# lamm-mit/MoleculeDiffusionTransformer

Measured on AMD Instinct MI355X. Metric: molecules/sec @64 diffusion steps (QM9 max_len=64), higher is better.
Workload: dtype f32 storage/accumulate; GEMM products as split-bf16 (bf16x3) MFMA; 1 GPU; QMDiffusion inverse sample(): channels=64 pred_dim=16 max_len=64 cond_len=12, batch=1024/GPU, 64 timesteps (126 U-Net evals), cond_scale=1.0, fp32; global_batch=1024, parallelism=batch-shard x1

## Files before the change

### include/mdt_hip.h

```cpp
#ifndef MDT_HIP_H
#define MDT_HIP_H

#include <stdint.h>

#ifdef __cplusplus
extern "C" {
#endif

#define MDT_ABI_VERSION 5

int mdt_abi_version(void);
const char *mdt_last_error(void);
int mdt_set_tuning(const char *key, int32_t value);
int32_t mdt_pair_capacity(void);
int32_t mdt_tf256_block_core(int32_t T, int32_t Tk, int32_t cross);
int mdt_test_occupy(int32_t n_workgroups, int32_t lds_bytes, uint64_t ticks, void *stream);


enum mdt_space {
  MDT_SP_NONE = 0,
  MDT_SP_WEIGHT = 1,
  MDT_SP_ACT = 2,
  MDT_SP_SHR = 3,
  MDT_SP_EXT0 = 4
// ... 65 lines not shown
                MDT_N_CA = 6      };
enum mdt_gn_f { MDT_NF_EPS = 0, MDT_NF_SCALE2 = 1 };

enum mdt_rconv_i { MDT_R_T = 0, MDT_R_C = 1, MDT_R_LDA = 2, MDT_R_LDC = 3, MDT_R_LDR = 4, MDT_R_TAPS = 5,
                   MDT_R_GSIZE = 6 , MDT_R_SILU = 7,
                   MDT_R_FILM_LD = 8 ,
                   MDT_R_LDA2 = 9 ,
                   MDT_R_WF32 = 10 ,
                   MDT_R_KSRC = 11 ,
                   MDT_R_HALF_OUT = 12 ,
                   MDT_R_NB = 13  };
enum mdt_rconv_f { MDT_RF_EPS = 0, MDT_RF_IN_SCALE = 1 ,
                   MDT_RF_IN_SCALE2 = 2  };
enum mdt_resblock_i { MDT_K_T = 0, MDT_K_CIN = 1, MDT_K_COUT = 2, MDT_K_FILM_LD = 3,
                      MDT_K_WF32 = 4 ,
                      MDT_K_CIN_REAL = 5, MDT_K_COUT_REAL = 6 ,
                      MDT_K_PATCH_IN = 7, MDT_K_PATCH_OUT = 8  };
enum mdt_resblock_f { MDT_KF_EPS = 0 };

enum mdt_attn_i {
  MDT_A_T = 0, MDT_A_TK = 1, MDT_A_HEADS = 2, MDT_A_LDQ = 3, MDT_A_LDKV = 4, MDT_A_LDO = 5,
  MDT_A_KV_BSTRIDE = 6,
  MDT_A_OUT16 = 7,
  MDT_A_QCOL = 8,
  MDT_A_KCOL = 9,
  MDT_A_SPLIT = 10,
  MDT_A_IN16 = 11
};
enum mdt_attn_f { MDT_AF_SCALE = 0 };

enum mdt_concat_i { MDT_C_ROWS = 0, MDT_C_CA = 1, MDT_C_CB = 2 };
enum mdt_concat_f { MDT_CF_SCALE_B = 0 };

enum mdt_patch_i { MDT_P_ROWS_IN = 0, MDT_P_C_IN = 1, MDT_P_LD_IN = 2, MDT_P_LD_OUT = 3, MDT_P_PATCH = 4,
                   MDT_P_INVERSE = 5 };

enum mdt_time_i { MDT_T_HALF = 0, MDT_T_LD = 1 };

enum mdt_tblock_mode { MDT_TB_SELF = 0, MDT_TB_CROSS = 1, MDT_TB_FF = 2 };
enum mdt_tblock_i {
  MDT_B_MODE = 0, MDT_B_C = 1,
  MDT_B_T = 2,
  MDT_B_NCHUNK = 3,
  MDT_B_NBIAS = 4, MDT_B_TK = 5, MDT_B_KV_BSTRIDE = 6, MDT_B_LDKV = 7, MDT_B_HEADS = 8,
  MDT_B_KV2 = 11,
  MDT_B_POST = 10,
  MDT_B_VARIANT = 9,
  MDT_B_WF32 = 12
};
enum mdt_tblock_f { MDT_BF_EPS = 0, MDT_BF_SCALE = 1 };

enum mdt_tf128_i {
  MDT_F_C = 0,
  MDT_F_T = 1,
  MDT_F_NT = 2,
  MDT_F_NVEC = 3,
  MDT_F_TK = 4, MDT_F_KV_BSTRIDE = 5, MDT_F_LDKV = 6, MDT_F_HEADS = 7,
  MDT_F_HAS_IN = 8,
  MDT_F_NBLOCKS = 9 , MDT_F_NFF = 10 ,
  MDT_F_NPOST = 11,
  MDT_F_KV2 = 12,
  MDT_F_CROSS = 13,
  MDT_F_KV_LSTRIDE = 14,
  MDT_F_RES_KIND = 15,
  MDT_F_N_RES = 16,
  MDT_F_RES_PAIR1 = 17,
  MDT_F_RES_PAIR2 = 18,
  MDT_F_NFILM = 19,
  MDT_F_NSPLIT = 20,
  MDT_F_PAIR_STRIDE = 21,
  MDT_F_WF32 = 22
};
enum mdt_tf128_f { MDT_FF_EPS_LN = 0, MDT_FF_SCALE = 1, MDT_FF_EPS_GN = 2, MDT_FF_EPS_RES = 3, MDT_FF_SKIP_SCALE = 4 };

typedef struct mdt_op {
  int32_t kind;
  int32_t film_bstride;
  mdt_ref a;
  mdt_ref a2;
  mdt_ref w;
  mdt_ref bias;
  mdt_ref out;
  mdt_ref res;
  mdt_ref p0, p1, p2, p3;
  int32_t i[24];
  float f[8];
} mdt_op;

typedef struct mdt_bindings {
  const float *weights;
  float *act;
  float *shr;
  float *ext[MDT_N_EXT];
} mdt_bindings;

typedef struct mdt_program mdt_program;

mdt_program *mdt_program_create(const mdt_op *ops, int32_t n_ops);
void mdt_program_destroy(mdt_program *p);
int32_t mdt_program_num_ops(const mdt_program *p);
int mdt_program_run(const mdt_program *p, const mdt_bindings *b, int32_t B, int32_t n_shared_rows,
                    int32_t first, int32_t count, void *stream);

int mdt_cond_embed(const float *seq, const float *fc1_w, const float *fc1_b, const float *inv_freq,
                   float *out, int32_t B, int32_t n, int32_t D1, int32_t D2, void *stream);
int mdt_cond_embed_add(const float *seq, const float *fc1_w, const float *fc1_b, const float *inv_freq,
                       float *out, int32_t B, int32_t n, int32_t D1, int32_t D2, void *stream);

int mdt_precond_in(const float *x, float *xin, float c_in, int32_t B, int32_t C, int32_t L, int32_t Cp,
                   void *stream);
int mdt_precond_out(const float *x, const float *pred, float *D, float c_skip, float c_out, int32_t B,
                    int32_t C, int32_t L, int32_t Cp, const float *dyn_scale, void *stream);
int mdt_dyn_scale(const float *x, const float *pred, float *scale, float c_skip, float c_out, float q, int32_t B,
                  int32_t C, int32_t L, int32_t Cp, void *stream);
int mdt_noise_in_rows(const float *x0, const float *noise, const float *sigma, const float *c_in, float *x_noisy, float *xin,
                      uint64_t seed, uint32_t step, int64_t sample0, int32_t B, int32_t C, int32_t L, int32_t Cp, void *stream);
int mdt_precond_in_rows(const float *x, float *xin, const float *c_in, int32_t B, int32_t C, int32_t L, int32_t Cp, void *stream);
int mdt_precond_out_rows(const float *x, const float *pred, float *D, const float *c_skip, const float *c_out, int32_t B,
                         int32_t C, int32_t L, int32_t Cp, const float *dyn_scale, void *stream);
int mdt_dyn_scale_rows(const float *x, const float *pred, float *scale, const float *c_skip, const float *c_out, float q,
                       int32_t B, int32_t C, int32_t L, int32_t Cp, void *stream);
int mdt_loss_rows(const float *x0, const float *x_noisy, const float *pred, const float *c_skip, const float *c_out,
                  const float *weight, const float *dyn_scale, float *loss, int32_t B, int32_t C, int32_t L, int32_t Cp,
                  void *stream);
int mdt_cfg_mix(const float *cond, const float *uncond, float *out, float scale, int64_t n, void *stream);
int mdt_cfg_mix_rows(const float *cond, const float *uncond, float *out, const float *scale, int32_t B, int64_t row_elems,
                     void *stream);
int mdt_adpm2_mid(const float *x, const float *pred, float *x_mid, float *xin_mid, float c_skip,
                  float c_out, float sigma, float dt_mid, float c_in_mid, int32_t B, int32_t C, int32_t L,
                  int32_t Cp, const float *dyn_scale, void *stream);
int mdt_adpm2_next(float *x, const float *x_mid, const float *pred, const float *noise, float *xin_next,
                   float c_skip, float c_out, float sigma_mid, float dt_down, float sigma_up,
                   float c_in_next, uint64_t seed, uint32_t step, int64_t sample0, int32_t B, int32_t C,
                   int32_t L, int32_t Cp, int32_t *tokens, const float *dyn_scale, void *stream);
int mdt_adpm2_euler(const float *x_base, const float *x_from, const float *denoised, const float *noise,
                    float *out, float sigma, float dt, float sigma_up, int32_t noise_mode, uint64_t seed,
                    uint32_t step, int64_t sample0, int32_t B, int32_t C, int32_t L, void *stream);
int mdt_aeuler_next(float *x, const float *pred, const float *noise, float *xin_next, float c_skip, float c_out,
                    float sigma, float dt, float sigma_up, float c_in_next, uint64_t seed, uint32_t step,
                    int64_t sample0, int32_t B, int32_t C, int32_t L, int32_t Cp, int32_t *tokens,
                    const float *dyn_scale, void *stream);
int mdt_karras_hat(const float *x, const float *noise, float *x_hat, float *xin, float noise_scale, float s_noise,
                   float c_in_hat, uint64_t seed, uint32_t step, int64_t sample0, int32_t B, int32_t C, int32_t L,
                   int32_t Cp, void *stream);
int mdt_karras_mid(const float *x_hat, const float *pred, float *d, float *x_next, float *xin_next, float c_skip,
                   float c_out, float sigma_hat, float dt, float c_in_next, int32_t B, int32_t C, int32_t L,
                   int32_t Cp, int32_t *tokens, const float *dyn_scale, void *stream);
int mdt_karras_next(const float *x_hat, const float *x_next, const float *d, const float *pred, float *x,
                    float c_skip, float c_out, float sigma_next, float half, int32_t B, int32_t C, int32_t L,
                    int32_t Cp, int32_t *tokens, const float *dyn_scale, void *stream);
int mdt_init_noise(float *x, const float *noise, float sigma0, uint64_t seed, uint32_t step,
                   int64_t sample0, int32_t B, int32_t C, int32_t L, void *stream);
int mdt_copy_f32(float *dst, const float *src, int64_t n, void *stream);
int mdt_clamp(float *x, float lo, float hi, int64_t n, void *stream);
int mdt_inpaint_merge(float *x, const float *src, const uint8_t *mask, const float *noise, float sigma,
                      uint64_t seed, uint32_t step, int64_t sample0, int32_t B, int32_t C, int32_t L,
                      void *stream);
int mdt_add_noise(float *x, const float *noise, float s, uint64_t seed, uint32_t step, int64_t sample0,
                  int32_t B, int32_t C, int32_t L, void *stream);
int mdt_inpaint_enter(float *x, float *xin, const float *src, const int32_t *draft, const uint8_t *keep,
                      int32_t keep_per_token, const float *n_src, const float *n_re, float sigma, float renoise,
                      float c_in, uint64_t seed, uint32_t step_src, uint32_t step_re, int64_t sample0, int32_t B,
                      int32_t C, int32_t L, int32_t Cp, void *stream);
int mdt_inpaint_finish(float *x, const float *src, const int32_t *draft, const uint8_t *keep, int32_t keep_per_token,
                       int32_t *tokens, int32_t B, int32_t C, int32_t L, void *stream);
int mdt_refine_enter(float *x, float *xin, const int32_t *start, int32_t step_i, const float *src, const int32_t *draft,
                     const float *noise, float sigma, float c_in, uint64_t seed, uint32_t step, int64_t sample0, int32_t B,
                     int32_t C, int32_t L, int32_t Cp, void *stream);
int mdt_refine_keep_enter(float *x, float *xin, const int32_t *start, int32_t step_i, const float *src, const int32_t *draft,
                          const uint8_t *keep, int32_t keep_per_token, const float *n_entry, const float *n_src, float sigma,
                          float c_in, uint64_t seed, uint32_t step_entry, uint32_t step_src, int64_t sample0, int32_t B,
                          int32_t C, int32_t L, int32_t Cp, void *stream);
int mdt_argmax_tokens(const float *x, int32_t *tokens, int32_t B, int32_t C, int32_t L, void *stream);

int mdt_tokens_compact(const int32_t *tokens, int32_t B, int32_t L, float *fwd_in, int32_t Lf, double x_norm, int32_t *packed,
                       int32_t *length, uint64_t *key, void *stream);
int mdt_screen_score(const float *props, int64_t row_stride, const float *target, const float *weights, int32_t N, int32_t G,
                     int32_t n, float *score, void *stream);
enum mdt_screen_status {
  MDT_SCREEN_EMPTY = 1,
  MDT_SCREEN_NONFINITE = 2,
  MDT_SCREEN_DUPLICATE = 4,
  MDT_SCREEN_KNOWN = 8,
  MDT_SCREEN_CLOSE = 16,
  MDT_SCREEN_MALFORMED = 32,
  MDT_SCREEN_OVERVALENT = 64,
  MDT_SCREEN_SUBSTRUCTURE = 128
};
int mdt_screen_select(const float *score, const uint64_t *key, const int32_t *packed, const int32_t *length, int32_t L, int32_t N,
                      int32_t G, const uint64_t *known_key, const int32_t *known_packed, const int32_t *known_len, int32_t M,
                      int32_t K, uint8_t *status, int32_t *index, int32_t *count, void *stream);
int mdt_screen_select_reject(const float *score, const uint64_t *key, const int32_t *packed, const int32_t *length, int32_t L,
                             int32_t N, int32_t G, const uint64_t *known_key, const int32_t *known_packed, const int32_t *known_len,
                             int32_t M, int32_t K, const uint8_t *reject, uint8_t *status, int32_t *index, int32_t *count,
                             void *stream);

int mdt_edit_distance_rows(const int32_t *a_packed, const int32_t *a_len, const int32_t *b_packed, const int32_t *b_len, int32_t L,
                           int32_t R, int32_t *dist, void *stream);
#define MDT_EDIT_KNOWN_CHUNK 512
int mdt_edit_nearest(const int32_t *packed, const int32_t *length, int32_t L, int32_t R, const int32_t *known_packed,
                     const int32_t *known_len, int32_t M, uint64_t *best, int32_t *dist, int32_t *index, void *stream);
int mdt_screen_select_diverse(const float *score, const uint64_t *key, const int32_t *packed, const int32_t *length, int32_t L,
                              int32_t N, int32_t G, const uint64_t *known_key, const int32_t *known_packed, const int32_t *known_len,
                              int32_t M, int32_t K, const int32_t *known_dist, int32_t min_novelty, int32_t min_distance,
                              uint8_t *status, int32_t *index, int32_t *count, void *stream);
int mdt_screen_select_diverse_reject(const float *score, const uint64_t *key, const int32_t *packed, const int32_t *length,
                                     int32_t L, int32_t N, int32_t G, const uint64_t *known_key, const int32_t *known_packed,
                                     const int32_t *known_len, int32_t M, int32_t K, const int32_t *known_dist, int32_t min_novelty,
                                     int32_t min_distance, const uint8_t *reject, uint8_t *status, int32_t *index, int32_t *count,
                                     void *stream);

int mdt_smiles_check(const int32_t *packed, const int32_t *length, int32_t L, int32_t R, const uint8_t *classes,
                     const uint8_t *max_valence, const uint32_t *elements, uint8_t *status, int32_t *position, void *stream);

int mdt_mol_graph(const int32_t *packed, const int32_t *length, int32_t L, int32_t R, const uint8_t *classes,
                  const uint8_t *max_valence, const uint32_t *elements, int32_t *natoms, uint32_t *atoms, int32_t *nbonds,
                  uint32_t *bonds, uint8_t *status, int32_t *position, void *stream);
int mdt_mol_key(const int32_t *natoms, const uint32_t *atoms, const int32_t *nbonds, const uint32_t *bonds, int32_t L, int32_t R,
                uint64_t *key, void *stream);
int mdt_key_flags(const uint64_t *key, int32_t N, int32_t G, const uint64_t *known_key, int32_t M, uint8_t *flags, void *stream);

#define MDT_FP_BITS 1024
#define MDT_FP_SIM_DEN 65536
int mdt_mol_fp(const int32_t *natoms, const uint32_t *atoms, const int32_t *nbonds, const uint32_t *bonds, int32_t L, int32_t R,
               int32_t radius, uint64_t *fp, int32_t *count, void *stream);
int mdt_fp_tanimoto_rows(const uint64_t *a_fp, const uint64_t *b_fp, int32_t R, int32_t *inter, int32_t *uni, void *stream);
#define MDT_FP_KNOWN_CHUNK 512
int mdt_fp_nearest(const uint64_t *fp, int32_t R, const uint64_t *known_fp, int32_t M, uint64_t *best, int32_t *inter, int32_t *uni,
                   int32_t *index, void *stream);
int mdt_screen_select_similar(const float *score, const uint64_t *key, const int32_t *packed, const int32_t *length, int32_t L,
                              int32_t N, int32_t G, const uint64_t *known_key, const int32_t *known_packed, const int32_t *known_len,
                              int32_t M, int32_t K, const int32_t *known_dist, int32_t min_novelty, int32_t min_distance,
                              const uint8_t *reject, const uint64_t *fp, const int32_t *fp_count, int32_t sim_num, uint8_t *status,
                              int32_t *index, int32_t *count, void *stream);

#define MDT_SUB_MAX_PATTERNS 32
#define MDT_SUB_MAX_WIDTH 32
#define MDT_SUB_MAX_STEPS 4096
int mdt_sub_match(const int32_t *natoms, const uint32_t *atoms, const int32_t *nbonds, const uint32_t *bonds, int32_t L, int32_t R,
                  const int32_t *p_natoms, const uint32_t *p_atoms, const int32_t *p_nbonds, const uint32_t *p_bonds,
                  int32_t LP, int32_t P, uint32_t need, uint32_t ban,
                  uint32_t *match, uint32_t *undecided, uint8_t *flags, void *stream);

#define MDT_MOLH_MAX_STEPS 4096
#define MDT_MOLH_FORMULA 13
enum mdt_molh_verdict { MDT_MOLH_OK = 0, MDT_MOLH_AROMATIC_OVERVALENT = 1, MDT_MOLH_NO_KEKULE = 2, MDT_MOLH_UNDECIDED = 3 };
int mdt_mol_hydrogens(const int32_t *natoms, const uint32_t *atoms, const int32_t *nbonds, const uint32_t *bonds, int32_t L, int32_t R,
                      int32_t max_steps, uint8_t *hydrogens, uint8_t *partner, uint8_t *verdict, int32_t *atom, int32_t *formula,
                      void *stream);

#define MDT_MOLR_DESC 16
enum mdt_molr_slot {
  MDT_MOLR_HEAVY_ATOMS = 0, MDT_MOLR_HETERO_ATOMS = 1, MDT_MOLR_DONORS = 2, MDT_MOLR_ACCEPTORS = 3, MDT_MOLR_ROTATABLE_BONDS = 4,
  MDT_MOLR_RINGS = 5, MDT_MOLR_RING_ATOMS = 6, MDT_MOLR_RING_BONDS = 7, MDT_MOLR_SMALLEST_RING = 8, MDT_MOLR_LARGEST_RING = 9,
  MDT_MOLR_AROMATIC_ATOMS = 10, MDT_MOLR_AROMATIC_OUTSIDE_RING = 11, MDT_MOLR_SP3_CARBONS = 12, MDT_MOLR_CARBONS = 13,
  MDT_MOLR_COMPONENTS = 14, MDT_MOLR_WEIGHT = 15
};
int mdt_mol_rings(const int32_t *natoms, const uint32_t *atoms, const int32_t *nbonds, const uint32_t *bonds, const uint8_t *hydrogens,
                  int32_t L, int32_t R, const int32_t *lo, const int32_t *hi, uint8_t *bond_ring, uint8_t *atom_ring, int32_t *desc,
                  uint8_t *flags, void *stream);

enum mdt_moln_flag { MDT_MOLN_NORMALIZED = 1, MDT_MOLN_AROMATIC = 2, MDT_MOLN_CHANGED = 4 };
int mdt_mol_normalize(const int32_t *natoms, const uint32_t *atoms, const int32_t *nbonds, const uint32_t *bonds,
                      const uint8_t *hydrogens, const uint8_t *partner, const uint8_t *verdict, const uint8_t *bond_ring, int32_t L,
                      int32_t R, uint32_t *out_atoms, uint32_t *out_bonds, uint8_t *flags, void *stream);

typedef struct mdt_timer mdt_timer;
mdt_timer *mdt_timer_create(int32_t max_intervals);
void mdt_timer_destroy(mdt_timer *t);
int mdt_timer_start(mdt_timer *t, void *stream);
int mdt_timer_stop(mdt_timer *t, void *stream);
int32_t mdt_timer_collect(mdt_timer *t, float *ms, int32_t cap);

#ifdef __cplusplus
}
#endif
#endif
```

### moleculediffusiontransformer_amd/build.py

```python
from __future__ import annotations

import hashlib
import os
import shutil
import subprocess
from concurrent.futures import ThreadPoolExecutor

CSRC = os.path.join(os.path.dirname(os.path.abspath(__file__)), "csrc")
INCLUDE = os.path.join(os.path.dirname(os.path.dirname(os.path.abspath(__file__))), "include")
_TAG = os.environ.get("MDT_LIB_TAG", "")
LIB = os.path.join(CSRC, f"libmdt_hip{'_' + _TAG if _TAG else ''}.so")
STAMP = os.path.join(CSRC, f".build_stamp{'_' + _TAG if _TAG else ''}")

SOURCES = [
    ("k_gemm.hip", []),
    ("k_gemm_bf16x3.hip", []),
    ("k_gemm_b16.hip", []),
    ("k_gemm_as.hip", []),
    ("k_tblock_lw.hip", ["-mllvm", "-amdgpu-mfma-vgpr-form=1"]),
    ("k_tblock32.hip", ["-mllvm", "-amdgpu-mfma-vgpr-form=1"]),
    ("k_tf128.hip", ["-mllvm", "-amdgpu-mfma-vgpr-form=1"]),
    ("k_tf128_f32.hip", ["-mllvm", "-amdgpu-mfma-vgpr-form=1"]),
    ("k_tf256.hip", ["-mllvm", "-amdgpu-mfma-vgpr-form=1"]),
    ("k_tf256_f32.hip", ["-mllvm", "-amdgpu-mfma-vgpr-form=1"]),
    ("k_rconv.hip", ["-mllvm", "-amdgpu-mfma-vgpr-form=1"]),
    ("k_rconv_f32.hip", ["-mllvm", "-amdgpu-mfma-vgpr-form=1"]),
    ("k_proj.hip", ["-mllvm", "-amdgpu-mfma-vgpr-form=1"]),
    ("k_res256.hip", ["-mllvm", "-amdgpu-mfma-vgpr-form=1"]),
    ("k_resblock.hip", ["-mllvm", "-amdgpu-mfma-vgpr-form=1"]),
    ("k_norm.hip", []),
    ("k_attn.hip", []),
    ("k_elem.hip", ["-ffp-contract=off"]),
    ("k_screen.hip", ["-ffp-contract=off"]),
    ("k_edit.hip", []),
    ("k_smiles.hip", []),
    ("k_molgraph.hip", []),
    ("k_molfp.hip", []),
    ("k_molsub.hip", []),
    ("k_molh.hip", []),
    ("k_molring.hip", []),
    ("k_molnorm.hip", []),
    ("mdt_api.cpp", ["-x", "hip"]),
]
COMMON = ["-O3", "-std=c++17", "-fPIC", "--offload-arch=gfx950", "-fno-gpu-rdc", "-Wall", "-Wno-unused-function"]


def _hipcc() -> str:
    for cand in (shutil.which("hipcc"), "/opt/rocm/bin/hipcc"):
        if cand and os.path.exists(cand):
            return cand
    raise RuntimeError("hipcc not found: libmdt_hip.so cannot be built")


def _digest() -> str:
    h = hashlib.sha256()
    paths = [os.path.join(CSRC, n) for n in sorted(os.listdir(CSRC))] + [os.path.join(INCLUDE, "mdt_hip.h")]
    for p in paths:
        if p.endswith((".hip", ".cpp", ".h")):
            h.update(os.path.basename(p).encode())
            with open(p, "rb") as f:
                h.update(f.read())
    h.update(repr((SOURCES, COMMON, os.environ.get('MDT_BUILD_DEFS', ''))).encode())
    return h.hexdigest()


def library_path() -> str:
    return LIB


def is_fresh() -> bool:
    if not (os.path.exists(LIB) and os.path.exists(STAMP)):
        return False
    with open(STAMP) as f:
        return f.read().strip() == _digest()


def build_library(force: bool = False, verbose: bool = False) -> str:
    if not force and is_fresh():
        return LIB
    import fcntl
    with open(os.path.join(CSRC, ".build_lock"), "w") as lock:
        fcntl.flock(lock, fcntl.LOCK_EX)
        try:
            if not force and is_fresh():
                return LIB
            return _build_locked(verbose)
        finally:
            fcntl.flock(lock, fcntl.LOCK_UN)


def _build_locked(verbose: bool) -> str:
    hipcc = _hipcc()

    def compile_one(item):
        src, extra = item
        obj = os.path.join(CSRC, os.path.splitext(src)[0] + (f".{_TAG}.o" if _TAG else ".o"))
        defs = os.environ.get("MDT_BUILD_DEFS", "").split()
        cmd = [hipcc, *COMMON, *extra, *defs, "-I", INCLUDE, "-c", os.path.join(CSRC, src), "-o", obj]
        r = subprocess.run(cmd, capture_output=True, text=True)
        if r.returncode != 0:
            raise RuntimeError(f"hipcc failed on {src}:\n{r.stdout}\n{r.stderr}")
        if verbose and r.stderr.strip():
            print(r.stderr)
        return obj

    with ThreadPoolExecutor(max_workers=min(5, os.cpu_count() or 1)) as ex:
        objs = list(ex.map(compile_one, SOURCES))
    cmd = [hipcc, "-shared", "-fPIC", "--offload-arch=gfx950", "-o", LIB, *objs]
    r = subprocess.run(cmd, capture_output=True, text=True)
    if r.returncode != 0:
        raise RuntimeError(f"link failed:\n{r.stdout}\n{r.stderr}")
    with open(STAMP, "w") as f:
        f.write(_digest())
    return LIB


if __name__ == "__main__":
    import sys
    print(build_library(force="--force" in sys.argv, verbose=True))
```

### moleculediffusiontransformer_amd/compiler.py

```python
from __future__ import annotations

import os
from dataclasses import dataclass, field
from typing import Dict, List, Optional, Tuple

import torch

from . import runtime as rt
from .netspec import UNetConfig

EXT_XIN, EXT_CTX, EXT_OUT = 0, 1, 2
EXT_XFLAGS, EXT_XBUF = 3, 4
EXT_FILM = 5


def pad16(c: int) -> int:
    return (c + 15) // 16 * 16


@dataclass
class Ten:
    space: int
    off: int
    rows: int
    ld: int
    c: int = 0
    b16: bool = False

    def ref(self) -> rt.MdtRef:
        return rt.MdtRef(self.space, 0, self.off)


def _ref(space: int = 0, off: int = 0) -> rt.MdtRef:
    return rt.MdtRef(space, 0, off)


class _Arena:

    def __init__(self):
        self.free: List[Tuple[int, int]] = []
        self.top = 0

    def alloc(self, n: int) -> int:
        n = (n + 63) // 64 * 64
        for i, (o, s) in enumerate(self.free):
            if s >= n:
                if s == n:
                    self.free.pop(i)
                else:
                    self.free[i] = (o + n, s - n)
                return o
        o = self.top
        self.top += n
        return o

    def release(self, off: int, n: int) -> None:
        n = (n + 63) // 64 * 64
        self.free.append((off, n))
        self.free.sort()
        merged: List[Tuple[int, int]] = []
        for o, s in self.free:
            if merged and merged[-1][0] + merged[-1][1] == o:
                merged[-1] = (merged[-1][0], merged[-1][1] + s)
            else:
                merged.append((o, s))
        self.free = merged


class _Weights:
    def __init__(self):
        self.chunks: List[torch.Tensor] = []
        self.n = 0
        self.index: Dict[str, int] = {}
        self.starts: Dict[int, torch.Tensor] = {}

    def read(self, off: int, n: int) -> torch.Tensor:
        t = self.starts[off]
        assert t.numel() >= n, (off, n, t.numel())
        return t[:n].clone()

    def add(self, name: str, t: torch.Tensor) -> int:
        t = t.detach().to(torch.float32).contiguous().reshape(-1).cpu()
        off = self.n
        pad = (-t.numel()) % 64
        self.chunks.append(t)
        self.starts[off] = t
        if pad:
            self.chunks.append(torch.zeros(pad))
        self.n += t.numel() + pad
        self.index[name] = off
        return off

    def pack(self) -> torch.Tensor:
        return torch.cat(self.chunks) if self.chunks else torch.zeros(0)


@dataclass
class CompiledUNet:
    cfg: UNetConfig
    length: int
    cond_len: int
    in_pad: int
    weights: torch.Tensor
    programs: Dict[str, List[rt.MdtOp]]
    act_floats: int
    shr_floats: int
    max_time_rows: int
    shr: Dict[str, int]
    ss_total: int
    n_cross: int
    flops_per_sample_eval: int
    flops_ctx_per_sample: int
    gemm_mode: str = "bf16x3"
    weight_index: Dict[str, int] = field(default_factory=dict)
    dual_multiple: int = 1
    tf256: bool = False
    xchg_tokens: int = 0
    rows: bool = False
    act_named: Dict[str, int] = field(default_factory=dict)


class UNetCompiler:
    def __init__(self, cfg: UNetConfig, length: int, cond_len: int, sd: Dict[str, torch.Tensor],
                 max_time_rows: int = 1024, gemm_mode: str = "bf16x3", fuse_blocks: bool = True, tf256: bool = False):
        self.fuse_blocks = fuse_blocks
        self.use_rconv = os.environ.get("MDT_RCONV", "1") == "1"
        self.use_resblock = os.environ.get("MDT_RESBLOCK", "1") == "1"
        self.t1_fold = os.environ.get("MDT_T1_FOLD", "1") == "1"
        self.ctx_split = os.environ.get("MDT_CTX_SPLIT", "1") == "1"
        self.fold_out = os.environ.get("MDT_FOLD_OUT", "1") == "1"
        self.rconv_two = os.environ.get("MDT_RCONV2", "k1") == "1"
        self.rconv_two_k1 = os.environ.get("MDT_RCONV2", "k1") in ("1", "k1")
        self.res128 = os.environ.get("MDT_RES128", "1") == "1"
        self.res256_mode = os.environ.get("MDT_RES256", "auto")
        self.patch_conv = os.environ.get("MDT_PATCH_CONV", "1") != "0"
        self.fold_patch = os.environ.get("MDT_FOLD_PATCH", "1") != "0"
        self.use_proj = os.environ.get("MDT_PROJ", "1") != "0"
        self.b16 = os.environ.get("MDT_B16", "1") == "1"
        self.res16 = os.environ.get("MDT_RES16", "1") == "1"
        self.lnfold = os.environ.get("MDT_LNFOLD", "1") == "1"
        self.cat_fold = os.environ.get("MDT_CAT_FOLD", "1") == "1"
        self.qkv_merge = os.environ.get("MDT_QKV_MERGE", "1") == "1"
        self.fold_ctx = os.environ.get("MDT_FOLD_CTX", "1") == "1"
        self.has_chat = False
        self.tf128 = os.environ.get("MDT_TF128", "1") == "1"
        self.tf256 = bool(tf256)
        self.tf256_pair = os.environ.get("MDT_TF256_PAIR", "1") == "1"
        self.pair_stride = int(os.environ.get("MDT_PAIR_STRIDE", "8"))
        self.xchg_tokens = 0
        if gemm_mode not in ("f32", "bf16x3", "bf16"):
            raise ValueError("gemm_mode must be 'f32' (exact fp32 MFMA), 'bf16x3' (split-bf16 MFMA, fp32-class) or 'bf16' "
                             "(plain bf16 products, reduced precision: layer-by-layer GEMMs only)")
        self.gemm_mode = gemm_mode
        self.wf32 = gemm_mode == "f32" and os.environ.get("MDT_F32_FUSED", "1") == "1"
        self.ring_mode = gemm_mode == "bf16x3" or self.wf32
        self.rows = False
        self._packed: Dict = {}
        self._zeros_off, self._zeros_len = 0, 0
        if cfg.channels % 16:
            raise ValueError("channels must be a multiple of 16")
        if length % (cfg.patch_size * _prod(cfg.factors)):
            raise ValueError("max_length must be divisible by patch_size * prod(factors)")
        if cfg.head_features != 64:
            raise ValueError("attention kernel is specialised for head_features == 64")
        if cfg.ctx_features % 16:
            raise ValueError("context features must be a multiple of 16")
        self.cfg, self.L, self.n_ctx, self.sd = cfg, length, cond_len, sd
        self.W = _Weights()
        self.arena = _Arena()
        self._ones_off: Dict[int, int] = {}
        self.ops: List[rt.MdtOp] = []
        self.flops = 0
        self.max_time_rows = max_time_rows
        self.kv_slots: List[int] = []
        self.kv_fixed: List[int] = []
        self.cross_layers: List[str] = []
        self.ss_offsets: Dict[str, int] = {}
        self.ss_total = 0
        self.shr_top = 0
        self.shr: Dict[str, int] = {}

    def use_rows(self) -> "UNetCompiler":
        if self.gemm_mode == "bf16":
            raise ValueError("the per-row evaluation (batched=True, eval_loss) is built and pinned for gemm_mode 'bf16x3' and 'f32'; "
                             "in the plain-bf16 mode the FiLM rows also enter MDT_OP_PREP16, which reads one shared row")
        self.rows = True
        self.res128, self.res256_mode = False, "0"
        return self

    def _shr_alloc(self, name: str, n: int) -> int:
        off = self.shr_top
        self.shr_top += (n + 63) // 64 * 64
        self.shr[name] = off
        return off

    def _new(self, rows: int, ld: int, c: int = 0) -> Ten:
        return Ten(rt.SP_ACT, self.arena.alloc(rows * ld), rows, ld, c or ld)

    def _new16(self, rows: int, n: int) -> Ten:
        return Ten(rt.SP_ACT, self.arena.alloc(rows * n // 2), rows, n, n, True)

    def _free(self, t: Ten) -> None:
        if t.space == rt.SP_ACT:
            self.arena.release(t.off, t.rows * t.ld // (2 if t.b16 else 1))

    def b16_ok(self, cin: int) -> bool:
        return self.gemm_mode == "bf16" and self.b16 and cin % 64 == 0

    def _ones(self, n: int) -> int:
        if n not in self._ones_off:
            self._ones_off[n] = self.W.add(f"ones{n}", torch.ones(n))
        return self._ones_off[n]

    def _zeros(self, n: int) -> int:
        if n > self._zeros_len:
            self._zeros_off = self.W.add(f"zeros{n}", torch.zeros(n))
            self._zeros_len = n
        return self._zeros_off

    def _vec(self, key: str, pad_to: int) -> int:
        v = self.sd[key]
        out = torch.zeros(pad_to)
        out[: v.numel()] = v
        return self.W.add(key, out)

    def _lin_w(self, key: str, n_pad: Optional[int] = None, k_pad: Optional[int] = None):
        w = self.sd[key]
        n, k = w.shape
        out = torch.zeros(n_pad or pad16(n), k_pad or pad16(k))
        out[:n, :k] = w
        return (key, out)

    def _conv_w(self, key: str, cin_pad: int, n_pad: int):
        w = self.sd[key]
        co, ci, k = w.shape
        out = torch.zeros(n_pad, k, cin_pad)
        out[:co, :, :ci] = w.permute(0, 2, 1)
        return (key, out.reshape(n_pad, k * cin_pad))

    def _pack_w(self, wt, cin: int):
        name, w = wt
        split = self.gemm_mode == "bf16x3" and cin % 32 == 0
        plain = self.gemm_mode == "bf16" and cin % 32 == 0
        key = (name, split, plain)
        if key not in self._packed:
            if plain:
                hi = w.to(torch.bfloat16)
                self._packed[key] = (self.W.add(name + "/bf16", hi.contiguous().view(-1).view(torch.float32)), None, 1)
            elif split:
                hi = w.to(torch.bfloat16)
                lo = (w - hi.float()).to(torch.bfloat16)
                self._packed[key] = (self.W.add(name + "/bf16_hi", hi.contiguous().view(-1).view(torch.float32)),
                                     self.W.add(name + "/bf16_lo", lo.contiguous().view(-1).view(torch.float32)))
            else:
                self._packed[key] = (self.W.add(name, w), None)
        return self._packed[key]

    def _emit(self, op: rt.MdtOp) -> None:
        self.ops.append(op)

    def gemm(self, a: Ten, wt, n: int, out: Ten, *, cin: int, bias_off: Optional[int] = None,
             taps: int = 1, t_stride: int = 1, t_dj: int = 0, t_off: int = 0, r_out: Optional[int] = None,
             o_stride: int = 1, o_off: int = 0, res: Optional[Ten] = None, pro: int = rt.PRO_NONE,
             gain: Optional[int] = None, nbias: Optional[int] = None, stats: Optional[Ten] = None,
             film: Optional[rt.MdtRef] = None, groups: int = 0, gsize: int = 0, pro_silu: int = 0,
             act: int = 0, eps: float = 0.0, m_mode: int = 0, a_col: int = 0, o_col: int = 0,
             count_flops: bool = True, phases: int = 0, copy16: Optional[Ten] = None) -> None:
        r_out_ = a.rows if r_out is None else r_out
        a16 = None
        regular = (self.b16_ok(cin) and t_stride == 1 and phases <= 1 and o_stride == 1 and o_off == 0 and r_out_ == a.rows
                   and out.rows == r_out_ and m_mode == 0)
        assert not (a.b16 or out.b16) or (regular and (not a.b16 or (pro in (rt.PRO_NONE, rt.PRO_LAYERNORM) and a_col == 0))), "bf16 operand"
        lnf = None
        if (self.lnfold and regular and a.b16 and pro == rt.PRO_LAYERNORM and taps == 1 and t_off == 0 and out.b16 and res is None
                and copy16 is None and n % 8 == 0 and o_col % 8 == 0 and out.ld % 8 == 0):
            key = (wt[0], "lnfold", gain, nbias, bias_off)
            if key not in self._packed:
                w = wt[1].double()
                gv, bv = self.W.read(gain, cin).double(), self.W.read(nbias, cin).double()
                b0 = self.W.read(bias_off, n).double() if bias_off is not None else torch.zeros(n, dtype=torch.float64)
                w2 = (w * gv.unsqueeze(0)).float()
                csum = w2.to(torch.bfloat16).double().sum(dim=1).float()
                self._packed[key] = ((wt[0] + "/lnfold", w2), self.W.add(wt[0] + "/lnfold.bias", (b0 + w @ bv).float()),
                                     self.W.add(wt[0] + "/lnfold.csum", csum))
            wt, bias_off, csum_off = self._packed[key]
            lnf = csum_off
            pro, gain, nbias = rt.PRO_NONE, None, None
        if regular and (not a.b16 or pro == rt.PRO_LAYERNORM):
            a16 = self._new16(a.rows, cin)
            pre = rt.MdtOp()
            pre.kind = rt.OP_PREP16
            pre.a, pre.out = a.ref(), a16.ref()
            if gain is not None:
                pre.p0 = _ref(rt.SP_WEIGHT, gain)
            if nbias is not None:
                pre.p1 = _ref(rt.SP_WEIGHT, nbias)
            if stats is not None:
                pre.p2 = stats.ref()
# ... 1322 lines not shown
            blocks = [dp + f"blocks.{j}." for j in range(nb)]
            res_ok = nb > 0 and all(self.res128_ok(bp, co, x.rows, g, False) for bp in blocks)
            together = res_ok and self.tf128_ok(co, x.rows, nat, nat > 0, 1, nb)
            alone = res_ok and not together and self.tf128_ok(co, x.rows, 0, False, 1, nb)
            if together or alone:
                n_out = nb + (1 if nat > 0 else 0)
                base = self.arena.alloc(n_out * x.rows * co)
                outs = [Ten(rt.SP_ACT, base + k * x.rows * co, x.rows, co, co) for k in range(n_out)]
                if together:
                    self.transformer_fused128(x, dp + "transformer.", co, nat, nat > 0, free_input=not x_is_skip,
                                              res=(1, blocks, g, outs[:nb], 1.0), y=outs[-1])
                else:
                    self.transformer_fused128(x, "", co, 0, False, free_input=not x_is_skip,
                                              res=(1, blocks, g, outs[:nb], 1.0), y=outs[nb - 1])
                    if nat > 0:
                        yy = self.transformer(outs[nb - 1], dp + "transformer.", co, nat, True, free_input=False, y_out=outs[nb])
                        if yy is not outs[nb]:
                            self._free(outs[nb])
                            outs[nb] = yy
                skips += outs
                x = outs[-1]
            elif nb > 0 and x.ld == co and all(self.res256_ok(bp, co, x.rows, g, False) for bp in blocks):
                n_out = nb + (1 if nat > 0 else 0)
                base = self.arena.alloc(n_out * x.rows * co)
                outs = [Ten(rt.SP_ACT, base + k * x.rows * co, x.rows, co, co) for k in range(n_out)]
                self.resnet_chain256(x, blocks, 1, outs[:nb], 1.0, outs[nb - 1], free_input=not x_is_skip)
                if nat > 0:
                    yy = self.transformer(outs[nb - 1], dp + "transformer.", co, nat, True, free_input=False, y_out=outs[nb])
                    if yy is not outs[nb]:
                        self._free(outs[nb])
                        outs[nb] = yy
                skips += outs
                x = outs[-1]
            else:
                for bp in blocks:
                    x = self.resnet(x, bp, co, co, g, free_input=not x_is_skip)
                    skips.append(x)
                    x_is_skip = True
                if nat > 0:
                    x = self.transformer(x, dp + "transformer.", co, nat, True, free_input=False)
                    skips.append(x)
            skips_list.append(skips)
        cb = cfg.level_channels(cfg.num_layers)
        keep = x in skips_list[-1]
        x = self.resnet(x, "bottleneck.pre_block.", cb, cb, g, free_input=not keep)
        if cfg.attentions[-1] > 0:
            x = self.transformer(x, "bottleneck.transformer.", cb, cfg.attentions[-1], True)
        x = self.resnet(x, "bottleneck.post_block.", cb, cb, g)
        for u, i in enumerate(reversed(range(cfg.num_layers))):
            up = f"upsamples.{u}."
            ci, co, f = cfg.level_channels(i + 1), cfg.level_channels(i), cfg.factors[i]
            skips = skips_list.pop()
            n_res = cfg.num_blocks[i] + (1 if cfg.attentions[i] else 0)
            blocks = [up + f"blocks.{j}." for j in range(n_res)]
            tfs = []
            if cfg.pre_transformer > 0:
                tfs.append((up + "pre_transformer_block.", cfg.pre_transformer, False))
            if cfg.attentions[i] > 0:
                tfs.append((up + "transformer.", cfg.attentions[i], True))
            cons = skips[len(skips) - n_res:][::-1] if 0 < n_res <= len(skips) else []
            nxt = tfs[0] if tfs else ("", 0, False)
            res_ok = (bool(cons) and x.ld == ci and all(self.res128_ok(bp, ci, x.rows, g, True) for bp in blocks)
                      and all(sk.space == rt.SP_ACT and sk.rows == x.rows and sk.ld == ci
                              and sk.off == cons[0].off - k * x.rows * ci for k, sk in enumerate(cons)))
            together = res_ok and nxt[1] > 0 and self.tf128_ok(ci, x.rows, nxt[1], nxt[2], 2, n_res)
            fused = together or (res_ok and self.tf128_ok(ci, x.rows, 0, False, 2, n_res))
            if fused:
                del skips[len(skips) - n_res:]
                if together:
                    x = self.transformer_fused128(x, nxt[0], ci, nxt[1], nxt[2], True, res=(2, blocks, g, cons, 2 ** -0.5))
                    tfs = tfs[1:]
                else:
                    x = self.transformer_fused128(x, "", ci, 0, False, True, res=(2, blocks, g, cons, 2 ** -0.5))
                for sk in cons:
                    self._free(sk)
            elif (bool(cons) and x.ld == ci and all(self.res256_ok(bp, ci, x.rows, g, True) for bp in blocks)
                  and all(sk.space == rt.SP_ACT and sk.rows == x.rows and sk.ld == ci
                          and sk.off == cons[0].off - k * x.rows * ci for k, sk in enumerate(cons))):
                del skips[len(skips) - n_res:]
                x = self.resnet_chain256(x, blocks, 2, cons, 2 ** -0.5, self._new(x.rows, ci), True)
                for sk in cons:
                    self._free(sk)
            else:
                for bp in blocks:
                    sk = skips.pop()
                    x = self.resnet_cat(x, sk, 2 ** -0.5, bp, ci, g)
            for sk in skips:
                self._free(sk)
            for tp, tl, tc in tfs:
                x = self.transformer(x, tp, ci, tl, tc)
            if f % 2:
                raise ValueError("odd upsample factors are not supported")
            wt = self.sd[up + "upsample.weight"]
            bias = self._vec(up + "upsample.bias", co)
            y = self._new(x.rows * f, co)
            last = u == cfg.num_layers - 1
            res = skips_list[0][0] if last else None
            if self.up_patch_ok(x, ci, co, f, res):
                self.up_patch(x, up, ci, co, f, y, res)
            else:
                wall = torch.cat([torch.stack((wt[:, :, ph], wt[:, :, ph + f]), dim=0).permute(2, 0, 1).reshape(co, 2 * ci)
                                  for ph in range(f)])
                self.gemm(x, (f"{up}upsample.weight/phases", wall), co, y, cin=ci, bias_off=bias, taps=2, t_stride=1,
                          t_dj=-1, t_off=0, r_out=x.rows, o_stride=f, o_off=0, res=res, phases=f)
            self._free(x)
            x = y
        self._free(skips_list.pop()[0])
        fold_in = (ps > 1 and self.fold_patch and x.ld % ps == 0
                   and self.resblock_ok(x.rows * ps, c0 // ps, cin, 1, "to_out.block.") and x.ld // ps == pad16(c0 // ps))
        if fold_in:
            x = Ten(x.space, x.off, x.rows * ps, x.ld // ps, x.ld // ps)
        elif ps > 1:
            y = self.patch(x, ps, inverse=True)
            self._free(x)
            x = y
        out = Ten(rt.SP_EXT0 + EXT_OUT, 0, L, self.in_pad, cin)
        y = self.resnet(x, "to_out.block.", c0 // ps, cin, 1)
        if fold_in:
            assert self.ops[-1].kind == rt.OP_RESBLOCK
            self.ops[-1].i[rt.K_PATCH_IN] = ps
        last_op = self.ops[-1]
        assert last_op.kind in (rt.OP_GEMM, rt.OP_RESBLOCK)
        last_op.out = out.ref()
        self._free(y)

    def build(self) -> CompiledUNet:
        cfg = self.cfg
        mid2 = 2 * cfg.mid_features
        self.build_eval()
        eval_ops = self.ops
        flops_eval = self.flops
        n_cross = len(self.cross_layers)
        kv_base = self.arena.top
        self.kv_slots = [kv_base + i * self.n_ctx * mid2 for i in range(n_cross)]
        act_floats = kv_base + n_cross * self.n_ctx * mid2
        chat_slot = act_floats
        if self.has_chat:
            act_floats += (self.n_ctx * cfg.ctx_features + 63) // 64 * 64

        rows = 0 if self.rows else self.max_time_rows
        mapf = cfg.mapping_features
        ldt = pad16(cfg.channels + 1)
        cn = self._shr_alloc("c_noise", rows)
        temb = self._shr_alloc("time_embed", rows * ldt)
        m1 = self._shr_alloc("map1", rows * mapf)
        m2 = self._shr_alloc("map2", rows * mapf)
        m3 = self._shr_alloc("map3", rows * mapf)
        ss_all = self._shr_alloc("ss_all", rows * self.ss_total)
        ss_cur = self._shr_alloc("ss_cur", self.ss_total)
        kvf = self._shr_alloc("kv_fixed", n_cross * self.n_ctx * mid2)
        self.kv_fixed = [kvf + i * self.n_ctx * mid2 for i in range(n_cross)]
        chat_fixed = self._shr_alloc("chat_fixed", self.n_ctx * cfg.ctx_features)

        def resolve(ops, fixed: bool):
            out = []
            for op in ops:
                o = rt.MdtOp()
                C_memmove(o, op)
                if op.kind in (rt.OP_GEMM, rt.OP_GN_ACT, rt.OP_RCONV, rt.OP_RESBLOCK, rt.OP_PREP16, rt.OP_TF128, rt.OP_RES256) and isinstance(getattr(op, "_film", None), tuple):
                    if self.rows:
                        if not (op.kind in (rt.OP_GN_ACT, rt.OP_RCONV, rt.OP_RESBLOCK)
                                or (op.kind == rt.OP_GEMM and op.i[rt.G_PRO] == rt.PRO_GROUPNORM and op.i[rt.G_WFMT] == 0
                                    and op.i[rt.G_M_MODE] == 0)):
                            raise NotImplementedError(f"per-row evaluation: the FiLM rows reach op kind {op.kind} "
                                                      f"({rt.OP_NAMES.get(op.kind)}), which reads one shared row: this U-Net shape is "
                                                      "outside the per-row envelope")
                        o.p3 = _ref(rt.SP_EXT0 + EXT_FILM, op._film[1])
                        o.film_bstride = self.ss_total
                    else:
                        o.p3 = _ref(rt.SP_SHR, ss_cur + op._film[1])
                if op.kind == rt.OP_ATTN_CTX:
                    if fixed:
                        o.a2 = _ref(rt.SP_SHR, chat_fixed)
                        o.i[rt.A_KV_BSTRIDE] = 0
                    else:
                        o.a2 = _ref(rt.SP_ACT, chat_slot)
                elif op.kind in (rt.OP_ATTN, rt.OP_TBLOCK, rt.OP_TF128, rt.OP_TF256) and isinstance(getattr(op, "_kv", None), tuple):
                    idx = op._kv[1]
                    slot = {rt.OP_ATTN: rt.A_KV_BSTRIDE, rt.OP_TBLOCK: rt.B_KV_BSTRIDE, rt.OP_TF128: rt.F_KV_BSTRIDE,
                            rt.OP_TF256: rt.F_KV_BSTRIDE}[op.kind]
                    if fixed:
                        o.a2 = _ref(rt.SP_SHR, self.kv_fixed[idx])
                        o.i[slot] = 0
                    else:
                        o.a2 = _ref(rt.SP_ACT, self.kv_slots[idx])
                out.append(o)
            return out

        if self.rows:
            programs = {"eval_rows": resolve(eval_ops, False), "eval_rows_fixed": resolve(eval_ops, True)}
        else:
            programs = {"eval": resolve(eval_ops, False), "eval_fixed": resolve(eval_ops, True)}
        cross = [op for op in eval_ops if isinstance(getattr(op, "_kv", None), tuple)]
        ring = all(op.kind in (rt.OP_TF128, rt.OP_TF256) or
                   (op.kind == rt.OP_TBLOCK and (op.i[rt.B_VARIANT] >= 2 or (op.i[rt.B_VARIANT] == 0 and op.i[rt.B_C] == 128
                                                                         and (16 // op.i[rt.B_T]) * op.i[rt.B_TK] <= 16)))
                   for op in cross)
        dual_multiple = 1
        if cross and ring and not self.rows and os.environ.get("MDT_CFG_DUAL", "1") == "1":
            dual_multiple = max(64 // op.i[rt.F_T] if op.kind == rt.OP_TF128 else 32 // op.i[rt.F_T] if op.kind == rt.OP_TF256
                                else (32 if op.i[rt.B_VARIANT] >= 2 else 64) // op.i[rt.B_T] for op in cross)
            dual = resolve(eval_ops, False)
            for o, op in zip(dual, eval_ops):
                if isinstance(getattr(op, "_kv", None), tuple):
                    o.p1 = _ref(rt.SP_SHR, self.kv_fixed[op._kv[1]])
                    o.i[rt.F_KV2 if op.kind in (rt.OP_TF128, rt.OP_TF256) else rt.B_KV2] = 1
            programs["eval_dual"] = dual

        self.ops, self.flops = [], 0
        act_named: Dict[str, int] = {}
        tm = 0 if self.rows else 1
        if self.rows:
            def act_alloc(name: str, n: int) -> int:
                nonlocal act_floats
                off = act_named[name] = act_floats
                act_floats += (n + 63) // 64 * 64
                return off
            sp = rt.SP_ACT
            cn, temb = act_alloc("c_noise", 1), act_alloc("time_embed", ldt)
            m1, m2, m3 = act_alloc("map1", mapf), act_alloc("map2", mapf), act_alloc("map3", mapf)
        else:
            sp = rt.SP_SHR
        t_cn = Ten(sp, cn, 1, 1)
        t_emb = Ten(sp, temb, 1, ldt)
        op = rt.MdtOp()
        op.kind = rt.OP_TIME_EMBED
        op.a, op.w, op.out = t_cn.ref(), _ref(rt.SP_WEIGHT, self.W.add("to_time.0.0.weights", self.sd["to_time.0.0.weights"])), t_emb.ref()
        op.i[rt.T_HALF], op.i[rt.T_LD] = cfg.channels // 2, ldt
        self._emit(op)
        t1, t2, t3 = Ten(sp, m1, 1, mapf), Ten(sp, m2, 1, mapf), Ten(sp, m3, 1, mapf)
        self.gemm(t_emb, self._lin_w("to_time.0.1.weight", mapf, ldt), mapf, t1, cin=ldt,
                  bias_off=self._vec("to_time.0.1.bias", mapf), act=1, m_mode=tm)
        self.gemm(t1, self._lin_w("to_mapping.0.weight"), mapf, t2, cin=mapf,
                  bias_off=self._vec("to_mapping.0.bias", mapf), act=1, m_mode=tm)
        self.gemm(t2, self._lin_w("to_mapping.2.weight"), mapf, t3, cin=mapf,
                  bias_off=self._vec("to_mapping.2.bias", mapf), act=1, m_mode=tm)
        w_all = torch.zeros(self.ss_total, mapf)
        b_all = torch.zeros(self.ss_total)
        for p, off in self.ss_offsets.items():
            w = self.sd[p + "to_scale_shift.to_scale_shift.1.weight"]
            b = self.sd[p + "to_scale_shift.to_scale_shift.1.bias"]
            c = w.shape[0] // 2
            cp = pad16(c)
            w_all[off: off + c] = w[:c]
            w_all[off + cp: off + cp + c] = w[c:]
            b_all[off: off + c] = b[:c]
            b_all[off + cp: off + cp + c] = b[c:]
        t_ss = Ten(rt.SP_EXT0 + EXT_FILM, 0, 1, self.ss_total) if self.rows else Ten(rt.SP_SHR, ss_all, 1, self.ss_total)
        self.gemm(t3, ("scale_shift_all.weight", w_all), self.ss_total, t_ss, cin=mapf,
                  bias_off=self.W.add("scale_shift_all.bias", b_all), pro=rt.PRO_SILU, m_mode=tm)
        programs["time_rows" if self.rows else "time"] = self.ops

        self.ops, self.flops = [], 0
        ctx = Ten(rt.SP_EXT0 + EXT_CTX, 0, self.n_ctx, cfg.ctx_features)
        fixed = Ten(rt.SP_WEIGHT, self.W.add("fixed_embedding.embedding.weight",
                                             self.sd["fixed_embedding.embedding.weight"][: self.n_ctx]),
                    self.n_ctx, cfg.ctx_features)
        ctx_ops, fixed_ops = [], []
        for idx, p in enumerate(self.cross_layers):
            w = self._lin_w(p + "to_kv.weight")
            gain = self._vec(p + "norm_context.weight", cfg.ctx_features)
            nb = self._vec(p + "norm_context.bias", cfg.ctx_features)
            self.ops = ctx_ops
            self.gemm(ctx, w, mid2, Ten(rt.SP_ACT, self.kv_slots[idx], self.n_ctx, mid2), cin=cfg.ctx_features,
                      pro=rt.PRO_LAYERNORM, gain=gain, nbias=nb, eps=1e-5)
            self.ops = fixed_ops
            self.gemm(fixed, w, mid2, Ten(rt.SP_SHR, self.kv_fixed[idx], self.n_ctx, mid2), cin=cfg.ctx_features,
                      pro=rt.PRO_LAYERNORM, gain=gain, nbias=nb, eps=1e-5, m_mode=2, count_flops=False)
        if self.has_chat:
            F_ = cfg.ctx_features
            eye = ("ctx_identity", torch.eye(F_))
            ones, zeros = self.W.add("ctx_ones", torch.ones(F_)), self._zeros(F_)
            self.ops = ctx_ops
            self.gemm(ctx, eye, F_, Ten(rt.SP_ACT, chat_slot, self.n_ctx, F_), cin=F_, pro=rt.PRO_LAYERNORM, gain=ones,
                      nbias=zeros, eps=1e-5)
            self.ops = fixed_ops
            self.gemm(fixed, eye, F_, Ten(rt.SP_SHR, chat_fixed, self.n_ctx, F_), cin=F_, pro=rt.PRO_LAYERNORM, gain=ones,
                      nbias=zeros, eps=1e-5, m_mode=2, count_flops=False)
        programs["ctx"], programs["ctx_fixed"] = ctx_ops, fixed_ops
        flops_ctx = self.flops

        return CompiledUNet(cfg=cfg, length=self.L, cond_len=self.n_ctx, in_pad=self.in_pad, weights=self.W.pack(),
                            programs=programs, act_floats=act_floats, shr_floats=self.shr_top,
                            max_time_rows=rows, shr=dict(self.shr), ss_total=self.ss_total, n_cross=n_cross,
                            flops_per_sample_eval=flops_eval, flops_ctx_per_sample=flops_ctx, gemm_mode=self.gemm_mode,
                            weight_index=dict(self.W.index), dual_multiple=dual_multiple, tf256=self.tf256,
                            xchg_tokens=self.xchg_tokens, rows=self.rows, act_named=act_named)


def C_memmove(dst: rt.MdtOp, src: rt.MdtOp) -> None:
    import ctypes
    ctypes.memmove(ctypes.byref(dst), ctypes.byref(src), ctypes.sizeof(rt.MdtOp))


def _prod(xs) -> int:
    r = 1
    for x in xs:
        r *= x
    return r


def compile_unet(cfg: UNetConfig, length: int, cond_len: int, sd: Dict[str, torch.Tensor],
                 max_time_rows: int = 1024, gemm_mode: str = "bf16x3", fuse_blocks: bool = True,
                 tf256: bool = False, rows: bool = False) -> CompiledUNet:
    comp = UNetCompiler(cfg, length, cond_len, sd, max_time_rows, gemm_mode, fuse_blocks, tf256)
    return (comp.use_rows() if rows else comp).build()
```

### moleculediffusiontransformer_amd/csrc/k_tf128.hip

```cpp
#include <cstdlib>
#include <type_traits>

#include "mdt_kernels.h"
#include "mdt_device.h"

#ifndef MDT_TF_F32
#define MDT_TF_F32 0
#endif

#ifndef MDT_KV_CPOL
#define MDT_KV_CPOL 2
#endif

namespace mdt {

namespace {

enum { K_T = 0, K_N = 1, K_O = 2 };

constexpr int C = 128;
constexpr int SLOT = 256 * C;
constexpr int NS = 4;
constexpr int IPT = C / 16;
constexpr int NST = C / 32;
constexpr int NCT = C / 16;
constexpr int NU = 8;

typedef short s16x4 __attribute__((ext_vector_type(4)));
__device__ __forceinline__ f32x4 mfma_k16(const bf16x4& a, const bf16x4& b, const f32x4& c) {
  return __builtin_amdgcn_mfma_f32_16x16x16bf16_1k(__builtin_bit_cast(s16x4, a), __builtin_bit_cast(s16x4, b), c, 0, 0, 0);
}
__device__ __forceinline__ f32x4 scores_split(const f32x4* kf, const f32x4* qf) {
  f32x4 s = {0.f, 0.f, 0.f, 0.f};
#pragma unroll
  for (int sp = 0; sp < 2; ++sp) {
    float kv[8], qv[8];
#pragma unroll
    for (int e = 0; e < 8; ++e) {
      kv[e] = kf[2 * sp + (e >> 2)][e & 3];
      qv[e] = qf[2 * sp + (e >> 2)][e & 3];
    }
    bf16x8 kh, kl, qh, ql;
    split8<false>(kv, kh, kl);
    split8<false>(qv, qh, ql);
    s = MDT_MFMA_BF16(kl, qh, s, 0, 0, 0);
    s = MDT_MFMA_BF16(kh, ql, s, 0, 0, 0);
    s = MDT_MFMA_BF16(kh, qh, s, 0, 0, 0);
  }
  return s;
}
__device__ __forceinline__ void split_v(const f32x4* vT, bf16x4* vh, bf16x4* vl) {
#pragma unroll
  for (int dt = 0; dt < 4; ++dt) {
    const float v[4] = {vT[dt][0], vT[dt][1], vT[dt][2], vT[dt][3]};
    split4(v, vh[dt], vl[dt]);
  }
}
__device__ __forceinline__ void pv_split(const bf16x4* vh, const bf16x4* vl, const float p[4], f32x4* oT) {
  bf16x4 ph, pl;
  split4(p, ph, pl);
  const f32x4 zero = {0.f, 0.f, 0.f, 0.f};
#pragma unroll
  for (int dt = 0; dt < 4; ++dt) oT[dt] = mfma_k16(vl[dt], ph, zero);
#pragma unroll
  for (int dt = 0; dt < 4; ++dt) oT[dt] = mfma_k16(vh[dt], pl, oT[dt]);
#pragma unroll
  for (int dt = 0; dt < 4; ++dt) oT[dt] = mfma_k16(vh[dt], ph, oT[dt]);
}

}

template <int NPW, int RES, bool F32>
__global__ __launch_bounds__(512) void k_tf128(TFArgs a) {
  extern __shared__ __attribute__((aligned(1024))) unsigned char smem[];

  const int tid = threadIdx.x, lane = tid & 63;
  const int wave = __builtin_amdgcn_readfirstlane(tid >> 6);
  const int NT = a.NT;
  const unsigned char* wsrc = reinterpret_cast<const unsigned char*>(a.w);

  if (wave >= 4) {
    const int iw = wave - 4;
    __builtin_amdgcn_s_setprio(MDT_LOADER_PRIO);
    const cu32p tiles = (cu32p)a.tiles;
    const int lpP = lane >> 5;
    const int xP = (lane & 15) ^ lpP;
    const int baseP = ((lane >> 4) & 1) * (128 * C) + lpP * (2 * C);
    const int xO = (lane & 7) ^ (lane >> 4);
    const int baseO = (lane >> 3) * 128;
    unsigned voffP[IPT], voffO[IPT];
#pragma unroll
    for (int q = 0; q < IPT; ++q) {
      const int inst = iw + 4 * q;
      const int U = 2 * inst;
      voffP[q] = F32 ? (unsigned)(inst * 1024 + lane * 16) : (unsigned)(U * (2 * C) + ((xP ^ (U & 15)) << 4) + baseP);
      voffO[q] = F32 ? (unsigned)(inst * 1024 + lane * 16)
                     : (unsigned)(((inst * 8) / C) * (128 * C) + ((inst * 8) % C) * 128 + ((xO ^ (4 * (inst & 1))) << 4) + baseO);
    }
    const int sample0 = blockIdx.x * (64 / a.T);
    const bool second = a.kv2 && sample0 >= a.nsamples / 2;
    unsigned voffKV[4];
    if constexpr (NPW > 0) {
      const int kv_rows = (64 / a.T) * a.Tk;
      const int bstr = second ? 0 : a.kv_bstride;
#pragma unroll
      for (int q = 0; q < NPW; ++q) {
        const int R = 4 * (iw + 4 * q) + (lane >> 4);
        const int Rc = min(R, kv_rows - 1);
        const int sm = min(Rc / a.Tk, a.nsamples - 1 - sample0), key = Rc % a.Tk;
        voffKV[q] = (unsigned)(((sm * bstr + key) * a.ldkv + 4 * ((lane & 15) ^ (R & 15))) * 4);
      }
    }
    const int rowb = blockIdx.x * 64;
    auto pieces_of = [&](unsigned d) -> int { return (NPW > 0 && (d & 2u)) ? NPW : IPT; };
    auto issue_tile = [&](int tau, unsigned d) {
      unsigned char* slot = smem + MDT_SLOT_IDX(tau) * SLOT + iw * 1024;
      const unsigned kind = d & 3u, aux = d >> 2;
      if (NPW > 0 && kind >= 2u) {
        if constexpr (NPW > 0) {
          const int layer = (int)(aux >> 4), head = (int)(aux & 15u);
          const float* lb = second ? a.kv2 + (int64_t)layer * a.kv2_lstride
                                   : a.kv + (int64_t)layer * a.kv_lstride + (int64_t)sample0 * a.kv_bstride * a.ldkv;
          const unsigned char* base = reinterpret_cast<const unsigned char*>(lb + 64 * head + (kind == 3u ? 64 * a.nheads : 0));
#pragma unroll
          for (int q = 0; q < NPW; ++q)
            __builtin_amdgcn_global_load_lds(base + voffKV[q], (__attribute__((address_space(3))) void*)(slot + q * 4096), 16, 0, MDT_KV_CPOL);
        }
      } else if (RES == 2 && kind == 0u && (aux >> 20)) {
        if constexpr (RES == 2) {
          const unsigned char* base = reinterpret_cast<const unsigned char*>(
              a.skip + (int64_t)(aux & 0xffu) * a.skip_stride + (int64_t)blockIdx.x * 64 * C);
#pragma unroll
          for (int q = 0; q < IPT; ++q) {
            const int R = 2 * (iw + 4 * q) + (lane >> 5), pch = lane & 31;
            const int c = (pch & 16) | ((pch & 15) ^ (R & 15));
            const unsigned off = (unsigned)((min(rowb + R, a.M - 1) - rowb) * (C * 4) + c * 16);
            __builtin_amdgcn_global_load_lds(base + off, (__attribute__((address_space(3))) void*)(slot + q * 4096), 16, 0, 0);
          }
        }
      } else {
        const unsigned char* tile = wsrc + (int64_t)aux * SLOT;
        const bool ptile = kind == 0u;
#pragma unroll
        for (int q = 0; q < IPT; ++q) {
          const unsigned off = ptile ? voffP[q] : voffO[q];
          __builtin_amdgcn_global_load_lds(tile + off, (__attribute__((address_space(3))) void*)(slot + q * 4096), 16, 0, 0);
        }
      }
    };
    auto wait_vm = [&](int allow) {
      switch (allow) {
        case 0: asm volatile("s_waitcnt vmcnt(0)" ::: "memory"); break;
        case 1: asm volatile("s_waitcnt vmcnt(1)" ::: "memory"); break;
        case 2: asm volatile("s_waitcnt vmcnt(2)" ::: "memory"); break;
        case 3: asm volatile("s_waitcnt vmcnt(3)" ::: "memory"); break;
        case 4: asm volatile("s_waitcnt vmcnt(4)" ::: "memory"); break;
        case 5: asm volatile("s_waitcnt vmcnt(5)" ::: "memory"); break;
        case 6: asm volatile("s_waitcnt vmcnt(6)" ::: "memory"); break;
        case 7: asm volatile("s_waitcnt vmcnt(7)" ::: "memory"); break;
        default: asm volatile("s_waitcnt vmcnt(8)" ::: "memory"); break;
      }
    };
    const unsigned d0 = tiles[0], d1 = NT > 1 ? tiles[1] : 0u;
    __builtin_amdgcn_s_barrier();
    for (int q = iw; q * 256 < a.nvec; q += 4)
      __builtin_amdgcn_global_load_lds(reinterpret_cast<const unsigned char*>(a.vec) + q * 1024 + lane * 16,
                                       (__attribute__((address_space(3))) void*)(smem + NS * SLOT + q * 1024), 16, 0, 0);
    if constexpr (RES > 0) {
      for (int q = iw; q * 256 < a.nfilm; q += 4)
        __builtin_amdgcn_global_load_lds(reinterpret_cast<const unsigned char*>(a.film) + q * 1024 + lane * 16,
                                         (__attribute__((address_space(3))) void*)(smem + NS * SLOT + a.nvec * 4 + q * 1024), 16, 0, 0);
    }
    issue_tile(0, d0);
    if (NT > 1) issue_tile(1, d1);
    unsigned dn = d1;
    for (int k = 0; k < NT; ++k) {
      const unsigned d2 = k + 2 < NT ? tiles[k + 2] : 0u;
      if (k + 1 < NT && pieces_of(dn) == IPT) asm volatile("s_waitcnt vmcnt(8)" ::: "memory");
      else if (NPW > 0 && k + 1 < NT) asm volatile("s_waitcnt vmcnt(%0)" ::"n"(NPW > 0 ? NPW : 1) : "memory");
      else wait_vm(k + 1 < NT ? pieces_of(dn) : 0);
      __builtin_amdgcn_s_barrier();
      if (k + 2 < NT) issue_tile(k + 2, d2);
      dn = d2;
    }
    prefetch_next_weights(a.pf_ptr, a.pf_lines, iw * 64 + lane);
    return;
  }

  const int i = lane & 15, g = lane >> 4;
  const int row0 = blockIdx.x * 64 + wave * 16;
  const int m = row0 + i;
  const bool mvalid = m < a.M;
  const int mc = mvalid ? m : a.M - 1;
  float* vec_s = reinterpret_cast<float*>(smem + NS * SLOT);

  f32x4 accT[NCT];
  {
    const float* xp = a.x + (int64_t)mc * C + 4 * g;
    float4 xr[NCT];
#pragma unroll
    for (int ct = 0; ct < NCT; ++ct) xr[ct] = *reinterpret_cast<const float4*>(xp + 16 * ct);
    __builtin_amdgcn_sched_barrier(0);
    __builtin_amdgcn_s_barrier();
    __builtin_amdgcn_sched_barrier(0);
#pragma unroll
    for (int ct = 0; ct < NCT; ++ct) accT[ct] = f32x4{xr[ct].x, xr[ct].y, xr[ct].z, xr[ct].w};
  }

  int aP[NST], aO[2];
#pragma unroll
  for (int st = 0; st < NST; ++st) {
    const int lc = 4 * st + g;
    aP[st] = F32 ? lane * 16 : i * (4 * C) + ((lc & ~15) | ((lc & 15) ^ i)) * 16;
  }
#pragma unroll
  for (int sp = 0; sp < 2; ++sp) aO[sp] = F32 ? lane * 16 : i * 128 + ((4 * sp + g) ^ ((i >> 1) & 7)) * 16;

  bf16x8 fh[3][2], fl[3][2];
  auto frag_read = [&](auto kind, unsigned base, auto uc, int set, auto jc) __attribute__((always_inline)) {
    constexpr int KIND = decltype(kind)::value, u = decltype(uc)::value, j = decltype(jc)::value;
    constexpr int q = j >> 1, lo = j & 1;
    constexpr int off = F32 ? ((KIND == K_O) ? ((2 * (u % (NCT / 2)) + q) * 4096 + (u / (NCT / 2)) * 2048 + lo * 1024)
                                             : ((2 * (u & 1) + q) * 8192 + (u >> 1) * 2048 + lo * 1024))
                            : ((KIND == K_O) ? ((2 * (u % (NCT / 2)) + q) * 16 * 128 + lo * (C * 128))
                                             : ((2 * (u & 1) + q) * 16 * 4 * C + lo * (2 * C)));
#ifdef MDT_ABL_LDSBC
    lds_read16_off<off>(lo ? fl[set][q] : fh[set][q], base & 0x18000u);
#else
    lds_read16_off<off>(lo ? fl[set][q] : fh[set][q], base);
#endif
  };
  using J0 = std::integral_constant<int, 0>;
  using J1 = std::integral_constant<int, 1>;
  using J2 = std::integral_constant<int, 2>;
  using J3 = std::integral_constant<int, 3>;
  auto prefetch2 = [&](auto kind, const unsigned char* slot, int off) __attribute__((always_inline)) {
    constexpr int KIND = decltype(kind)::value;
    const unsigned base = lds_addr(slot) + (KIND == K_O ? aO[0] : aP[0]);
    frag_read(kind, base, J0{}, off % 3, J0{}); frag_read(kind, base, J0{}, off % 3, J1{});
    frag_read(kind, base, J0{}, off % 3, J2{}); frag_read(kind, base, J0{}, off % 3, J3{});
    frag_read(kind, base, J1{}, (off + 1) % 3, J0{}); frag_read(kind, base, J1{}, (off + 1) % 3, J1{});
    frag_read(kind, base, J1{}, (off + 1) % 3, J2{}); frag_read(kind, base, J1{}, (off + 1) % 3, J3{});
  };

  int tau = 0;
  auto slot_of = [&](int t) -> const unsigned char* { return smem + MDT_SLOT_IDX(t) * SLOT; };

  auto phase = [&](auto kind, auto offc, auto nkind, bool has_next, f32x4* acc, const bf16x8* bh, const bf16x8* bl) __attribute__((always_inline)) {
    constexpr int KIND = decltype(kind)::value, OFF = decltype(offc)::value, NK = decltype(nkind)::value;
    const unsigned lc = lds_addr(slot_of(tau)), ln = lds_addr(slot_of(tau + 1));
    unsigned bc[4];
#pragma unroll
    for (int k = 0; k < 4; ++k) bc[k] = lc + (KIND == K_O ? aO[k & 1] : aP[k]);
    const unsigned bn = ln + (NK == K_O ? aO[0] : aP[0]);
    auto unit = [&](auto uc) __attribute__((always_inline)) {
      constexpr int u = decltype(uc)::value;
      if (u == NU - 2 && has_next) {
        __builtin_amdgcn_sched_barrier(0);
        __builtin_amdgcn_s_barrier();
        __builtin_amdgcn_sched_barrier(0);
      }
      constexpr int s0 = (OFF + u) % 3, s2 = (OFF + u + 2) % 3;
      constexpr bool in_phase = u + 2 < NU;
      const bool pre = in_phase || has_next;
      const bool later = (u + 1 < NU) || has_next;
      if (later) lgkm_wait<4>(); else lgkm_wait<0>();
      constexpr int ia = (KIND == K_O) ? 2 * (u % (NCT / 2)) : 2 * (u & 1);
      constexpr int ib = (KIND == K_O) ? u / (NCT / 2) : (u >> 1);
      auto rd = [&](auto jc) __attribute__((always_inline)) {
        if (!pre) return;
        __builtin_amdgcn_sched_barrier(0);
        if constexpr (in_phase) {
          constexpr int u2 = u + 2;
          frag_read(kind, bc[KIND == K_O ? u2 / (NCT / 2) : (u2 >> 1)], std::integral_constant<int, u2>{}, s2, jc);
        } else {
          frag_read(nkind, bn, std::integral_constant<int, u + 2 - NU>{}, s2, jc);
        }
        __builtin_amdgcn_sched_barrier(0);
      };
      auto mm = [&](const bf16x8& w, const bf16x8& x, int q) __attribute__((always_inline)) {
        if constexpr (KIND == K_N) acc[ia + q] = MDT_MFMA_BF16(x, w, acc[ia + q], 0, 0, 0);
        else acc[ia + q] = MDT_MFMA_BF16(w, x, acc[ia + q], 0, 0, 0);
      };
      if constexpr (F32) {
        auto mm4 = [&](const bf16x8& w0, const bf16x8& w1, const bf16x8& x, auto r0c) __attribute__((always_inline)) {
          constexpr int r0 = decltype(r0c)::value;
          const f32x4 a0 = __builtin_bit_cast(f32x4, w0), a1 = __builtin_bit_cast(f32x4, w1), xb = __builtin_bit_cast(f32x4, x);
#pragma unroll
          for (int r = r0; r < r0 + 2; ++r) {
            if constexpr (KIND == K_N) {
              acc[ia] = MDT_MFMA_F32(xb[r], a0[r], acc[ia], 0, 0, 0);
              acc[ia + 1] = MDT_MFMA_F32(xb[r], a1[r], acc[ia + 1], 0, 0, 0);
            } else {
              acc[ia] = MDT_MFMA_F32(a0[r], xb[r], acc[ia], 0, 0, 0);
              acc[ia + 1] = MDT_MFMA_F32(a1[r], xb[r], acc[ia + 1], 0, 0, 0);
            }
          }
        };
        mm4(fh[s0][0], fh[s0][1], bh[ib], J0{}); rd(J0{});
        mm4(fh[s0][0], fh[s0][1], bh[ib], J2{}); rd(J1{});
        mm4(fl[s0][0], fl[s0][1], bl[ib], J0{}); rd(J2{});
        mm4(fl[s0][0], fl[s0][1], bl[ib], J2{}); rd(J3{});
      } else {
        mm(fl[s0][0], bh[ib], 0); rd(J0{});
        mm(fl[s0][1], bh[ib], 1); rd(J1{});
        mm(fh[s0][0], bl[ib], 0); rd(J2{});
        mm(fh[s0][1], bl[ib], 1); rd(J3{});
        mm(fh[s0][0], bh[ib], 0);
        mm(fh[s0][1], bh[ib], 1);
      }
      __builtin_amdgcn_sched_barrier(0);
    };
    unit(std::integral_constant<int, 0>{}); unit(std::integral_constant<int, 1>{});
    unit(std::integral_constant<int, 2>{}); unit(std::integral_constant<int, 3>{});
    unit(std::integral_constant<int, 4>{}); unit(std::integral_constant<int, 5>{});
    unit(std::integral_constant<int, 6>{}); unit(std::integral_constant<int, 7>{});
    ++tau;
  };
  using IC0 = std::integral_constant<int, 0>;
  using IC1 = std::integral_constant<int, 1>;
  using IC2 = std::integral_constant<int, 2>;
  const IC0 kT{};
  const IC1 kN{};
  const IC2 kO{};

  const f32x4 zero4 = f32x4{0.f, 0.f, 0.f, 0.f};
  const float t1 = a.T > 1 ? 1.f : 0.f, t2 = a.T > 2 ? 1.f : 0.f, t4 = a.T > 4 ? 1.f : 0.f, t8 = a.T > 8 ? 1.f : 0.f;
  auto dpp_fma = [](float v, float f, auto ctrl) {
// ... 87 lines not shown
#pragma unroll
        for (int r = 0; r < 4; ++r) {
          const float d = src[ct][r] - mu[ct];
          ss += d * d;
        }
        rs[ct] = ss;
      }
      reduce(rs);
#pragma unroll
      for (int ct = 0; ct < NCT; ++ct) rs[ct] = __builtin_amdgcn_rsqf(rs[ct] * inv_n + a.eps_res);
    };
    auto gn_operands = [&](const f32x4* src, const float (&mu)[NCT], const float (&rs)[NCT], const float* gam, const float* bet,
                           const float* film) __attribute__((always_inline)) {
#pragma unroll
      for (int st = 0; st < NST; ++st) {
        float v[8];
#pragma unroll
        for (int hf = 0; hf < 2; ++hf) {
          const int ct = 2 * st + hf;
          const float4 gv = *reinterpret_cast<const float4*>(gam + 16 * ct + 4 * g);
          const float4 bv = *reinterpret_cast<const float4*>(bet + 16 * ct + 4 * g);
          const float g4[4] = {gv.x, gv.y, gv.z, gv.w}, b4[4] = {bv.x, bv.y, bv.z, bv.w};
          float u[4];
#pragma unroll
          for (int r = 0; r < 4; ++r) {
            const float sc = rs[ct] * g4[r];
            u[r] = src[ct][r] * sc + (b4[r] - sc * mu[ct]);
          }
          if (film) {
            const float4 fv = *reinterpret_cast<const float4*>(film + 16 * ct + 4 * g);
            const float4 hv = *reinterpret_cast<const float4*>(film + C + 16 * ct + 4 * g);
            const float f4[4] = {fv.x, fv.y, fv.z, fv.w}, h4[4] = {hv.x, hv.y, hv.z, hv.w};
#pragma unroll
            for (int r = 0; r < 4; ++r) u[r] = u[r] * f4[r] + (u[r] + h4[r]);
          }
#pragma unroll
          for (int r = 0; r < 4; ++r) v[4 * hf + r] = mvalid ? u[r] * __builtin_amdgcn_rcpf(1.0f + __expf(-u[r])) : 0.f;
        }
        split8<F32>(v, xh[st], xl[st]);
      }
    };
    auto raw_operands = [&](const f32x4* src) __attribute__((always_inline)) {
#pragma unroll
      for (int st = 0; st < NST; ++st) {
        float v[8];
#pragma unroll
        for (int e = 0; e < 8; ++e) v[e] = mvalid ? src[2 * st + (e >> 2)][e & 3] : 0.f;
        split8<F32>(v, xh[st], xl[st]);
      }
    };
    auto set_vec = [&](f32x4* acc, const float* p, bool add) __attribute__((always_inline)) {
#pragma unroll
      for (int ct = 0; ct < NCT; ++ct) {
        const float4 b = *reinterpret_cast<const float4*>(p + 16 * ct + 4 * g);
        const f32x4 bb = f32x4{b.x, b.y, b.z, b.w};
        acc[ct] = add ? acc[ct] + bb : bb;
      }
    };
    auto conv3 = [&](auto o0, f32x4* acc, bool has_next) __attribute__((always_inline)) {
      constexpr int O0 = decltype(o0)::value;
      using A0 = std::integral_constant<int, O0 % 3>;
      using A1 = std::integral_constant<int, (O0 + 2) % 3>;
      using A2 = std::integral_constant<int, (O0 + 1) % 3>;
      bf16x8 sh[NST], sl[NST];
#pragma unroll
      for (int st = 0; st < NST; ++st) { sh[st] = row_shift<true>(xh[st], keep_l); sl[st] = row_shift<true>(xl[st], keep_l); }
      phase(kT, A0{}, kT, true, acc, sh, sl);
      phase(kT, A1{}, kT, true, acc + 4, sh, sl);
      phase(kT, A2{}, kT, true, acc, xh, xl);
      phase(kT, A0{}, kT, true, acc + 4, xh, xl);
#pragma unroll
      for (int st = 0; st < NST; ++st) { sh[st] = row_shift<false>(xh[st], keep_r); sl[st] = row_shift<false>(xl[st], keep_r); }
      phase(kT, A1{}, kT, true, acc, sh, sl);
      phase(kT, A2{}, kT, has_next, acc + 4, sh, sl);
    };
    const bool tf_follows = a.has_in || a.nblocks > 0;
    float mu[NCT], rs[NCT];
    for (int rb = 0; rb < a.n_res; ++rb) {
      const bool more = rb + 1 < a.n_res || tf_follows;
      const float* pv = vec_s + voff;
      f32x4 hT[NCT];
      if constexpr (RES == 1) {
        gn_stats(accT, a.res_pair1 != 0, mu, rs);
        gn_operands(accT, mu, rs, pv, pv + C, nullptr);
        set_vec(hT, pv + 2 * C, false);
        conv3(IC0{}, hT, true);
        gn_stats(hT, a.res_pair2 != 0, mu, rs);
        gn_operands(hT, mu, rs, pv + 3 * C, pv + 4 * C, film_s + rb * 2 * C);
        set_vec(accT, pv + 5 * C, true);
        conv3(IC0{}, accT, more);
        if (mvalid) {
          float* so = a.skip + (int64_t)rb * a.skip_stride + (int64_t)m * C + 4 * g;
#pragma unroll
          for (int ct = 0; ct < NCT; ++ct)
            store_nt(so + 16 * ct, make_float4(accT[ct][0], accT[ct][1], accT[ct][2], accT[ct][3]));
        }
        voff += 6 * C;
      } else {
        auto skip_rows = [&](f32x4* xbT) __attribute__((always_inline)) {
          __builtin_amdgcn_s_barrier();
          const unsigned char* ss_ = slot_of(tau) + (wave * 16 + i) * (C * 4);
#pragma unroll
          for (int ct = 0; ct < NCT; ++ct) {
            const int ch = 4 * ct + g;
            const float4 xr = *reinterpret_cast<const float4*>(ss_ + (((ch & 16) | ((ch & 15) ^ i)) << 4));
            xbT[ct] = f32x4{xr.x, xr.y, xr.z, xr.w} * a.skip_scale;
          }
          asm volatile("s_waitcnt lgkmcnt(0)" ::: "memory");
          ++tau;
          __builtin_amdgcn_s_barrier();
        };
        f32x4 rT[NCT];
        raw_operands(accT);
        set_vec(rT, pv + 5 * C, false);
        phase(kT, IC0{}, kT, true, rT, xh, xl);
        phase(kT, IC2{}, kT, false, rT + 4, xh, xl);
        {
          f32x4 xbT[NCT];
          skip_rows(xbT);
          prefetch2(kT, slot_of(tau), 0);
          raw_operands(xbT);
        }
        phase(kT, IC0{}, kT, true, rT, xh, xl);
        phase(kT, IC2{}, kT, true, rT + 4, xh, xl);
        gn_stats(accT, a.res_pair1 != 0, mu, rs);
        gn_operands(accT, mu, rs, pv, pv + 2 * C, nullptr);
        set_vec(hT, pv + 4 * C, false);
        conv3(IC1{}, hT, false);
        {
          f32x4 xbT[NCT];
          skip_rows(xbT);
          gn_stats(xbT, a.res_pair1 != 0, mu, rs);
          gn_operands(xbT, mu, rs, pv + C, pv + 3 * C, nullptr);
          prefetch2(kT, slot_of(tau), 0);
        }
        conv3(IC0{}, hT, true);
#pragma unroll
        for (int ct = 0; ct < NCT; ++ct) accT[ct] = rT[ct];
        gn_stats(hT, a.res_pair2 != 0, mu, rs);
        gn_operands(hT, mu, rs, pv + 6 * C, pv + 7 * C, film_s + rb * 2 * C);
        set_vec(accT, pv + 8 * C, true);
        conv3(IC0{}, accT, more);
        voff += 9 * C;
      }
    }
  }
  const int samp_q = i / a.T;
  float kmask[4];
#pragma unroll
  for (int r = 0; r < 4; ++r) kmask[r] = ((4 * g + r) / a.T == samp_q) ? 0.f : -INFINITY;
  const float scale2 = a.scale * 1.44269504088896340736f;
  int aK = 0, xK = 0, aV[4] = {0, 0, 0, 0}, xV[4] = {0, 0, 0, 0};
  bool kok[4] = {false, false, false, false};
  if constexpr (NPW > 0) {
    const int nkeys = (16 / a.T) * a.Tk;
    const int Rw = wave * nkeys;
    const int Rk = Rw + min(i, nkeys - 1);
    aK = Rk * 256;
    xK = Rk & 15;
#pragma unroll
    for (int r = 0; r < 4; ++r) {
      const int jj = 4 * g + r;
      const int Rv = Rw + min(jj, nkeys - 1);
      aV[r] = Rv * 256 + (i & 3) * 4;
      xV[r] = Rv & 15;
      kok[r] = jj < nkeys && (jj / a.Tk) == samp_q;
    }
  }
  if (a.has_in) {
    float gm[NCT], gv[NCT];
#pragma unroll
    for (int ct = 0; ct < NCT; ++ct) gm[ct] = (accT[ct][0] + accT[ct][1]) + (accT[ct][2] + accT[ct][3]);
    token_sum(gm);
    const float inv_n = 1.0f / (float)(4 * a.T);
#pragma unroll
    for (int ct = 0; ct < NCT; ++ct) {
      gm[ct] *= inv_n;
      float ss = 0.f;
#pragma unroll
      for (int r = 0; r < 4; ++r) {
        const float d = accT[ct][r] - gm[ct];
        ss += d * d;
      }
      gv[ct] = ss;
    }
    token_sum(gv);
#pragma unroll
    for (int ct = 0; ct < NCT; ++ct) {
      const float rs = __builtin_amdgcn_rsqf(gv[ct] * inv_n + a.eps_gn);
#pragma unroll
      for (int r = 0; r < 4; ++r) accT[ct][r] = (accT[ct][r] - gm[ct]) * rs;
    }
    make_operands(false);
    add_vec(voff, true);
    phase(kT, IC0{}, kT, true, accT, xh, xl);
    phase(kT, IC2{}, kT, false, accT + 4, xh, xl);
    __builtin_amdgcn_s_barrier();
    prefetch2(kT, slot_of(tau), 0);
    voff += C;
  }

  const int nheads = a.nheads, nff = a.nff;
  for (int blk = 0; blk < a.nblocks; ++blk) {
    const bool last_blk = blk + 1 == a.nblocks;
    {
      make_operands(true);
      add_vec(voff + 64 * nheads, false);
      const unsigned bias_l = vec_l + 4u * (unsigned)voff + 16u * (unsigned)g;
      for (int h = 0; h < nheads; ++h) {
        f32x4 oT[4];
        f32x4 qT[4], kTt[4], vT[4];
#pragma unroll
        for (int ft = 0; ft < 4; ++ft) { qT[ft] = zero4; kTt[ft] = zero4; vT[ft] = zero4; }
        phase(kT, IC0{}, kT, true, qT, xh, xl);
        phase(kT, IC2{}, kN, true, kTt, xh, xl);
        phase(kN, IC1{}, kN, false, vT, xh, xl);
        __builtin_amdgcn_s_barrier();
        prefetch2(kO, slot_of(tau), 1);
        {
          f32x4 bq[4];
          lds_read_f4_off<0>(bq[0], bias_l + 256 * h); lds_read_f4_off<64>(bq[1], bias_l + 256 * h);
          lds_read_f4_off<128>(bq[2], bias_l + 256 * h); lds_read_f4_off<192>(bq[3], bias_l + 256 * h);
          lgkm_wait<0>();
#pragma unroll
          for (int ft = 0; ft < 4; ++ft) qT[ft] += bq[ft];
        }
#ifdef MDT_ABL_ATTN
#pragma unroll
        for (int dt = 0; dt < 4; ++dt) oT[dt] = qT[dt] + kTt[dt] + vT[dt];
#else
        f32x4 s0 = zero4, s1 = zero4;
        bf16x4 vh[4], vl[4];
        if constexpr (F32) {
#pragma unroll
          for (int ft = 0; ft < 4; ++ft) {
            s0 = MDT_MFMA_F32(kTt[ft][0], qT[ft][0], s0, 0, 0, 0);
            s1 = MDT_MFMA_F32(kTt[ft][1], qT[ft][1], s1, 0, 0, 0);
            s0 = MDT_MFMA_F32(kTt[ft][2], qT[ft][2], s0, 0, 0, 0);
            s1 = MDT_MFMA_F32(kTt[ft][3], qT[ft][3], s1, 0, 0, 0);
          }
        } else {
          s0 = scores_split(kTt, qT);
          split_v(vT, vh, vl);
        }
        f32x4 st;
        float mx = -INFINITY;
#pragma unroll
        for (int r = 0; r < 4; ++r) {
          const float sv = (F32 ? s0[r] + s1[r] : s0[r]) * scale2 + kmask[r];
          st[r] = sv;
          mx = fmaxf(mx, sv);
        }
        mx = xg16_max(mx);
        mx = xg32_max(mx);
        float sum = 0.f;
#pragma unroll
        for (int r = 0; r < 4; ++r) {
          const float e = __builtin_amdgcn_exp2f(st[r] - mx);
          st[r] = e;
          sum += e;
        }
        sum = xg16_add(sum);
        sum = xg32_add(sum);
        const float inv = __builtin_amdgcn_rcpf(sum);
        if constexpr (F32) {
#pragma unroll
          for (int dt = 0; dt < 4; ++dt) oT[dt] = zero4;
#pragma unroll
          for (int r = 0; r < 4; ++r) {
            const float p = st[r] * inv;
#pragma unroll
            for (int dt = 0; dt < 4; ++dt) oT[dt] = MDT_MFMA_F32(vT[dt][r], p, oT[dt], 0, 0, 0);
          }
        } else {
          const float p[4] = {st[0] * inv, st[1] * inv, st[2] * inv, st[3] * inv};
          pv_split(vh, vl, p, oT);
        }
#endif
        bf16x8 oh[2], ol[2];
#pragma unroll
        for (int sp = 0; sp < 2; ++sp) {
          float v[8];
#pragma unroll
          for (int e = 0; e < 8; ++e) v[e] = oT[2 * sp + (e >> 2)][e & 3];
          split8<F32>(v, oh[sp], ol[sp]);
        }
        phase(kO, IC1{}, kT, true, accT, oh, ol);
      }
      voff += 64 * nheads + C;
    }
    if constexpr (NPW > 0) {
      make_operands(true);
      add_vec(voff + 64 * nheads, false);
      const unsigned bias_l = vec_l + 4u * (unsigned)voff + 16u * (unsigned)g;
      for (int h = 0; h < nheads; ++h) {
        f32x4 oT[4];
        f32x4 qT[4];
#pragma unroll
        for (int ft = 0; ft < 4; ++ft) qT[ft] = zero4;
        phase(kT, IC0{}, kT, false, qT, xh, xl);
        __builtin_amdgcn_s_barrier();
        const unsigned char* sk = slot_of(tau);
        float4 kk[4];
#pragma unroll
        for (int ft = 0; ft < 4; ++ft)
          kk[ft] = *reinterpret_cast<const float4*>(sk + aK + (((4 * ft + g) ^ xK) << 4));
        {
          f32x4 bq[4];
          lds_read_f4_off<0>(bq[0], bias_l + 256 * h); lds_read_f4_off<64>(bq[1], bias_l + 256 * h);
          lds_read_f4_off<128>(bq[2], bias_l + 256 * h); lds_read_f4_off<192>(bq[3], bias_l + 256 * h);
          lgkm_wait<0>();
#pragma unroll
          for (int ft = 0; ft < 4; ++ft) qT[ft] += bq[ft];
        }
        f32x4 s0 = zero4, s1 = zero4;
#ifndef MDT_ABL_ATTNX
        if constexpr (F32) {
#pragma unroll
          for (int ft = 0; ft < 4; ++ft) {
            s0 = MDT_MFMA_F32(kk[ft].x, qT[ft][0], s0, 0, 0, 0);
            s1 = MDT_MFMA_F32(kk[ft].y, qT[ft][1], s1, 0, 0, 0);
            s0 = MDT_MFMA_F32(kk[ft].z, qT[ft][2], s0, 0, 0, 0);
            s1 = MDT_MFMA_F32(kk[ft].w, qT[ft][3], s1, 0, 0, 0);
          }
        } else {
          f32x4 kf[4];
#pragma unroll
          for (int ft = 0; ft < 4; ++ft) kf[ft] = f32x4{kk[ft].x, kk[ft].y, kk[ft].z, kk[ft].w};
          s0 = scores_split(kf, qT);
        }
#endif
        ++tau;
        __builtin_amdgcn_s_barrier();
        const unsigned char* sv = slot_of(tau);
        f32x4 vT[4];
#pragma unroll
        for (int dt = 0; dt < 4; ++dt)
#pragma unroll
          for (int r = 0; r < 4; ++r)
            vT[dt][r] = *reinterpret_cast<const float*>(sv + aV[r] + (((4 * dt + (i >> 2)) ^ xV[r]) << 4));
#ifdef MDT_ABL_ATTNX
#pragma unroll
        for (int dt = 0; dt < 4; ++dt) oT[dt] = qT[dt] + f32x4{kk[dt].x, kk[dt].y, kk[dt].z, kk[dt].w} + vT[dt] + s0 + s1;
#else
        bf16x4 vh[4], vl[4];
        if constexpr (!F32) split_v(vT, vh, vl);
        f32x4 st;
        float mx = -INFINITY;
#pragma unroll
        for (int r = 0; r < 4; ++r) {
          const float sv2 = kok[r] ? (F32 ? s0[r] + s1[r] : s0[r]) * scale2 : -INFINITY;
          st[r] = sv2;
          mx = fmaxf(mx, sv2);
        }
        mx = xg16_max(mx);
        mx = xg32_max(mx);
        float sum = 0.f;
#pragma unroll
        for (int r = 0; r < 4; ++r) {
          const float e = __builtin_amdgcn_exp2f(st[r] - mx);
          st[r] = e;
          sum += e;
        }
        sum = xg16_add(sum);
        sum = xg32_add(sum);
        const float inv = __builtin_amdgcn_rcpf(sum);
        if constexpr (F32) {
#pragma unroll
          for (int dt = 0; dt < 4; ++dt) oT[dt] = zero4;
#pragma unroll
          for (int r = 0; r < 4; ++r) {
            const float p = st[r] * inv;
#pragma unroll
            for (int dt = 0; dt < 4; ++dt) oT[dt] = MDT_MFMA_F32(vT[dt][r], p, oT[dt], 0, 0, 0);
          }
        } else {
          const float p[4] = {st[0] * inv, st[1] * inv, st[2] * inv, st[3] * inv};
          pv_split(vh, vl, p, oT);
        }
#endif
        asm volatile("s_waitcnt lgkmcnt(0)" ::: "memory");
        ++tau;
        __builtin_amdgcn_s_barrier();
        prefetch2(kO, slot_of(tau), 1);
        bf16x8 oh[2], ol[2];
#pragma unroll
        for (int sp = 0; sp < 2; ++sp) {
          float v[8];
#pragma unroll
          for (int e = 0; e < 8; ++e) v[e] = oT[2 * sp + (e >> 2)][e & 3];
          split8<F32>(v, oh[sp], ol[sp]);
        }
        phase(kO, IC1{}, kT, true, accT, oh, ol);
      }
      voff += 64 * nheads + C;
    }
    {
      const int npost = last_blk ? a.npost : 0;
      make_operands(false);
      add_vec(voff + 64 * nff, npost > 0);
      const unsigned bias_l = vec_l + 4u * (unsigned)voff + 16u * (unsigned)g;
      for (int h = 0; h < nff; ++h) {
        const bool more = h + 1 < nff;
        f32x4 oT[4];
#pragma unroll
        for (int ft = 0; ft < 4; ++ft) oT[ft] = zero4;
        phase(kT, IC0{}, kT, false, oT, xh, xl);
        __builtin_amdgcn_s_barrier();
        prefetch2(kO, slot_of(tau), 1);
        {
          f32x4 b1[4];
          lds_read_f4_off<0>(b1[0], bias_l + 256 * h); lds_read_f4_off<64>(b1[1], bias_l + 256 * h);
          lds_read_f4_off<128>(b1[2], bias_l + 256 * h); lds_read_f4_off<192>(b1[3], bias_l + 256 * h);
          lgkm_wait<0>();
#pragma unroll
          for (int ft = 0; ft < 4; ++ft)
#pragma unroll
#ifdef MDT_ABL_GELU
            for (int r = 0; r < 4; ++r) oT[ft][r] = oT[ft][r] + b1[ft][r];
#else
            for (int r = 0; r < 4; ++r) oT[ft][r] = gelu(oT[ft][r] + b1[ft][r]);
#endif
        }
        bf16x8 oh[2], ol[2];
#pragma unroll
        for (int sp = 0; sp < 2; ++sp) {
          float v[8];
#pragma unroll
          for (int e = 0; e < 8; ++e) v[e] = oT[2 * sp + (e >> 2)][e & 3];
          split8<F32>(v, oh[sp], ol[sp]);
        }
        if (npost > 0 && !more) phase(kO, IC1{}, kO, true, accT, oh, ol);
        else phase(kO, IC1{}, kT, more || !last_blk, accT, oh, ol);
      }
      if (npost > 0) {
        phase(kO, IC0{}, kO, true, accT, xh, xl);
        phase(kO, IC2{}, kT, false, accT, xh + 2, xl + 2);
      }
      voff += 64 * nff + C;
    }
  }

  if (mvalid) {
    float* xo = a.out + (int64_t)m * C + 4 * g;
#pragma unroll
    for (int ct = 0; ct < NCT; ++ct)
      store_nt(xo + 16 * ct, make_float4(accT[ct][0], accT[ct][1], accT[ct][2], accT[ct][3]));
  }
}

template <int NPW, int RES, bool F32>
static hipError_t launch_tf(const TFArgs& a, hipStream_t s) {
  const size_t smem = (size_t)NS * SLOT + (size_t)(a.nvec + (RES > 0 ? a.nfilm : 0)) * sizeof(float);
  static DevOnce attr_once;
  if (attr_once.first()) {
    (void)hipFuncSetAttribute(reinterpret_cast<const void*>(&k_tf128<NPW, RES, F32>), hipFuncAttributeMaxDynamicSharedMemorySize,
                              (int)(160 * 1024));
  }
  hipLaunchKernelGGL((k_tf128<NPW, RES, F32>), dim3((unsigned)((a.M + 63) / 64)), dim3(512), smem, s, a);
  return hipGetLastError();
}

template <int RES, bool F32>
static hipError_t launch_tf_res(const TFArgs& a, hipStream_t s, bool cross) {
  if (!cross) return launch_tf<0, RES, F32>(a, s);
  switch (((64 / a.T) * a.Tk + 15) / 16) {
    case 1: return launch_tf<1, RES, F32>(a, s);
    case 2: return launch_tf<2, RES, F32>(a, s);
    case 3: return launch_tf<3, RES, F32>(a, s);
    case 4: return launch_tf<4, RES, F32>(a, s);
    default: return hipErrorInvalidValue;
  }
}

#if MDT_TF_F32
hipError_t launch_tf128_f32(const TFArgs& a, hipStream_t s) {
#else
bool tf128_supported(int T, int Tk, int nvec, bool cross) {
  if (T <= 0 || 16 % T || nvec <= 0 || nvec % 256 || nvec > 8192) return false;
  if (cross && (Tk <= 0 || (16 / T) * Tk > 16)) return false;
  return true;
}

hipError_t launch_tf128(const TFArgs& a, hipStream_t s) {
  if (a.wf32) return launch_tf128_f32(a, s);
#endif
  if (a.M <= 0) return hipSuccess;
  const bool cross = a.kv != nullptr;
  if (!tf128_supported(a.T, a.Tk, a.nvec, cross) || a.nblocks < 0 || a.NT <= 0 || a.nheads <= 0 || a.nff <= 0)
    return hipErrorInvalidValue;
  if (a.npost != 0 && a.npost != 2) return hipErrorInvalidValue;
  if (a.n_res < 0 || a.res_kind < 0 || a.res_kind > 2 || (a.res_kind == 0) != (a.n_res == 0)) return hipErrorInvalidValue;
  if (a.n_res == 0 && a.nblocks == 0) return hipErrorInvalidValue;
  if (a.n_res > 0 && (!a.skip || !a.film || a.nfilm % 256 || a.nfilm < 2 * C * a.n_res || a.nvec + a.nfilm > 8192))
    return hipErrorInvalidValue;
  if (a.nblocks == 0 && a.has_in) return hipErrorInvalidValue;
  constexpr bool kF32 = MDT_TF_F32 != 0;
  switch (a.res_kind) {
    case 0: return launch_tf_res<0, kF32>(a, s, cross);
    case 1: return launch_tf_res<1, kF32>(a, s, cross);
    default: return launch_tf_res<2, kF32>(a, s, cross);
  }
}

}
```

### moleculediffusiontransformer_amd/csrc/mdt_api.cpp

```cpp
#include <hip/hip_runtime.h>

#include <cstdio>
#include <cstdlib>
#include <cstring>
#include <string>
#include <vector>

#include "../../include/mdt_hip.h"
#include "mdt_kernels.h"

namespace {
thread_local std::string g_err;

int fail(const std::string& m) {
  g_err = m;
  return 1;
}

int hip_fail(const char* what, hipError_t e) {
  return fail(std::string(what) + ": " + hipGetErrorString(e));
}
}

__global__ void k_test_occupy(unsigned long long ticks) {
  extern __shared__ unsigned char hog_lds[];
  if (threadIdx.x == 0) hog_lds[0] = 1;
  const unsigned long long t0 = __builtin_amdgcn_s_memrealtime();
  while (__builtin_amdgcn_s_memrealtime() - t0 < ticks) __builtin_amdgcn_s_sleep(64);
}

struct mdt_program {
  std::vector<mdt_op> ops;
};

struct mdt_timer {
  std::vector<hipEvent_t> start, stop;
  int n = 0;
  bool open = false;
};

extern "C" {

static int g_pair_stride = 0;

__attribute__((visibility("hidden"))) void mdt_set_error(const char* msg) { g_err = msg ? msg : ""; }
static bool test_hooks_enabled() {
  const char* e = getenv("MDT_TEST_HOOKS");
  return e && e[0] == '1';
}
int mdt_set_tuning(const char* key, int32_t value) {
  const std::string k = key ? key : "";
  if (k == "pair_stride") { g_pair_stride = value; return 0; }
  if (k == "tile16") { mdt::set_tile16(value); return 0; }
  if (k == "w16") { mdt::set_w16(value); return 0; }
  if (k == "pair_capacity") {
    if (value > 0 && !test_hooks_enabled()) return fail("mdt_set_tuning(pair_capacity): a test hook, needs MDT_TEST_HOOKS=1");
    mdt::g_pair_capacity_override = value > 0 ? value : 0;
    return 0;
  }
  g_err = "mdt_set_tuning: unknown key '" + k + "'";
  return 1;
}
const char* mdt_last_error(void) { return g_err.c_str(); }
int32_t mdt_pair_capacity(void) { return mdt::tf256_pair_capacity(); }
int32_t mdt_tf256_block_core(int32_t T, int32_t Tk, int32_t cross) { return mdt::tf256_block_core(T, Tk, cross != 0) ? 1 : 0; }
int mdt_test_occupy(int32_t n_workgroups, int32_t lds_bytes, uint64_t ticks, void* stream) {
  if (!test_hooks_enabled()) return fail("mdt_test_occupy: a test hook, needs MDT_TEST_HOOKS=1 in the environment");
  if (n_workgroups <= 0 || n_workgroups > 4096 || lds_bytes < 0 || lds_bytes > 160 * 1024) return fail("mdt_test_occupy: bad arguments");
  if (ticks > 300000000ull) return fail("mdt_test_occupy: at most 3 s (3e8 ticks of the 100 MHz counter)");
  (void)hipFuncSetAttribute(reinterpret_cast<const void*>(&k_test_occupy), hipFuncAttributeMaxDynamicSharedMemorySize, 160 * 1024);
  hipLaunchKernelGGL(k_test_occupy, dim3((unsigned)n_workgroups), dim3(64), (size_t)lds_bytes, (hipStream_t)stream, (unsigned long long)ticks);
  const hipError_t e = hipGetLastError();
  return e == hipSuccess ? 0 : hip_fail("mdt_test_occupy", e);
}
#ifdef MDT_TUNING
int mdt_abi_version(void) { return MDT_ABI_VERSION | MDT_ABI_TUNING_BIT; }
#else
int mdt_abi_version(void) { return MDT_ABI_VERSION; }
#endif

static const char* validate(const mdt_op& o, int idx, char* buf, size_t nbuf) {
  auto bad = [&](const char* why) {
    snprintf(buf, nbuf, "op %d (kind %d): %s", idx, o.kind, why);
    return buf;
  };
  auto space_ok = [](const mdt_ref& r) { return r.space >= 0 && r.space < MDT_SP_EXT0 + MDT_N_EXT; };
  for (const mdt_ref* r : {&o.a, &o.a2, &o.w, &o.bias, &o.out, &o.res, &o.p0, &o.p1, &o.p2, &o.p3})
    if (!space_ok(*r) || r->off < 0) return bad("bad operand reference");
  if (o.film_bstride && (o.film_bstride < 0 || o.film_bstride % 4 || !o.p3.space ||
                         !(o.kind == MDT_OP_GN_ACT || o.kind == MDT_OP_RESBLOCK ||
                           (o.kind == MDT_OP_RCONV && !o.a2.space && o.i[MDT_R_GSIZE] > 0 && o.i[MDT_R_KSRC] <= 1 && !o.i[MDT_R_HALF_OUT] && o.i[MDT_R_NB] <= 1) ||
                           (o.kind == MDT_OP_GEMM && o.i[MDT_G_PRO] == MDT_PRO_GROUPNORM && o.i[MDT_G_WFMT] == 0 &&
                                                       o.i[MDT_G_M_MODE] == 0))))
    return bad("film_bstride: a FiLM batch stride (a positive multiple of 4 floats, with p3 bound) is taken by MDT_OP_GN_ACT, "
               "MDT_OP_RESBLOCK, a single-source MDT_OP_RCONV with its GroupNorm prologue and the GroupNorm prologue of an fp32 / split-bf16 "
               "MDT_OP_GEMM over the batch (WFMT 0, M_MODE 0) only");
  switch (o.kind) {
    case MDT_OP_GEMM: {
      const int32_t* i = o.i;
      if (i[MDT_G_CIN] <= 0 || i[MDT_G_CIN] % 16) return bad("cin must be a positive multiple of 16");
      if (i[MDT_G_N] <= 0 || i[MDT_G_TAPS] <= 0 || i[MDT_G_R_OUT] <= 0 || i[MDT_G_R_IN] <= 0) return bad("bad dims");
      if (i[MDT_G_LDA] % 4 || i[MDT_G_A_COL] % 4) return bad("A rows must be 16-byte aligned");
      if (i[MDT_G_LDA] < i[MDT_G_A_COL] + i[MDT_G_CIN]) return bad("lda < a_col + cin");
      if (!o.a.space || !o.w.space || !o.out.space) return bad("missing A / W / out");
      if (i[MDT_G_PRO] < 0 || i[MDT_G_PRO] > 3) return bad("bad prologue");
      if (i[MDT_G_PRO] == MDT_PRO_LAYERNORM) {
        if (i[MDT_G_TAPS] != 1) return bad("LayerNorm prologue needs taps == 1");
        if (i[MDT_G_CIN] > 2048) return bad("LayerNorm prologue supports <= 2048 features");
        if ((i[MDT_G_WFMT] == 16 || i[MDT_G_WFMT] == 17) ? (!o.p0.space != !o.p1.space) : (!o.p0.space || !o.p1.space))
          return bad("LayerNorm prologue needs gain and bias (ring-tile projection: both or neither -- neither = no affine)");
      }
      if (i[MDT_G_PRO] == MDT_PRO_GROUPNORM) {
        if (!o.p0.space || !o.p1.space || !o.p2.space) return bad("GroupNorm prologue needs gain, bias, stats");
        if (i[MDT_G_GROUPS] <= 0 || i[MDT_G_GSIZE] <= 0) return bad("bad groups");
      }
      if (i[MDT_G_M_MODE] < 0 || i[MDT_G_M_MODE] > 2) return bad("bad m_mode");
      if (o.res.space && i[MDT_G_LDR] <= 0) return bad("residual without ldr");
      if (o.a2.space && i[MDT_G_CIN] % 32) return bad("split-bf16 weights need cin % 32 == 0");
      if (i[MDT_G_WFMT] < 0 || (i[MDT_G_WFMT] > 2 && i[MDT_G_WFMT] != 6 && i[MDT_G_WFMT] != 10 && i[MDT_G_WFMT] != 16 && i[MDT_G_WFMT] != 17 &&
                                i[MDT_G_WFMT] != 38 && i[MDT_G_WFMT] != 134))
        return bad("bad weight format");
      if (i[MDT_G_WFMT] == 38 && !o.res.space) return bad("WFMT 38 (bf16 residual stream) needs the residual");
      if (i[MDT_G_WFMT] == 134) {
        if (!o.p0.space || o.res.space || i[MDT_G_TAPS] != 1 || i[MDT_G_T_OFF] || i[MDT_G_N] % 8 || i[MDT_G_LDC] % 8 || i[MDT_G_O_COL] % 8)
          return bad("WFMT 134 (folded LayerNorm): p0 = column sums of W, one tap, no residual, N / ldc / o_col % 8 == 0");
      }
      if (i[MDT_G_WFMT] == 16 || i[MDT_G_WFMT] == 17) {
        if (!mdt::proj_supported(i[MDT_G_CIN], i[MDT_G_N], i[MDT_G_LDA], i[MDT_G_LDC], o.res.space ? i[MDT_G_LDR] : 0) || o.a2.space)
          return bad("ring-tile projection needs cin in {128, 256}, N % 64 == 0, 16-byte aligned rows and no lo plane (the tiles hold both)");
        if (i[MDT_G_PRO] > 1 || i[MDT_G_TAPS] != 1 || i[MDT_G_T_STRIDE] != 1 || i[MDT_G_T_OFF] || i[MDT_G_PHASES] > 1 || i[MDT_G_O_STRIDE] != 1 ||
            i[MDT_G_O_OFF] || i[MDT_G_R_OUT] != i[MDT_G_R_IN] || i[MDT_G_O_ROWS] != i[MDT_G_R_OUT] || i[MDT_G_ACT] || i[MDT_G_O_COL] % 4 ||
            i[MDT_G_A_COL] % 4)
          return bad("ring-tile projection: LayerNorm or no prologue, one tap, no stride / phases / output row mapping / activation, "
                     "A_COL and O_COL multiples of 4 (16-byte row pieces)");
      }
      if (i[MDT_G_WFMT] == 10 && (!o.p0.space || i[MDT_G_O_COL] || i[MDT_G_N] % 2)) return bad("bf16 copy needs its tensor (p0) and whole rows");
      if (i[MDT_G_WFMT] & 2) {
        if (!mdt::gemm_b16_supported(i[MDT_G_CIN], i[MDT_G_TAPS], i[MDT_G_LDA], i[MDT_G_A_COL]) || o.a2.space)
          return bad("bf16 x bf16 GEMM needs cin % 64 == 0 and 16-byte aligned bf16 rows");
        if (i[MDT_G_N] % 4 || i[MDT_G_LDC] % 4 || i[MDT_G_O_COL] % 4 || (o.res.space && i[MDT_G_LDR] % 4))
          return bad("bf16 x bf16 GEMM: N, ldc, o_col and ldr must be multiples of 4 (float4 epilogue)");
        if (i[MDT_G_PRO] || i[MDT_G_T_STRIDE] != 1 || i[MDT_G_PHASES] > 1 || i[MDT_G_O_STRIDE] != 1 || i[MDT_G_O_OFF] ||
            i[MDT_G_R_OUT] != i[MDT_G_R_IN] || i[MDT_G_O_ROWS] != i[MDT_G_R_OUT] || i[MDT_G_M_MODE])
          return bad("bf16 x bf16 GEMM: no prologue / stride / phases / output row mapping (use MDT_OP_PREP16 + WFMT 1 forms)");
      }
      if (i[MDT_G_WFMT] == 1 && (i[MDT_G_CIN] % 32 || o.a2.space)) return bad("bf16 weights need cin % 32 == 0 and no lo plane");
      break;
    }
    case MDT_OP_PREP16: {
      const int32_t* i = o.i;
      if (i[MDT_G_CIN] <= 0 || i[MDT_G_CIN] % 8 || i[MDT_G_R_IN] <= 0) return bad("bad dims");
      if (i[MDT_G_LDA] % 4 || i[MDT_G_A_COL] % 4 || i[MDT_G_LDA] < i[MDT_G_A_COL] + i[MDT_G_CIN]) return bad("bad A rows");
      if (i[MDT_G_PRO] < 0 || i[MDT_G_PRO] > 3) return bad("bad prologue");
      if (i[MDT_G_WFMT] != 0 && (i[MDT_G_WFMT] != 2 || i[MDT_G_PRO] != MDT_PRO_LAYERNORM || i[MDT_G_CIN] > 1024 || i[MDT_G_LDA] % 8 || i[MDT_G_A_COL] % 8))
        return bad("PREP16 with a bf16 input (WFMT 2): LayerNorm of rows of at most 1024 channels, LDA / A_COL multiples of 8 elements");
      if (!o.a.space || !o.out.space) return bad("missing operand");
      if (i[MDT_G_PRO] == MDT_PRO_LAYERNORM && (!o.p0.space || !o.p1.space)) return bad("LayerNorm needs gain and bias");
      if (i[MDT_G_PRO] == MDT_PRO_GROUPNORM &&
          (!o.p0.space || !o.p1.space || !o.p2.space || !o.p3.space || i[MDT_G_GROUPS] <= 0 || i[MDT_G_GSIZE] <= 0))
        return bad("GroupNorm needs gain, bias, stats, FiLM vector and groups");
      break;
    }
// ... 241 lines not shown
          mdt::Gemm16Args h;
          h.A = reinterpret_cast<const unsigned short*>(g.A); h.W = reinterpret_cast<const unsigned short*>(g.W);
          h.bias = g.bias; h.res = g.res; h.out = g.out; h.M = g.M; h.N = g.N; h.cin = g.cin; h.taps = g.taps; h.rows = g.r_in;
          h.lda = g.lda; h.a_col = g.a_col; h.t_dj = g.t_dj; h.t_off = g.t_off; h.ldc = g.ldc; h.ldr = g.ldr; h.o_col = g.o_col;
          h.act = g.act; h.out16 = (i[MDT_G_WFMT] & 4) ? 1 : 0; h.res16 = (i[MDT_G_WFMT] & 32) ? 1 : 0;
          h.copy16 = (i[MDT_G_WFMT] & 8) ? reinterpret_cast<unsigned short*>(ptr(o.p0)) : nullptr;
          h.csum = (i[MDT_G_WFMT] & 128) ? ptr(o.p0) : nullptr;
          h.eps = g.eps;
          e = mdt::launch_gemm_b16(h, stream);
        } else if (!missing) {
          static const bool no_as = mdt_tuning_env("MDT_NO_AS") != nullptr;
          if (i[MDT_G_WFMT] == 1) e = mdt::launch_gemm_bf16(g, stream);
          else if (!g.W_lo) e = mdt::launch_gemm(g, stream);
          else if (!no_as && mdt::gemm_as_eligible(g)) e = mdt::launch_gemm_as(g, stream);
          else e = mdt::launch_gemm_bf16x3(g, stream);
        }
        break;
      }
      case MDT_OP_PREP16: {
        const int32_t* i = o.i;
        mdt::Prep16Args g;
        g.a = ptr(o.a); g.out = reinterpret_cast<unsigned short*>(ptr(o.out)); g.p0 = ptr(o.p0); g.p1 = ptr(o.p1);
        g.p2 = ptr(o.p2); g.p3 = ptr(o.p3); g.rows = i[MDT_G_R_IN]; g.total_rows = B * g.rows; g.lda = i[MDT_G_LDA];
        g.a_col = i[MDT_G_A_COL]; g.cin = i[MDT_G_CIN]; g.pro = i[MDT_G_PRO]; g.groups = i[MDT_G_GROUPS];
        g.gsize = i[MDT_G_GSIZE]; g.pro_silu = i[MDT_G_PRO_SILU]; g.eps = o.f[MDT_GF_EPS]; g.in16 = i[MDT_G_WFMT] == 2 ? 1 : 0;
        if (!missing) e = mdt::launch_prep16(g, stream);
        break;
      }
      case MDT_OP_GN_STATS: {
        mdt::GnStatsArgs g;
        g.x = ptr(o.a); g.stats = ptr(o.out); g.batch = B; g.rows = o.i[MDT_N_ROWS]; g.ld = o.i[MDT_N_LD];
        g.groups = o.i[MDT_N_GROUPS]; g.gsize = o.i[MDT_N_GSIZE]; g.eps = o.f[MDT_NF_EPS];
        if (!missing) e = mdt::launch_gn_stats(g, stream);
        break;
      }
      case MDT_OP_GN_ACT: {
        mdt::GnActArgs a;
        a.x = ptr(o.a); a.y = ptr(o.out); a.gamma = ptr(o.p0); a.beta = ptr(o.p1); a.film = ptr(o.p3); a.film_bs = o.film_bstride;
        a.batch = B; a.rows = o.i[MDT_N_ROWS]; a.ld = o.i[MDT_N_LD]; a.groups = o.i[MDT_N_GROUPS];
        a.gsize = o.i[MDT_N_GSIZE]; a.silu = o.i[MDT_N_SILU]; a.eps = o.f[MDT_NF_EPS]; a.out16 = o.i[MDT_N_OUT16];
        a.x2 = ptr(o.a2); a.ca = o.i[MDT_N_CA]; a.scale2 = o.f[MDT_NF_SCALE2]; a.raw16 = reinterpret_cast<unsigned short*>(ptr(o.p2));
        if (!missing) e = mdt::launch_gn_act(a, stream);
        break;
      }
      case MDT_OP_RCONV: {
        mdt::RConvArgs a;
        a.x = ptr(o.a); a.x2 = ptr(o.a2); a.w = ptr(o.w); a.bias = ptr(o.bias); a.res = ptr(o.res); a.out = ptr(o.out);
        a.gamma = ptr(o.p0); a.beta = ptr(o.p1); a.film = ptr(o.p3); a.film_bs = o.film_bstride; a.dbgbuf = ptr(o.p2);
        a.T = o.i[MDT_R_T]; a.M = B * a.T; a.C = o.i[MDT_R_C]; a.lda = o.i[MDT_R_LDA]; a.ldc = o.i[MDT_R_LDC];
        a.ldr = o.i[MDT_R_LDR]; a.taps = o.i[MDT_R_TAPS]; a.gsize = o.i[MDT_R_GSIZE]; a.silu = o.i[MDT_R_SILU];
        a.film_ld = o.i[MDT_R_FILM_LD]; a.eps = o.f[MDT_RF_EPS]; a.in_scale = o.f[MDT_RF_IN_SCALE];
        a.lda2 = o.i[MDT_R_LDA2]; a.in_scale2 = o.f[MDT_RF_IN_SCALE2];
        a.pf_ptr = pf_ptr; a.pf_lines = pf_lines; a.wf32 = o.i[MDT_R_WF32]; a.ksrc = o.i[MDT_R_KSRC]; a.half_out = o.i[MDT_R_HALF_OUT]; a.nb = o.i[MDT_R_NB];
        if (!missing) e = mdt::launch_rconv(a, stream);
        break;
      }
      case MDT_OP_RESBLOCK: {
        mdt::ResBlockArgs a;
        a.x = ptr(o.a); a.out = ptr(o.out); a.w = ptr(o.w); a.vec = ptr(o.bias); a.film = ptr(o.p3); a.film_bs = o.film_bstride;
        a.B = B; a.T = o.i[MDT_K_T]; a.cin = o.i[MDT_K_CIN]; a.cout = o.i[MDT_K_COUT]; a.film_ld = o.i[MDT_K_FILM_LD];
        a.eps = o.f[MDT_KF_EPS]; a.wf32 = o.i[MDT_K_WF32];
        a.cin_real = o.i[MDT_K_CIN_REAL] > 0 ? o.i[MDT_K_CIN_REAL] : a.cin;
        a.cout_real = o.i[MDT_K_COUT_REAL] > 0 ? o.i[MDT_K_COUT_REAL] : a.cout;
        a.patch_in = o.i[MDT_K_PATCH_IN]; a.patch_out = o.i[MDT_K_PATCH_OUT];
        if (!missing) e = mdt::launch_resblock(a, stream);
        break;
      }
      case MDT_OP_ATTN: {
        mdt::AttnArgs a;
        a.q = ptr(o.a); a.k = ptr(o.a2); a.out = ptr(o.out); a.batch = B; a.T = o.i[MDT_A_T]; a.Tk = o.i[MDT_A_TK];
        a.in16 = o.i[MDT_A_IN16]; a.split_scores = 0;
        if (a.q) a.q = reinterpret_cast<const float*>(reinterpret_cast<const char*>(a.q) + (size_t)o.i[MDT_A_QCOL] * ((a.in16 & 1) ? 2 : 4));
        if (a.k) a.k = reinterpret_cast<const float*>(reinterpret_cast<const char*>(a.k) + (size_t)o.i[MDT_A_KCOL] * ((a.in16 & 2) ? 2 : 4));
        a.heads = o.i[MDT_A_HEADS]; a.ldq = o.i[MDT_A_LDQ]; a.ldkv = o.i[MDT_A_LDKV]; a.ldo = o.i[MDT_A_LDO];
        a.kv_bstride = o.i[MDT_A_KV_BSTRIDE]; a.scale = o.f[MDT_AF_SCALE]; a.out16 = o.i[MDT_A_OUT16];
        if (!missing) e = mdt::launch_attn(a, stream);
        break;
      }
      case MDT_OP_ATTN_CTX: {
        mdt::AttnArgs a;
        a.q = ptr(o.a); a.k = ptr(o.a2); a.out = ptr(o.out); a.batch = B; a.T = o.i[MDT_A_T]; a.Tk = o.i[MDT_A_TK];
        a.heads = o.i[MDT_A_HEADS]; a.ldq = 128; a.ldkv = o.i[MDT_A_LDKV]; a.ldo = 128;
        a.kv_bstride = o.i[MDT_A_KV_BSTRIDE]; a.scale = o.f[MDT_AF_SCALE]; a.out16 = 0; a.split_scores = o.i[MDT_A_SPLIT]; a.in16 = 0;
        if (!missing) e = mdt::launch_attn_ctx(a, stream);
        break;
      }
      case MDT_OP_CONCAT: {
        float *a = ptr(o.a), *b2 = ptr(o.a2), *out = ptr(o.out);
        if (!missing)
          e = mdt::launch_concat(a, b2, out, (int64_t)B * o.i[MDT_C_ROWS], o.i[MDT_C_CA], o.i[MDT_C_CB],
                                 o.f[MDT_CF_SCALE_B], stream);
        break;
      }
      case MDT_OP_PATCH: {
        float *in = ptr(o.a), *out = ptr(o.out);
        if (!missing)
          e = mdt::launch_patch(in, out, B, o.i[MDT_P_ROWS_IN], o.i[MDT_P_C_IN], o.i[MDT_P_LD_IN], o.i[MDT_P_LD_OUT],
                                o.i[MDT_P_PATCH], o.i[MDT_P_INVERSE], stream);
        break;
      }
      case MDT_OP_TBLOCK: {
        mdt::TBlockArgs a;
        a.x = ptr(o.a); a.w = ptr(o.w); a.bias = ptr(o.bias); a.kv = ptr(o.a2); a.dbgbuf = ptr(o.p0);
        a.mode = o.i[MDT_B_MODE]; a.C = o.i[MDT_B_C]; a.T = o.i[MDT_B_T]; a.M = B * a.T;
        a.nchunk = o.i[MDT_B_NCHUNK]; a.nbias = o.i[MDT_B_NBIAS]; a.ldx = a.C; a.Tk = o.i[MDT_B_TK];
        a.kv_bstride = o.i[MDT_B_KV_BSTRIDE]; a.ldkv = o.i[MDT_B_LDKV]; a.nheads = o.i[MDT_B_HEADS]; a.nsamples = B;
        a.eps = o.f[MDT_BF_EPS]; a.scale = o.f[MDT_BF_SCALE];
        a.part = nullptr; a.nsplit = 1; a.xout = nullptr; a.pin = nullptr; a.pout = nullptr;
        a.pf_ptr = pf_ptr; a.pf_lines = pf_lines;
        a.kv2 = o.i[MDT_B_KV2] ? ptr(o.p1) : nullptr;
        if (o.i[MDT_B_KV2]) {
          const int per_wg = (o.i[MDT_B_VARIANT] >= 2 ? 32 : 64) / a.T;
          if (!o.p1.space || B % 2 || (B / 2) % (per_wg > 0 ? per_wg : 1))
            return fail("mdt_program_run: a dual-batch cross block needs the shared K/V rows and B = 2 x (a multiple of the samples per workgroup)");
        }
        a.post = o.i[MDT_B_POST]; a.wf32 = o.i[MDT_B_WF32];
        if (a.post) a.xout = ptr(o.out);
        if (o.i[MDT_B_VARIANT] == 3) { a.part = ptr(o.out); a.nsplit = 2; }
        if (o.i[MDT_B_VARIANT] == 4) {
          a.xout = ptr(o.out); a.pin = ptr(o.res); a.pout = ptr(o.p2);
          a.nsplit = o.p2.space ? 2 : 1;
        }
        if (!missing)
          e = o.i[MDT_B_VARIANT] >= 2 ? mdt::launch_tblock32(a, stream) : mdt::launch_tblock_lw(a, stream);
        break;
      }
      case MDT_OP_TF128:
      case MDT_OP_TF256: {
        const int32_t* i = o.i;
        const bool wide = o.kind == MDT_OP_TF256;
        mdt::TFArgs a;
        a.x = ptr(o.a); a.out = ptr(o.out); a.w = ptr(o.w); a.vec = ptr(o.bias);
        a.tiles = reinterpret_cast<const unsigned*>(ptr(o.p0));
        a.kv = i[MDT_F_CROSS] ? ptr(o.a2) : nullptr;
        a.kv2 = i[MDT_F_KV2] ? ptr(o.p1) : nullptr;
        a.dbgbuf = nullptr;
        a.T = i[MDT_F_T]; a.M = B * a.T; a.NT = i[MDT_F_NT]; a.nvec = i[MDT_F_NVEC]; a.Tk = i[MDT_F_TK];
        a.kv_bstride = i[MDT_F_KV_BSTRIDE]; a.ldkv = i[MDT_F_LDKV]; a.nheads = i[MDT_F_HEADS]; a.nsamples = B;
        a.has_in = i[MDT_F_HAS_IN]; a.nblocks = i[MDT_F_NBLOCKS]; a.nff = i[MDT_F_NFF]; a.npost = i[MDT_F_NPOST];
        a.kv_lstride = (int64_t)i[MDT_F_KV_LSTRIDE] * (o.a2.space == MDT_SP_ACT ? B : 1);
        a.kv2_lstride = (int64_t)i[MDT_F_KV_LSTRIDE] * (o.p1.space == MDT_SP_ACT ? B : 1);
        a.eps_ln = o.f[MDT_FF_EPS_LN]; a.scale = o.f[MDT_FF_SCALE]; a.eps_gn = o.f[MDT_FF_EPS_GN];
        a.res_kind = wide ? 0 : i[MDT_F_RES_KIND]; a.n_res = wide ? 0 : i[MDT_F_N_RES];
        a.res_pair1 = i[MDT_F_RES_PAIR1]; a.res_pair2 = i[MDT_F_RES_PAIR2]; a.nfilm = wide ? 0 : i[MDT_F_NFILM];
        a.film = a.n_res ? ptr(o.p3) : nullptr; a.skip = a.n_res ? ptr(o.res) : nullptr;
        a.skip_stride = (int64_t)B * a.T * i[MDT_F_C] * (a.res_kind == 2 ? -1 : 1);
        a.skip_scale = o.f[MDT_FF_SKIP_SCALE]; a.eps_res = o.f[MDT_FF_EPS_RES];
        a.pf_ptr = pf_ptr; a.pf_lines = pf_lines;
        a.nsplit = wide && i[MDT_F_NSPLIT] == 2 ? 2 : 1;
        a.pair_stride = g_pair_stride > 0 ? g_pair_stride : (i[MDT_F_PAIR_STRIDE] > 0 ? i[MDT_F_PAIR_STRIDE] : 8);
        a.xflags = a.nsplit == 2 ? reinterpret_cast<unsigned*>(const_cast<float*>(ptr(o.p2))) : nullptr;
        a.xbuf = a.nsplit == 2 ? const_cast<float*>(ptr(o.p3)) : nullptr;
        a.wf32 = i[MDT_F_WF32]; a.rb_base = 0;
        if (i[MDT_F_KV2]) {
          const int per_wg = (wide ? 32 : 64) / a.T;
          if (!o.p1.space || B % 2 || (B / 2) % (per_wg > 0 ? per_wg : 1))
            return fail("mdt_program_run: a dual-batch fused transformer needs the shared K/V rows and B = 2 x (a multiple of the samples per workgroup)");
        }
        if (!missing) e = wide ? mdt::launch_tf256(a, stream) : mdt::launch_tf128(a, stream);
        break;
      }
      case MDT_OP_RES256: {
        const int32_t* i = o.i;
        mdt::TFArgs a = {};
        a.x = ptr(o.a); a.out = ptr(o.out); a.w = ptr(o.w); a.vec = ptr(o.bias);
        a.tiles = reinterpret_cast<const unsigned*>(ptr(o.p0));
        a.T = i[MDT_F_T]; a.M = B * a.T; a.NT = i[MDT_F_NT]; a.nvec = i[MDT_F_NVEC]; a.nsamples = B;
        a.nheads = i[MDT_F_HEADS];
        a.npost = i[MDT_F_NPOST];
        a.res_kind = i[MDT_F_RES_KIND]; a.n_res = i[MDT_F_N_RES]; a.nfilm = i[MDT_F_NFILM];
        a.film = ptr(o.p3); a.skip = ptr(o.res);
        a.skip_stride = (int64_t)B * a.T * 256 * (a.res_kind == 2 ? -1 : 1);
        a.skip_scale = o.f[MDT_FF_SKIP_SCALE]; a.eps_res = o.f[MDT_FF_EPS_RES];
        a.pf_ptr = pf_ptr; a.pf_lines = pf_lines;
        a.nsplit = i[MDT_F_NSPLIT] == 2 ? 2 : 1; a.wf32 = i[MDT_F_WF32];
        a.pair_stride = g_pair_stride > 0 ? g_pair_stride : (i[MDT_F_PAIR_STRIDE] > 0 ? i[MDT_F_PAIR_STRIDE] : 8);
        a.xflags = a.nsplit == 2 ? reinterpret_cast<unsigned*>(const_cast<float*>(ptr(o.a2))) : nullptr;
        a.xbuf = a.nsplit == 2 ? const_cast<float*>(ptr(o.p1)) : nullptr;
        a.nff = i[MDT_F_NFF]; a.rb_base = 0;
        a.dbgbuf = ptr(o.p2);
        if (!missing) e = mdt::launch_res256(a, stream);
        break;
      }
      case MDT_OP_TIME_EMBED: {
        float *cn = ptr(o.a), *w = ptr(o.w), *out = ptr(o.out);
        if (!missing) e = mdt::launch_time_embed(cn, w, out, n_shared_rows, o.i[MDT_T_HALF], o.i[MDT_T_LD], stream);
        break;
      }
      default:
        return fail("mdt_program_run: unknown op kind");
    }
    if (missing) {
      char buf[128];
      snprintf(buf, sizeof buf, "mdt_program_run: op %d references an unbound buffer", idx);
      return fail(buf);
    }
    if (e != hipSuccess) {
      char buf[128];
      snprintf(buf, sizeof buf, "mdt_program_run: op %d (kind %d) launch failed", idx, o.kind);
      return hip_fail(buf, e);
    }
  }
  return 0;
}

mdt_timer* mdt_timer_create(int32_t max_intervals) {
  if (max_intervals <= 0) {
    fail("mdt_timer_create: max_intervals must be positive");
    return nullptr;
  }
  mdt_timer* t = new mdt_timer();
  t->start.resize(max_intervals);
  t->stop.resize(max_intervals);
  for (int i = 0; i < max_intervals; ++i) {
    if (hipEventCreate(&t->start[i]) != hipSuccess || hipEventCreate(&t->stop[i]) != hipSuccess) {
      fail("mdt_timer_create: hipEventCreate failed");
      delete t;
      return nullptr;
    }
  }
  return t;
}

void mdt_timer_destroy(mdt_timer* t) {
  if (!t) return;
  for (auto e : t->start) (void)hipEventDestroy(e);
  for (auto e : t->stop) (void)hipEventDestroy(e);
  delete t;
}

int mdt_timer_start(mdt_timer* t, void* stream) {
  if (!t || t->open || t->n >= (int)t->start.size()) return fail("mdt_timer_start: timer full or interval open");
  hipError_t e = hipEventRecord(t->start[t->n], (hipStream_t)stream);
  if (e != hipSuccess) return hip_fail("mdt_timer_start", e);
  t->open = true;
  return 0;
}

int mdt_timer_stop(mdt_timer* t, void* stream) {
  if (!t || !t->open) return fail("mdt_timer_stop: no open interval");
  hipError_t e = hipEventRecord(t->stop[t->n], (hipStream_t)stream);
  if (e != hipSuccess) return hip_fail("mdt_timer_stop", e);
  t->open = false;
  t->n++;
  return 0;
}

int32_t mdt_timer_collect(mdt_timer* t, float* ms, int32_t cap) {
  if (!t || t->open) {
    fail("mdt_timer_collect: interval still open");
    return -1;
  }
  const int n = t->n < cap ? t->n : cap;
  for (int i = 0; i < n; ++i) {
    hipError_t e = hipEventSynchronize(t->stop[i]);
    if (e == hipSuccess) e = hipEventElapsedTime(&ms[i], t->start[i], t->stop[i]);
    if (e != hipSuccess) {
      hip_fail("mdt_timer_collect", e);
      return -1;
    }
  }
  t->n = 0;
  return n;
}

}
```

### moleculediffusiontransformer_amd/csrc/mdt_kernels.h

```cpp
#pragma once
#include <hip/hip_runtime.h>
#include <stdint.h>

#if (defined(MDT_ABL_BAR) || defined(MDT_ABL_VMWAIT) || defined(MDT_ABL_LGKM) || defined(MDT_ABL_LDSBC) || defined(MDT_ABL_GELU) ||     \
     defined(MDT_ABL_ATTN) || defined(MDT_ABL_ATTNX) || defined(MDT_RING_NODRAIN) || defined(MDT_STAGGER) || defined(MDT_XH_D2) ||                               \
     (defined(MDT_XH_ADDR) && MDT_XH_ADDR == 0) || (defined(MDT_XH_MODE) && MDT_XH_MODE != 0)) &&                                       \
    !defined(MDT_TUNING)
#error "MDT_ABL_* / MDT_RING_NODRAIN / MDT_STAGGER / MDT_XH_D2 / MDT_XH_ADDR=0 / MDT_XH_MODE!=0 give wrong results: timing builds only, add -DMDT_TUNING"
#endif
#define MDT_ABI_TUNING_BIT 0x40000000

#include <cstdlib>
static inline const char* mdt_tuning_env(const char* name) {
#ifdef MDT_TUNING
  return getenv(name);
#else
  (void)name;
  return nullptr;
#endif
}

#include <cstdio>
extern "C" __attribute__((visibility("hidden"))) void mdt_set_error(const char* msg);
static inline int mdt_bad(const char* msg) {
  mdt_set_error(msg);
  return 2;
}
static inline int mdt_bad(const char* name, const char* msg) {
  char buf[256];
  snprintf(buf, sizeof buf, "%s%s", name, msg);
  return mdt_bad(buf);
}
static inline int mdt_finish(const char* who) {
  hipError_t e = hipGetLastError();
  if (e == hipSuccess) return 0;
  char buf[256];
  snprintf(buf, sizeof buf, "%s: %s", who, hipGetErrorString(e));
  mdt_set_error(buf);
  return 1;
}

#ifndef MDT_LOADER_PRIO
#define MDT_LOADER_PRIO 3
#endif

namespace mdt {

struct GemmArgs {
  const float* A;
  const float* W;
  const float* W_lo;
  const float* bias;
  float* out;
  const float* res;
  const float* p0;
  const float* p1;
  const float* p2;
  const float* p3;
  int film_bs = 0;
  int M, r_out, r_in, lda, cin, taps, t_stride, t_dj, t_off;
  int N, ldc, o_rows, o_stride, o_off, ldr;
  int pro, groups, gsize, pro_silu, act, a_col, o_col;
  int wfmt;
  int phases;
  float eps;
};
#ifdef __HIPCC__
__device__ __forceinline__ void gemm_select_phase(GemmArgs& g) {
  if (g.phases > 1) {
    const int ph = blockIdx.z, f = g.phases;
    const int shift = ph < f / 2 ? 1 : 0;
    const long wo = (long)ph * g.N * (g.taps * g.cin) / ((g.W_lo || g.wfmt == 1) ? 2 : 1);
    g.W += wo;
    if (g.W_lo) g.W_lo += wo;
    g.t_off = shift;
    g.o_off = f * shift + ph - f / 2;
  }
}
#endif
hipError_t launch_gemm(const GemmArgs& g, hipStream_t s);
hipError_t launch_gemm_bf16x3(const GemmArgs& g, hipStream_t s);
hipError_t launch_gemm_bf16(const GemmArgs& g, hipStream_t s);

struct Gemm16Args {
  const unsigned short* A;
  const unsigned short* W;
  const float* bias;
  const float* res;
  float* out;
  int M, N, cin, taps, rows;
  int lda, a_col;
  int t_dj, t_off, ldc, ldr, o_col, act;
  int out16;
  int res16;
  unsigned short* copy16;
  const float* csum;
  float eps;
};
bool gemm_b16_supported(int cin, int taps, int lda, int a_col);
bool gemm_b16_epilogue_ok(const Gemm16Args& g);
hipError_t launch_gemm_b16(const Gemm16Args& g, hipStream_t s);
void set_tile16(int v);
void set_w16(int v);
struct Prep16Args {
  const float* a;
  unsigned short* out;
  const float* p0; const float* p1; const float* p2; const float* p3;
  int total_rows, rows, lda, a_col, cin, pro, groups, gsize, pro_silu;
  float eps;
  int in16;
};
hipError_t launch_prep16(const Prep16Args& g, hipStream_t s);
bool gemm_as_eligible(const GemmArgs& g);
hipError_t launch_gemm_as(const GemmArgs& g, hipStream_t s);

struct DevOnce {
  unsigned long long mask = 0;
  bool first() {
    int d = 0;
    if (hipGetDevice(&d) != hipSuccess || d < 0 || d >= 64) return true;
    if ((mask >> d) & 1ull) return false;
    mask |= 1ull << d;
    return true;
  }
};

#ifdef __HIPCC__
__device__ __forceinline__ void prefetch_next_weights(const void* p, int lines, int lane256) {
  if (!p) return;
  const int nwg = gridDim.x * gridDim.y, id = blockIdx.x + blockIdx.y * gridDim.x;
  const int nx = (nwg + 7) >> 3, xw = id >> 3;
  const int per = (lines + nx - 1) / nx;
  const int lo = xw * per, hi = lo + per < lines ? lo + per : lines;
  const unsigned char* b = reinterpret_cast<const unsigned char*>(p);
  unsigned acc = 0;
  for (int l = lo + lane256; l < hi; l += 256) acc |= *reinterpret_cast<const volatile unsigned*>(b + (int64_t)l * 128);
  asm volatile("" :: "v"(acc));
}
#endif

struct GnStatsArgs {
  const float* x;
  float* stats;
  int batch, rows, ld, groups, gsize;
  float eps;
};
hipError_t launch_gn_stats(const GnStatsArgs& g, hipStream_t s);

struct GnActArgs {
  const float* x;
  float* y;
  const float* gamma;
  const float* beta;
  const float* film;
  int film_bs = 0;
  int batch, rows, ld, groups, gsize, silu;
  float eps;
  int out16;
  const float* x2;
  int ca;
  float scale2;
  unsigned short* raw16;
};
bool gn_act_eligible(int rows, int ld, int groups, int gsize);
hipError_t launch_gn_act(const GnActArgs& a, hipStream_t s);

struct RConvArgs {
  const float* x;
  const float* x2;
  const float* w;
  const float* bias;
  const float* res;
  float* out;
  const float* gamma;
  const float* beta;
  const float* film;
  int film_bs = 0;
  const float* dbgbuf;
  int M, T, C, lda, lda2, ldc, ldr, taps, gsize, silu, film_ld;
  float eps, in_scale, in_scale2;
  const void* pf_ptr;
  int pf_lines;
  int wf32;
  int ksrc;
  int half_out;
  int nb;
};
struct ProjArgs {
  const float* x;
  const float* w;
  const float* bias;
  const float* res;
  const float* gamma;
  const float* beta;
  float* out;
  int M, N, K, lda, ldc, ldr, ln;
  float eps;
  int nch;
  int wf32;
};
bool proj_supported(int K, int N, int lda, int ldc, int ldr);
hipError_t launch_proj(const ProjArgs& a, hipStream_t s);

bool rconv_supported(int C, int T, int taps, int gsize);
hipError_t launch_rconv(const RConvArgs& a, hipStream_t s);
hipError_t launch_rconv_f32(const RConvArgs& a, hipStream_t s);

struct ResBlockArgs {
  const float* x;
  float* out;
  const float* w;
  const float* vec;
  const float* film;
  int film_bs = 0;
  int B, T, cin, cout, film_ld;
  float eps;
  int wf32;
  int cin_real, cout_real;
  int patch_in, patch_out;
};
bool resblock_supported(int T, int cin, int cout);
hipError_t launch_resblock(const ResBlockArgs& a, hipStream_t s);

struct AttnArgs {
  const float* q;
  const float* k;
  float* out;
  int batch, T, Tk, heads, ldq, ldkv, ldo, kv_bstride;
  float scale;
  int out16;
  int split_scores;
  int in16;
};
hipError_t launch_attn(const AttnArgs& a, hipStream_t s);
hipError_t launch_attn_ctx(const AttnArgs& a, hipStream_t s);

struct TBlockArgs {
  float* x;
  const float* w;
  const float* bias;
  const float* kv;
  const float* kv2;
  const float* dbgbuf;
  float* part;
  int nsplit;
  float* xout;
  const float* pin;
  float* pout;
  int post;
  int wf32;
  int mode, C, M, T, nchunk, nbias, ldx, Tk, kv_bstride, ldkv, nheads, nsamples;
  float eps, scale;
  const void* pf_ptr;
  int pf_lines;
};
bool tblock_lw_supported(const TBlockArgs& a);
hipError_t launch_tblock_lw(const TBlockArgs& a, hipStream_t s);
hipError_t launch_tblock32(const TBlockArgs& a, hipStream_t s);

struct TFArgs {
  const float* x;
  float* out;
  const float* w;
  const float* vec;
  const unsigned* tiles;
  const float* kv;
  const float* kv2;
  const float* dbgbuf;
  int64_t kv_lstride, kv2_lstride;
  int M, T, NT, nvec, Tk, kv_bstride, ldkv, nheads, nsamples;
  int has_in;
  int nblocks;
  int nff;
  int npost;
  float eps_ln, eps_gn, scale;
  int res_kind;
  int n_res, res_pair1, res_pair2;
  int nfilm;
  const float* film;
  float* skip;
  int64_t skip_stride;
  float skip_scale, eps_res;
  const void* pf_ptr;
  int pf_lines;
  int nsplit;
  int pair_stride;
  float* xbuf;
  unsigned* xflags;
  int wf32;
  int rb_base;
};
bool tf128_supported(int T, int Tk, int nvec, bool cross);
hipError_t launch_tf128(const TFArgs& a, hipStream_t s);
hipError_t launch_tf128_f32(const TFArgs& a, hipStream_t s);
bool tf256_supported(int T, int Tk, int nheads, int nff, bool cross);
bool tf256_block_core(int T, int Tk, bool cross);
hipError_t launch_tf256(const TFArgs& a, hipStream_t s);
hipError_t launch_tf256_f32(const TFArgs& a, hipStream_t s);
bool res256_supported(int T, int kind, int n_res, int taps);
hipError_t launch_res256(const TFArgs& a, hipStream_t s);
int tf256_pair_capacity();
extern int g_pair_capacity_override;

hipError_t launch_concat(const float* a, const float* b, float* out, int64_t rows, int ca, int cb, float scale_b,
                         hipStream_t s);
hipError_t launch_patch(const float* in, float* out, int batch, int rows_in, int c_in, int ld_in, int ld_out,
                        int patch, int inverse, hipStream_t s);
hipError_t launch_time_embed(const float* cn, const float* w, float* out, int rows, int half, int ld,
                             hipStream_t s);


#if defined(__HIPCC__)
template <int BM, int BN>
__device__ __forceinline__ void store_tile_coalesced(const float* Cs, const GemmArgs& g, int m0, int n0) {
  constexpr int C4 = BN / 4, LDC = BN + 4, U = 4;
  typedef float f4 __attribute__((ext_vector_type(4)));
  for (int base = threadIdx.x; base < BM * C4; base += 256 * U) {
    float4 v[U], b[U], r[U];
    int64_t oidx[U], ridx[U];
    int ncol[U];
    bool ok[U];
#pragma unroll
    for (int u = 0; u < U; ++u) {
      const int idx = base + 256 * u;
      const int row = idx / C4, c4 = idx - row * C4;
      const int m = m0 + row, n = n0 + c4 * 4;
      ok[u] = idx < BM * C4 && m < g.M && n < g.N;
      const int mm = ok[u] ? m : m0, nn = ok[u] ? n : n0;
      const int bb = mm / g.r_out;
      const int64_t orow = (int64_t)bb * g.o_rows + (int64_t)(mm - bb * g.r_out) * g.o_stride + g.o_off;
      oidx[u] = orow * g.ldc + g.o_col + nn;
      ridx[u] = orow * g.ldr + nn;
      ncol[u] = nn;
      v[u] = ok[u] ? *reinterpret_cast<const float4*>(Cs + row * LDC + c4 * 4) : make_float4(0.f, 0.f, 0.f, 0.f);
    }
    if (g.bias) {
#pragma unroll
      for (int u = 0; u < U; ++u) b[u] = *reinterpret_cast<const float4*>(g.bias + ncol[u]);
    }
    if (g.res) {
#pragma unroll
      for (int u = 0; u < U; ++u) r[u] = *reinterpret_cast<const float4*>(g.res + ridx[u]);
    }
#pragma unroll
    for (int u = 0; u < U; ++u) {
      float4 w = v[u];
      if (g.bias) { w.x += b[u].x; w.y += b[u].y; w.z += b[u].z; w.w += b[u].w; }
      if (g.act == 1) {
        w.x = 0.5f * w.x * (1.0f + erff(w.x * 0.70710678118654752440f));
        w.y = 0.5f * w.y * (1.0f + erff(w.y * 0.70710678118654752440f));
        w.z = 0.5f * w.z * (1.0f + erff(w.z * 0.70710678118654752440f));
        w.w = 0.5f * w.w * (1.0f + erff(w.w * 0.70710678118654752440f));
      }
      if (g.res) { w.x += r[u].x; w.y += r[u].y; w.z += r[u].z; w.w += r[u].w; }
      if (ok[u]) __builtin_nontemporal_store(f4{w.x, w.y, w.z, w.w}, reinterpret_cast<f4*>(g.out + oidx[u]));
    }
  }
}
#endif

}
```

### moleculediffusiontransformer_amd/engine.py

```python
from __future__ import annotations

import ctypes as C
import os
from typing import Dict, Optional

import torch

from . import runtime as rt
from .compiler import EXT_CTX, EXT_FILM, EXT_OUT, EXT_XBUF, EXT_XFLAGS, EXT_XIN, CompiledUNet


def _require_gpu(device: torch.device) -> None:
    if device.type != "cuda" or not torch.cuda.is_available():
        raise RuntimeError(
            "moleculediffusiontransformer_amd runs its sampling path only on an AMD GPU through libmdt_hip.so; "
            f"device '{device}' is not a HIP device (there is no CPU fallback by design)")


class UNetEngine:

    def __init__(self, compiled: CompiledUNet, device, use_graph: Optional[bool] = None):
        device = torch.device(device)
        _require_gpu(device)
        rt.load_library()
        self.c = compiled
        self.device = device
        with torch.cuda.device(device):
            self.weights = compiled.weights.to(device)
            self.shr = torch.zeros(compiled.shr_floats, device=device)
            try:
                self.programs: Dict[str, rt.Program] = {k: rt.Program(v) for k, v in compiled.programs.items()}
            except RuntimeError as e:
                if "mdt_program_create" not in str(e):
                    raise
                raise RuntimeError(
                    f"U-Net configuration outside the envelope of the MI355X kernels (max_length={compiled.length}, "
                    f"channels={compiled.cfg.channels}, patch_size={compiled.cfg.patch_size}): {e}.  Supported: at most 8192 "
                    "tokens per sample on an attention level, head_features 64, channels a multiple of 16 -- see DESIGN.md "
                    "section 8") from e
            tile = compiled.length * (compiled.in_pad + 1) * 4
            if tile > 160 * 1024:
                raise RuntimeError(f"max_length={compiled.length} with {compiled.in_pad} (padded) channels needs a {tile}-byte "
                                   "sampler tile; the preconditioning / update kernels stage one sample in the 160 KiB of LDS of a "
                                   "compute unit (max_length * (pred_dim_padded + 1) * 4 <= 163840) -- see DESIGN.md section 8")
        if use_graph is None:
            use_graph = os.environ.get("MDT_GRAPH", "1") != "0"
        self.use_graph = use_graph
        self.B = 0
        self.act = None
        self.xin = None
        self.pred = None
        self.pred_fixed = None
        self.xflags = self.xbuf = None
        self.film = None
        self._graphs: Dict[str, torch.cuda.CUDAGraph] = {}
        self._time_rows = 0
        self._fixed_ready = False

    def reserve(self, B: int) -> None:
        if B == self.B:
            return
        c = self.c
        self._graphs.clear()
        self.act = self.xin = self.pred = self.pred_fixed = None
        self.act = torch.empty(c.act_floats * B, device=self.device)
        self.xin = torch.zeros(B, c.length, c.in_pad, device=self.device)
        self.pred = torch.zeros(B, c.length, c.in_pad, device=self.device)
        self.pred_fixed = torch.zeros(B, c.length, c.in_pad, device=self.device)
        self.xflags = self.xbuf = None
        self.film = torch.empty(B, c.ss_total, device=self.device) if c.rows else None
        if c.xchg_tokens:
            nrb = (B * c.xchg_tokens + 31) // 32
            self.xflags = torch.zeros(64 + 64 * nrb + (8 * 4096 + 16384 if os.environ.get("MDT_XH_LOG") else 0), dtype=torch.int32,
                                      device=self.device)
            self.xbuf = torch.empty(2 * nrb * 2 * 32 * 256, device=self.device)
        self.B = B

    def _bind(self, xin=None, ctx=None, out=None) -> rt.MdtBindings:
        b = rt.MdtBindings()
        b.weights, b.act, b.shr = rt.ptr(self.weights), rt.ptr(self.act), rt.ptr(self.shr)
        b.ext[EXT_XIN], b.ext[EXT_CTX], b.ext[EXT_OUT] = rt.ptr(xin), rt.ptr(ctx), rt.ptr(out)
        b.ext[EXT_XFLAGS], b.ext[EXT_XBUF] = rt.ptr(getattr(self, "xflags", None)), rt.ptr(getattr(self, "xbuf", None))
        b.ext[EXT_FILM] = rt.ptr(getattr(self, "film", None))
        return b

    sync_handoff_check = True

    def note_handoff(self) -> None:
        if getattr(self, "xflags", None) is None:
            return
        if getattr(self, "_xstat_host", None) is None:
            self._xstat_host = torch.zeros(1, dtype=torch.int32).pin_memory()
            self._xstat_event = torch.cuda.Event()
        if torch.cuda.is_current_stream_capturing():
            self._xstat_captured = True
            return
        self._xstat_host.copy_(self.xflags[:1], non_blocking=True)
        self._xstat_event.record()
        self._xstat_pending = True
        if self.sync_handoff_check:
            self.handoff_check(wait=True)

    def handoff_check(self, wait: bool = False) -> None:
        if not getattr(self, "_xstat_pending", False):
            if getattr(self, "_xstat_captured", False) and wait and getattr(self, "xflags", None) is not None \
                    and not torch.cuda.is_current_stream_capturing():
                self._xstat_host.copy_(self.xflags[:1], non_blocking=True)
                self._xstat_event.record()
                self._xstat_pending = True
            else:
                return
        if wait:
            self._xstat_event.synchronize()
        if not self._xstat_event.query():
            return
        self._xstat_pending = False
        if int(self._xstat_host[0]) != 0:
            if getattr(self, "xflags", None) is not None:
                self.xflags[0] = 0
            when = "this" if wait else "the PREVIOUS"
            if getattr(self, "_xstat_captured", False):
                when = "this call OR of a replay of a graph that captured evaluations of this engine since the last check; every such"
            raise RuntimeError(f"a pair hand-off inside a 256-channel transformer launch timed out (a partner workgroup was not "
                               f"scheduled within 0.3 s): the results of {when} call are invalid.  The pair-split launches need "
                               "their workgroups resident at the same time (compute units taken by another stream or process?); "
                               "set model.kernel_choice = 'wide' or MDT_TF256_PAIR=0 for forms without in-launch hand-offs")

    def handoff_status(self) -> int:
        if getattr(self, "xflags", None) is None:
            return 0
        return int(self.xflags[0].item())

    def prepare_times(self, c_noise: torch.Tensor) -> None:
        n = c_noise.numel()
        if self.c.rows:
            raise RuntimeError("this engine holds the per-row programs (one time value per sample): use prepare_time_rows / eval_rows")
        if n > self.c.max_time_rows:
            raise ValueError(f"{n} U-Net evaluations per call (timesteps = {n // 2 + 1}) exceed the time table of "
                             f"{self.c.max_time_rows} rows this engine was compiled with (at most "
                             f"{self.c.max_time_rows // 2 + 1} timesteps); compile_unet(max_time_rows=...) sets it")
        off = self.c.shr["c_noise"]
        self.shr[off: off + n].copy_(c_noise.to(device=self.device, dtype=torch.float32), non_blocking=True)
        self.programs["time"].run(self._bind(), max(self.B, 1), n)
        self._time_rows = n

    def select_time(self, row: int) -> None:
        assert 0 <= row < self._time_rows
        c = self.c
        src = c.shr["ss_all"] + row * c.ss_total
        dst = c.shr["ss_cur"]
        base = self.shr.data_ptr()
        rt.check(rt.load_library().mdt_copy_f32(base + 4 * dst, base + 4 * src, c.ss_total, rt.current_stream()))

    def prepare_time_rows(self, c_noise_rows: torch.Tensor) -> None:
        if not self.c.rows:
            raise RuntimeError("this engine holds the shared-row programs: compile_unet(rows=True) builds the per-row form")
        if c_noise_rows.numel() != self.B:
            raise ValueError(f"{c_noise_rows.numel()} time values for a reserved batch of {self.B}: the per-row form takes one per sample")
        off = self.c.act_named["c_noise"] * self.B
        self.act[off: off + self.B].copy_(c_noise_rows.to(device=self.device, dtype=torch.float32).flatten(), non_blocking=True)
        self.programs["time_rows"].run(self._bind(), self.B, self.B)

    def prepare_context(self, embedding: torch.Tensor) -> None:
        B = embedding.shape[0]
        self.reserve(B)
        emb = embedding.to(device=self.device, dtype=torch.float32).contiguous()
        assert emb.shape[1] == self.c.cond_len and emb.shape[2] == self.c.cfg.ctx_features, emb.shape
        self.programs["ctx"].run(self._bind(ctx=emb), B)

    def prepare_fixed(self) -> None:
        if not self._fixed_ready:
            self.programs["ctx_fixed"].run(self._bind(), max(self.B, 1))
            self._fixed_ready = True

    @property
    def has_dual(self) -> bool:
        return "eval_dual" in self.programs

    def eval(self, fixed: bool = False, dual: bool = False) -> torch.Tensor:
        name = "eval_dual" if dual else ("eval_fixed" if fixed else "eval")
        out = self.pred_fixed if fixed else self.pred
        if fixed or dual:
            self.prepare_fixed()
        if dual and (self.B % 2 or (self.B // 2) % self.c.dual_multiple):
            raise ValueError(f"the dual guidance batch needs 2 x (a multiple of {self.c.dual_multiple}) samples: a cross-attention "
                             "workgroup must not straddle the conditional and the unconditional half")
        return self._run_eval(name, out)

    def eval_rows(self, fixed: bool = False) -> torch.Tensor:
        if fixed:
            self.prepare_fixed()
        return self._run_eval("eval_rows_fixed" if fixed else "eval_rows", self.pred_fixed if fixed else self.pred)

    def _run_eval(self, name: str, out: torch.Tensor) -> torch.Tensor:
        if not self.use_graph:
            self.programs[name].run(self._bind(xin=self.xin, out=out), self.B)
            return out
        g = self._graphs.get(name)
        if g is None:
            self.programs[name].run(self._bind(xin=self.xin, out=out), self.B)
            torch.cuda.synchronize(self.device)
            g = torch.cuda.CUDAGraph()
            with torch.cuda.graph(g, capture_error_mode="thread_local"):
                self.programs[name].run(self._bind(xin=self.xin, out=out), self.B)
            self._graphs[name] = g
        g.replay()
        return out
```

### moleculediffusiontransformer_amd/runtime.py

```python
from __future__ import annotations

import ctypes as C
import os
from typing import Optional

from . import build as _build

N_EXT = 8
ABI_VERSION = 5
ABI_TUNING_BIT = 0x40000000
SP_NONE, SP_WEIGHT, SP_ACT, SP_SHR, SP_EXT0 = 0, 1, 2, 3, 4
OP_GEMM, OP_GN_STATS, OP_ATTN, OP_CONCAT, OP_PATCH, OP_TIME_EMBED, OP_TBLOCK, OP_GN_ACT, OP_RCONV = 1, 2, 3, 4, 5, 6, 7, 8, 9
OP_RESBLOCK = 10
OP_TF128 = 11
OP_TF256 = 12
OP_RES256 = 15
OP_ATTN_CTX = 13
OP_PREP16 = 14
W_KB = 23
OP_NAMES = {OP_GEMM: "k_gemm", OP_GN_STATS: "k_gn_stats", OP_ATTN: "k_attn", OP_CONCAT: "k_concat", OP_PATCH: "k_patch",
            OP_TIME_EMBED: "k_time_embed", OP_TBLOCK: "k_tblock", OP_GN_ACT: "k_gn_act", OP_RCONV: "k_rconv",
            OP_RESBLOCK: "k_resblock", OP_TF128: "k_tf128", OP_TF256: "k_tf256", OP_RES256: "k_res256", OP_ATTN_CTX: "k_attn_ctx", OP_PREP16: "k_prep16"}
TB_SELF, TB_CROSS, TB_FF = 0, 1, 2
PRO_NONE, PRO_LAYERNORM, PRO_GROUPNORM, PRO_SILU = 0, 1, 2, 3

G_R_OUT, G_R_IN, G_LDA, G_CIN, G_TAPS, G_T_STRIDE, G_T_DJ, G_T_OFF, G_N, G_LDC, G_O_ROWS, G_O_STRIDE, \
    G_O_OFF, G_LDR, G_PRO, G_GROUPS, G_GSIZE, G_PRO_SILU, G_ACT, G_M_MODE, G_A_COL, G_O_COL, G_PHASES, G_WFMT = range(24)
N_ROWS, N_LD, N_GROUPS, N_GSIZE, N_SILU, N_OUT16, N_CA = range(7)
A_T, A_TK, A_HEADS, A_LDQ, A_LDKV, A_LDO, A_KV_BSTRIDE, A_OUT16, A_QCOL, A_KCOL, A_SPLIT, A_IN16 = range(12)
C_ROWS, C_CA, C_CB = range(3)
P_ROWS_IN, P_C_IN, P_LD_IN, P_LD_OUT, P_PATCH, P_INVERSE = range(6)
T_HALF, T_LD = range(2)
R_T, R_C, R_LDA, R_LDC, R_LDR, R_TAPS, R_GSIZE, R_SILU, R_FILM_LD, R_LDA2, R_WF32, R_KSRC, R_HALF_OUT, R_NB = range(14)
K_T, K_CIN, K_COUT, K_FILM_LD, K_WF32, K_CIN_REAL, K_COUT_REAL, K_PATCH_IN, K_PATCH_OUT = range(9)
B_MODE, B_C, B_T, B_NCHUNK, B_NBIAS, B_TK, B_KV_BSTRIDE, B_LDKV, B_HEADS, B_VARIANT, B_POST = range(11)
B_KV2, B_WF32 = 11, 12
(F_C, F_T, F_NT, F_NVEC, F_TK, F_KV_BSTRIDE, F_LDKV, F_HEADS, F_HAS_IN, F_NBLOCKS, F_NFF, F_NPOST, F_KV2, F_CROSS,
 F_KV_LSTRIDE, F_RES_KIND, F_N_RES, F_RES_PAIR1, F_RES_PAIR2, F_NFILM, F_NSPLIT, F_PAIR_STRIDE, F_WF32) = range(23)
FF_EPS_LN, FF_SCALE, FF_EPS_GN, FF_EPS_RES, FF_SKIP_SCALE = range(5)
SCREEN_EMPTY, SCREEN_NONFINITE, SCREEN_DUPLICATE, SCREEN_KNOWN = 1, 2, 4, 8
SCREEN_CLOSE = 16
SCREEN_MALFORMED, SCREEN_OVERVALENT = 32, 64
SMILES_MAX_LENGTH = 128
MAX_KEY_CANDIDATES = 1024
MOL_MAX_LENGTH = 64
FP_BITS, FP_WORDS, FP_SIM_DEN, FP_MAX_RADIUS = 1024, 16, 65536, 3
SCREEN_SUBSTRUCTURE = 128
SUB_MAX_PATTERNS, SUB_MAX_WIDTH, SUB_MAX_STEPS = 32, 32, 4096
MOLH_MAX_STEPS, MOLH_FORMULA = 4096, 13
MOLH_OK, MOLH_AROMATIC_OVERVALENT, MOLH_NO_KEKULE, MOLH_UNDECIDED = 0, 1, 2, 3
MOLR_DESC = 16
MOLN_NORMALIZED, MOLN_AROMATIC, MOLN_CHANGED = 1, 2, 4
FP_KNOWN_CHUNK = 512
EDIT_KNOWN_CHUNK = 512
EDIT_MAX_LENGTH = EDIT_MAX_ID = 64


class MdtRef(C.Structure):
    _fields_ = [("space", C.c_int32), ("reserved", C.c_int32), ("off", C.c_int64)]


class MdtOp(C.Structure):
    _fields_ = [("kind", C.c_int32), ("film_bstride", C.c_int32),
                ("a", MdtRef), ("a2", MdtRef), ("w", MdtRef), ("bias", MdtRef), ("out", MdtRef),
                ("res", MdtRef), ("p0", MdtRef), ("p1", MdtRef), ("p2", MdtRef), ("p3", MdtRef),
                ("i", C.c_int32 * 24), ("f", C.c_float * 8)]


class MdtBindings(C.Structure):
    _fields_ = [("weights", C.c_void_p), ("act", C.c_void_p), ("shr", C.c_void_p),
                ("ext", C.c_void_p * N_EXT)]


_F, _P, _I, _L, _U64, _U32 = C.c_float, C.c_void_p, C.c_int32, C.c_int64, C.c_uint64, C.c_uint32
SYMBOLS = {
    "mdt_abi_version": (_I, []),
    "mdt_last_error": (C.c_char_p, []),
    "mdt_set_tuning": (_I, [C.c_char_p, _I]),
    "mdt_pair_capacity": (_I, []),
    "mdt_tf256_block_core": (_I, [_I, _I, _I]),
    "mdt_test_occupy": (_I, [_I, _I, _U64, _P]),
    "mdt_program_create": (_P, [C.POINTER(MdtOp), _I]),
    "mdt_program_destroy": (None, [_P]),
    "mdt_program_num_ops": (_I, [_P]),
    "mdt_program_run": (_I, [_P, C.POINTER(MdtBindings), _I, _I, _I, _I, _P]),
    "mdt_cond_embed": (_I, [_P, _P, _P, _P, _P, _I, _I, _I, _I, _P]),
    "mdt_cond_embed_add": (_I, [_P, _P, _P, _P, _P, _I, _I, _I, _I, _P]),
    "mdt_precond_in": (_I, [_P, _P, _F, _I, _I, _I, _I, _P]),
    "mdt_precond_out": (_I, [_P, _P, _P, _F, _F, _I, _I, _I, _I, _P, _P]),
    "mdt_dyn_scale": (_I, [_P, _P, _P, _F, _F, _F, _I, _I, _I, _I, _P]),
    "mdt_noise_in_rows": (_I, [_P, _P, _P, _P, _P, _P, _U64, _U32, _L, _I, _I, _I, _I, _P]),
    "mdt_precond_in_rows": (_I, [_P, _P, _P, _I, _I, _I, _I, _P]),
    "mdt_precond_out_rows": (_I, [_P, _P, _P, _P, _P, _I, _I, _I, _I, _P, _P]),
    "mdt_dyn_scale_rows": (_I, [_P, _P, _P, _P, _P, _F, _I, _I, _I, _I, _P]),
    "mdt_loss_rows": (_I, [_P, _P, _P, _P, _P, _P, _P, _P, _I, _I, _I, _I, _P]),
    "mdt_cfg_mix": (_I, [_P, _P, _P, _F, _L, _P]),
    "mdt_cfg_mix_rows": (_I, [_P, _P, _P, _P, _I, _L, _P]),
    "mdt_adpm2_mid": (_I, [_P, _P, _P, _P, _F, _F, _F, _F, _F, _I, _I, _I, _I, _P, _P]),
    "mdt_adpm2_next": (_I, [_P, _P, _P, _P, _P, _F, _F, _F, _F, _F, _F, _U64, _U32, _L, _I, _I, _I, _I, _P, _P, _P]),
    "mdt_adpm2_euler": (_I, [_P, _P, _P, _P, _P, _F, _F, _F, _I, _U64, _U32, _L, _I, _I, _I, _P]),
    "mdt_aeuler_next": (_I, [_P, _P, _P, _P, _F, _F, _F, _F, _F, _F, _U64, _U32, _L, _I, _I, _I, _I, _P, _P, _P]),
    "mdt_karras_hat": (_I, [_P, _P, _P, _P, _F, _F, _F, _U64, _U32, _L, _I, _I, _I, _I, _P]),
    "mdt_karras_mid": (_I, [_P, _P, _P, _P, _P, _F, _F, _F, _F, _F, _I, _I, _I, _I, _P, _P, _P]),
    "mdt_karras_next": (_I, [_P, _P, _P, _P, _P, _F, _F, _F, _F, _I, _I, _I, _I, _P, _P, _P]),
    "mdt_init_noise": (_I, [_P, _P, _F, _U64, _U32, _L, _I, _I, _I, _P]),
    "mdt_clamp": (_I, [_P, _F, _F, _L, _P]),
    "mdt_copy_f32": (_I, [_P, _P, _L, _P]),
    "mdt_inpaint_merge": (_I, [_P, _P, _P, _P, _F, _U64, _U32, _L, _I, _I, _I, _P]),
    "mdt_add_noise": (_I, [_P, _P, _F, _U64, _U32, _L, _I, _I, _I, _P]),
    "mdt_inpaint_enter": (_I, [_P, _P, _P, _P, _P, _I, _P, _P, _F, _F, _F, _U64, _U32, _U32, _L, _I, _I, _I, _I, _P]),
    "mdt_inpaint_finish": (_I, [_P, _P, _P, _P, _I, _P, _I, _I, _I, _P]),
    "mdt_refine_enter": (_I, [_P, _P, _P, _I, _P, _P, _P, _F, _F, _U64, _U32, _L, _I, _I, _I, _I, _P]),
    "mdt_refine_keep_enter": (_I, [_P, _P, _P, _I, _P, _P, _P, _I, _P, _P, _F, _F, _U64, _U32, _U32, _L, _I, _I, _I, _I, _P]),
    "mdt_argmax_tokens": (_I, [_P, _P, _I, _I, _I, _P]),
    "mdt_tokens_compact": (_I, [_P, _I, _I, _P, _I, C.c_double, _P, _P, _P, _P]),
    "mdt_screen_score": (_I, [_P, _L, _P, _P, _I, _I, _I, _P, _P]),
    "mdt_screen_select": (_I, [_P, _P, _P, _P, _I, _I, _I, _P, _P, _P, _I, _I, _P, _P, _P, _P]),
    "mdt_screen_select_diverse": (_I, [_P, _P, _P, _P, _I, _I, _I, _P, _P, _P, _I, _I, _P, _I, _I, _P, _P, _P, _P]),
    "mdt_screen_select_reject": (_I, [_P, _P, _P, _P, _I, _I, _I, _P, _P, _P, _I, _I, _P, _P, _P, _P, _P]),
    "mdt_screen_select_diverse_reject": (_I, [_P, _P, _P, _P, _I, _I, _I, _P, _P, _P, _I, _I, _P, _I, _I, _P, _P, _P, _P, _P]),
    "mdt_smiles_check": (_I, [_P, _P, _I, _I, _P, _P, _P, _P, _P, _P]),
    "mdt_mol_graph": (_I, [_P, _P, _I, _I, _P, _P, _P, _P, _P, _P, _P, _P, _P, _P]),
    "mdt_mol_key": (_I, [_P, _P, _P, _P, _I, _I, _P, _P]),
    "mdt_key_flags": (_I, [_P, _I, _I, _P, _I, _P, _P]),
    "mdt_mol_fp": (_I, [_P, _P, _P, _P, _I, _I, _I, _P, _P, _P]),
    "mdt_fp_tanimoto_rows": (_I, [_P, _P, _I, _P, _P, _P]),
    "mdt_fp_nearest": (_I, [_P, _I, _P, _I, _P, _P, _P, _P, _P]),
    "mdt_screen_select_similar": (_I, [_P, _P, _P, _P, _I, _I, _I, _P, _P, _P, _I, _I, _P, _I, _I, _P, _P, _P, _I, _P, _P, _P, _P]),
    "mdt_sub_match": (_I, [_P, _P, _P, _P, _I, _I, _P, _P, _P, _P, _I, _I, _U32, _U32, _P, _P, _P, _P]),
    "mdt_mol_hydrogens": (_I, [_P, _P, _P, _P, _I, _I, _I, _P, _P, _P, _P, _P, _P]),
    "mdt_mol_rings": (_I, [_P, _P, _P, _P, _P, _I, _I, _P, _P, _P, _P, _P, _P, _P]),
    "mdt_mol_normalize": (_I, [_P, _P, _P, _P, _P, _P, _P, _P, _I, _I, _P, _P, _P, _P]),
    "mdt_edit_distance_rows": (_I, [_P, _P, _P, _P, _I, _I, _P, _P]),
    "mdt_edit_nearest": (_I, [_P, _P, _I, _I, _P, _P, _I, _P, _P, _P, _P]),
    "mdt_timer_create": (_P, [_I]),
    "mdt_timer_destroy": (None, [_P]),
    "mdt_timer_start": (_I, [_P, _P]),
    "mdt_timer_stop": (_I, [_P, _P]),
    "mdt_timer_collect": (_I, [_P, C.POINTER(C.c_float), _I]),
}

_lib: Optional[C.CDLL] = None


def load_library(allow_build: bool = True) -> C.CDLL:
    global _lib
    if _lib is not None:
        return _lib
    path = _build.library_path()
    allow_build = allow_build and os.environ.get("MDT_NO_BUILD", "0") != "1"
    if allow_build and not _build.is_fresh():
        try:
            _build.build_library()
        except Exception as e:
            if not os.path.exists(path) or os.environ.get("MDT_ALLOW_STALE", "0") != "1":
                raise RuntimeError(f"libmdt_hip.so is missing or older than its sources and could not be rebuilt: {e} "
                                   "(set MDT_ALLOW_STALE=1 to load the stale library anyway)") from e
            import warnings
            warnings.warn(f"libmdt_hip.so is STALE (sources changed, rebuild failed: {e}); loading it because MDT_ALLOW_STALE=1")
    if not os.path.exists(path):
        raise RuntimeError("libmdt_hip.so not found; run `python -c 'import __graft_entry__ as g; g.build()'`")
    lib = C.CDLL(path)
    for name, (res, args) in SYMBOLS.items():
        fn = getattr(lib, name)
        fn.restype = res
        fn.argtypes = args
    abi = lib.mdt_abi_version()
    if abi & ABI_TUNING_BIT:
        if os.environ.get("MDT_ALLOW_TUNING", "0") != "1":
            raise RuntimeError(f"{path} is a TUNING build (-DMDT_TUNING: timing-only switches that give wrong results may be "
                               "compiled in); it is refused for sampling.  Tools that time such builds set MDT_ALLOW_TUNING=1")
        abi &= ~ABI_TUNING_BIT
    if abi != ABI_VERSION:
        raise RuntimeError(f"libmdt_hip.so ABI version {lib.mdt_abi_version()} != {ABI_VERSION} expected by this package: rebuild it")
    _lib = lib
    return lib


def pair_capacity() -> int:
    n = int(load_library().mdt_pair_capacity())
    if n <= 0:
        raise RuntimeError("libmdt_hip: the device's co-residency capacity for pair-split launches could not be determined")
    return n


def check(rc: int) -> None:
    if rc != 0:
        raise RuntimeError("libmdt_hip: " + load_library().mdt_last_error().decode())


def ptr(t) -> int:
    return 0 if t is None else t.data_ptr()


def current_stream() -> int:
    import torch
    return torch.cuda.current_stream().cuda_stream


class Program:

    def __init__(self, ops):
        lib = load_library()
        arr = (MdtOp * len(ops))(*ops)
        self._h = lib.mdt_program_create(arr, len(ops))
        if not self._h:
            raise RuntimeError("libmdt_hip: " + lib.mdt_last_error().decode())
        self.n_ops = len(ops)

    def run(self, bindings: MdtBindings, B: int, n_shared_rows: int = 0, first: int = 0, count: int = -1,
            stream: Optional[int] = None) -> None:
        lib = load_library()
        check(lib.mdt_program_run(self._h, C.byref(bindings), B, n_shared_rows, first, count,
                                  current_stream() if stream is None else stream))

    def __del__(self):
        try:
            if getattr(self, "_h", None) and _lib is not None:
                _lib.mdt_program_destroy(self._h)
        except Exception:
            pass


class EventTimer:

    def __init__(self, max_intervals: int):
        self._lib = load_library()
        self._h = self._lib.mdt_timer_create(max_intervals)
        if not self._h:
            raise RuntimeError("libmdt_hip: " + self._lib.mdt_last_error().decode())
        self.cap = max_intervals

    def start(self, stream=None):
        check(self._lib.mdt_timer_start(self._h, current_stream() if stream is None else stream))

    def stop(self, stream=None):
        check(self._lib.mdt_timer_stop(self._h, current_stream() if stream is None else stream))

    def collect(self):
        buf = (C.c_float * self.cap)()
        n = self._lib.mdt_timer_collect(self._h, buf, self.cap)
        if n < 0:
            raise RuntimeError("libmdt_hip: " + self._lib.mdt_last_error().decode())
        return [buf[i] for i in range(n)]

    def __del__(self):
        try:
            if getattr(self, "_h", None):
                self._lib.mdt_timer_destroy(self._h)
        except Exception:
            pass
```

Baseline: 4756 molecules/s.

## Pre-pack cross-attention K/V into split-bf16 MFMA-ready table once per context

Adds a kernel that, after the context program runs, converts each cross-attention layer's fp32 K/V rows into a pre-split hi/lo bf16 table laid out in the MFMA fragment order. The tf128 fused transformer kernel then streams these packed tiles straight into LDS and loads K and V fragments directly, instead of reloading fp32 K/V and splitting them on every one of the 126 U-Net evaluations. This removes repeated conversion work and halves the bytes fetched per K/V tile, at the cost of an extra buffer, a one-time pack per context, and a more involved tile loader and wait schedule.

Result: no change. 4773 molecules/s (median of 3 runs) (+0.4%).

```diff
diff --git a/include/mdt_hip.h b/include/mdt_hip.h
--- a/include/mdt_hip.h
+++ b/include/mdt_hip.h
@@ -241,6 +241,9 @@
 int mdt_init_noise(float *x, const float *noise, float sigma0, uint64_t seed, uint32_t step,
                    int64_t sample0, int32_t B, int32_t C, int32_t L, void *stream);
 int mdt_copy_f32(float *dst, const float *src, int64_t n, void *stream);
+int64_t mdt_kv_pack_bytes(int32_t n_layers, int32_t B, int32_t T, int32_t Tk, int32_t nheads, int32_t fixed);
+int mdt_kv_pack(const float *kv, void *table, int32_t n_layers, int64_t kv_lstride, int32_t B, int32_t T, int32_t Tk, int32_t ldkv,
+                int32_t nheads, int32_t kv_bstride, void *stream);
 int mdt_clamp(float *x, float lo, float hi, int64_t n, void *stream);
 int mdt_inpaint_merge(float *x, const float *src, const uint8_t *mask, const float *noise, float sigma,
                       uint64_t seed, uint32_t step, int64_t sample0, int32_t B, int32_t C, int32_t L,
diff --git a/moleculediffusiontransformer_amd/build.py b/moleculediffusiontransformer_amd/build.py
--- a/moleculediffusiontransformer_amd/build.py
+++ b/moleculediffusiontransformer_amd/build.py
@@ -31,6 +31,7 @@
     ("k_norm.hip", []),
     ("k_attn.hip", []),
     ("k_elem.hip", ["-ffp-contract=off"]),
+    ("k_kvpack.hip", []),
     ("k_screen.hip", ["-ffp-contract=off"]),
     ("k_edit.hip", []),
     ("k_smiles.hip", []),
diff --git a/moleculediffusiontransformer_amd/compiler.py b/moleculediffusiontransformer_amd/compiler.py
--- a/moleculediffusiontransformer_amd/compiler.py
+++ b/moleculediffusiontransformer_amd/compiler.py
@@ -12,6 +12,7 @@
 EXT_XIN, EXT_CTX, EXT_OUT = 0, 1, 2
 EXT_XFLAGS, EXT_XBUF = 3, 4
 EXT_FILM = 5
+EXT_KVP, EXT_KVP_FIXED = 6, 7
 
 
 def pad16(c: int) -> int:
@@ -118,6 +119,7 @@
     xchg_tokens: int = 0
     rows: bool = False
     act_named: Dict[str, int] = field(default_factory=dict)
+    kv_pack: Optional[Dict[str, object]] = None
 
 
 class UNetCompiler:
@@ -144,6 +146,7 @@
         self.fold_ctx = os.environ.get("MDT_FOLD_CTX", "1") == "1"
         self.has_chat = False
         self.tf128 = os.environ.get("MDT_TF128", "1") == "1"
+        self.kv_pack = os.environ.get("MDT_KV_PACK", "1") == "1"
         self.tf256 = bool(tf256)
         self.tf256_pair = os.environ.get("MDT_TF256_PAIR", "1") == "1"
         self.pair_stride = int(os.environ.get("MDT_PAIR_STRIDE", "8"))
@@ -1772,6 +1775,23 @@
         self.kv_fixed = [kvf + i * self.n_ctx * mid2 for i in range(n_cross)]
         chat_fixed = self._shr_alloc("chat_fixed", self.n_ctx * cfg.ctx_features)
 
+        kv_pack = None
+        packed_of: Dict[int, int] = {}
+        if self.kv_pack:
+            n_packed = 0
+            for op in eval_ops:
+                if op.kind == rt.OP_TF128 and isinstance(getattr(op, "_kv", None), tuple) and not op.i[rt.F_WF32] and op.i[rt.F_NBLOCKS] > 0:
+                    if kv_pack is None:
+                        kv_pack = dict(T=op.i[rt.F_T], Tk=op.i[rt.F_TK], heads=op.i[rt.F_HEADS], ldkv=op.i[rt.F_LDKV],
+                                       lstride=op.i[rt.F_KV_LSTRIDE], runs=[])
+                    if op.i[rt.F_T] != kv_pack["T"]:
+                        continue
+                    packed_of[id(op)] = n_packed
+                    kv_pack["runs"].append((op._kv[1], op.i[rt.F_NBLOCKS], n_packed))
+                    n_packed += op.i[rt.F_NBLOCKS]
+            if kv_pack is not None:
+                kv_pack.update(layers=n_packed, kv=self.kv_slots[0], kv_fixed=self.kv_fixed[0])
+
         def resolve(ops, fixed: bool):
             out = []
             for op in ops:
@@ -1804,6 +1824,8 @@
                         o.i[slot] = 0
                     else:
                         o.a2 = _ref(rt.SP_ACT, self.kv_slots[idx])
+                    if id(op) in packed_of:
+                        o.p2 = _ref(rt.SP_EXT0 + EXT_KVP, packed_of[id(op)])
                 out.append(o)
             return out
 
@@ -1905,7 +1927,7 @@
                             max_time_rows=rows, shr=dict(self.shr), ss_total=self.ss_total, n_cross=n_cross,
                             flops_per_sample_eval=flops_eval, flops_ctx_per_sample=flops_ctx, gemm_mode=self.gemm_mode,
                             weight_index=dict(self.W.index), dual_multiple=dual_multiple, tf256=self.tf256,
-                            xchg_tokens=self.xchg_tokens, rows=self.rows, act_named=act_named)
+                            xchg_tokens=self.xchg_tokens, rows=self.rows, act_named=act_named, kv_pack=kv_pack)
 
 
 def C_memmove(dst: rt.MdtOp, src: rt.MdtOp) -> None:
diff --git a/moleculediffusiontransformer_amd/csrc/k_kvpack.hip b/moleculediffusiontransformer_amd/csrc/k_kvpack.hip
--- /dev/null
+++ b/moleculediffusiontransformer_amd/csrc/k_kvpack.hip
@@ -0,0 +1,85 @@
+#include "mdt_hip.h"
+#include "mdt_kernels.h"
+#include "mdt_device.h"
+#include "mdt_kv_pack.h"
+
+namespace mdt {
+
+namespace {
+
+struct KvPackArgs {
+  const float* kv;
+  unsigned char* table;
+  int64_t kv_lstride;
+  int B, T, Tk, ldkv, nheads, kv_bstride, groups;
+};
+
+__global__ __launch_bounds__(256) void k_kv_pack(KvPackArgs a) {
+  const int nk = kvp::live_slots(a.T, a.Tk), nkp = kvp::padded_slots(a.T, a.Tk);
+  const int group = blockIdx.x, head = blockIdx.y, layer = blockIdx.z;
+  const int mid = 64 * a.nheads;
+  const float* src = a.kv + (int64_t)layer * a.kv_lstride + 64 * head;
+  unsigned char* chunk = a.table + ((int64_t)(layer * a.nheads + head) * a.groups + group) * kvp::chunk_bytes(nkp);
+  const int pb = kvp::plane_bytes(nkp);
+  auto row_of = [&](int ks) -> const float* {
+    const int live = kvp::slot_live(nk, ks);
+    const int sample = min(group * (16 / a.T) + live / a.Tk, a.B - 1);
+    return src + ((int64_t)sample * a.kv_bstride + live % a.Tk) * a.ldkv;
+  };
+  const int nK = 8 * nkp, nV = 16 * nkp;
+  for (int n = threadIdx.x; n < nK + nV; n += blockDim.x) {
+    if (n < nK) {
+      const int g = n & 3, ks = (n >> 2) % nkp, sp = (n >> 2) / nkp;
+      const float* p = row_of(ks) + 32 * sp + 4 * g;
+      const float4 v0 = *reinterpret_cast<const float4*>(p), v1 = *reinterpret_cast<const float4*>(p + 16);
+      uint4 hi, lo;
+      split2(v0.x, v0.y, hi.x, lo.x);
+      split2(v0.z, v0.w, hi.y, lo.y);
+      split2(v1.x, v1.y, hi.z, lo.z);
+      split2(v1.z, v1.w, hi.w, lo.w);
+      *reinterpret_cast<uint4*>(chunk + n * 16) = hi;
+      *reinterpret_cast<uint4*>(chunk + pb + n * 16) = lo;
+    } else {
+      const int m = n - nK;
+      const int kg = m % (nkp / 4), i = (m / (nkp / 4)) & 15, dt = m / (4 * nkp);
+      float v[4];
+#pragma unroll
+      for (int r = 0; r < 4; ++r) v[r] = row_of(4 * kg + r)[mid + 16 * dt + i];
+      uint2 hi, lo;
+      split2(v[0], v[1], hi.x, lo.x);
+      split2(v[2], v[3], hi.y, lo.y);
+      *reinterpret_cast<uint2*>(chunk + 2 * pb + m * 8) = hi;
+      *reinterpret_cast<uint2*>(chunk + 3 * pb + m * 8) = lo;
+    }
+  }
+}
+
+}
+
+}
+
+extern "C" {
+
+int64_t mdt_kv_pack_bytes(int32_t n_layers, int32_t B, int32_t T, int32_t Tk, int32_t nheads, int32_t fixed) {
+  if (n_layers <= 0 || B <= 0 || T <= 0 || 16 % T || Tk <= 0 || mdt::kvp::live_slots(T, Tk) > 16 || nheads <= 0) return 0;
+  const long long groups = fixed ? mdt::kvp::FIXED_GROUPS : mdt::kvp::groups_of(B, T);
+  return (int64_t)n_layers * mdt::kvp::layer_bytes(groups, nheads, mdt::kvp::padded_slots(T, Tk));
+}
+
+int mdt_kv_pack(const float* kv, void* table, int32_t n_layers, int64_t kv_lstride, int32_t B, int32_t T, int32_t Tk, int32_t ldkv,
+                int32_t nheads, int32_t kv_bstride, void* stream) {
+  if (!kv || !table) return mdt_bad("mdt_kv_pack: null pointer");
+  if (n_layers <= 0 || n_layers > 65535 || B <= 0 || T <= 0 || 16 % T || Tk <= 0 || mdt::kvp::live_slots(T, Tk) > 16)
+    return mdt_bad("mdt_kv_pack: tokens per sample must divide 16, at most 16 context rows per 16 tokens, 1..65535 layers");
+  if (nheads <= 0 || nheads > 16 || ldkv < 128 * nheads || ldkv % 4 || kv_bstride < 0 || kv_lstride % 4 ||
+      (reinterpret_cast<size_t>(kv) & 15) || (reinterpret_cast<size_t>(table) & 15))
+    return mdt_bad("mdt_kv_pack: 1..16 heads of 64 features, K | V rows of at least 128 heads floats, 16-byte aligned");
+  mdt::KvPackArgs a;
+  a.kv = kv; a.table = static_cast<unsigned char*>(table); a.kv_lstride = kv_lstride;
+  a.B = kv_bstride ? B : 1; a.T = T; a.Tk = Tk; a.ldkv = ldkv; a.nheads = nheads; a.kv_bstride = kv_bstride;
+  a.groups = (int)(kv_bstride ? mdt::kvp::groups_of(B, T) : mdt::kvp::FIXED_GROUPS);
+  hipLaunchKernelGGL(mdt::k_kv_pack, dim3((unsigned)a.groups, (unsigned)nheads, (unsigned)n_layers), dim3(256), 0, (hipStream_t)stream, a);
+  return mdt_finish("mdt_kv_pack");
+}
+
+}
diff --git a/moleculediffusiontransformer_amd/csrc/k_tf128.hip b/moleculediffusiontransformer_amd/csrc/k_tf128.hip
--- a/moleculediffusiontransformer_amd/csrc/k_tf128.hip
+++ b/moleculediffusiontransformer_amd/csrc/k_tf128.hip
@@ -3,6 +3,7 @@
 
 #include "mdt_kernels.h"
 #include "mdt_device.h"
+#include "mdt_kv_pack.h"
 
 #ifndef MDT_TF_F32
 #define MDT_TF_F32 0
@@ -12,9 +13,19 @@
 #define MDT_KV_CPOL 2
 #endif
 
+#if defined(MDT_KVP_ONE_TURN) && !defined(MDT_TUNING)
+#error "MDT_KVP_ONE_TURN is an A/B variant nobody tests: timing builds only, add -DMDT_TUNING"
+#endif
+
 namespace mdt {
 
 namespace {
+
+#ifdef MDT_KVP_ONE_TURN
+constexpr bool KVP_TWO = false;
+#else
+constexpr bool KVP_TWO = true;
+#endif
 
 enum { K_T = 0, K_N = 1, K_O = 2 };
 
@@ -49,6 +60,21 @@
   }
   return s;
 }
+__device__ __forceinline__ f32x4 scores_packed(const bf16x8* kh, const bf16x8* kl, const f32x4* qf) {
+  f32x4 s = {0.f, 0.f, 0.f, 0.f};
+#pragma unroll
+  for (int sp = 0; sp < 2; ++sp) {
+    float qv[8];
+#pragma unroll
+    for (int e = 0; e < 8; ++e) qv[e] = qf[2 * sp + (e >> 2)][e & 3];
+    bf16x8 qh, ql;
+    split8<false>(qv, qh, ql);
+    s = MDT_MFMA_BF16(kl[sp], qh, s, 0, 0, 0);
+    s = MDT_MFMA_BF16(kh[sp], ql, s, 0, 0, 0);
+    s = MDT_MFMA_BF16(kh[sp], qh, s, 0, 0, 0);
+  }
+  return s;
+}
 __device__ __forceinline__ void split_v(const f32x4* vT, bf16x4* vh, bf16x4* vl) {
 #pragma unroll
   for (int dt = 0; dt < 4; ++dt) {
@@ -70,8 +96,11 @@
 
 }
 
-template <int NPW, int RES, bool F32>
+template <int NPW, int RES, bool F32, bool PK>
 __global__ __launch_bounds__(512) void k_tf128(TFArgs a) {
+  static_assert(!PK || (NPW > 0 && !F32), "the packed table holds split-bf16 operands of a cross segment");
+  constexpr int NKP = 4 * NPW;
+  constexpr int CH = kvp::chunk_bytes(NKP), PB = kvp::plane_bytes(NKP);
   extern __shared__ __attribute__((aligned(1024))) unsigned char smem[];
 
   const int tid = threadIdx.x, lane = tid & 63;
@@ -100,7 +129,7 @@
     const int sample0 = blockIdx.x * (64 / a.T);
     const bool second = a.kv2 && sample0 >= a.nsamples / 2;
     unsigned voffKV[4];
-    if constexpr (NPW > 0) {
+    if constexpr (NPW > 0 && !PK) {
       const int kv_rows = (64 / a.T) * a.Tk;
       const int bstr = second ? 0 : a.kv_bstride;
 #pragma unroll
@@ -112,12 +141,30 @@
       }
     }
     const int rowb = blockIdx.x * 64;
-    auto pieces_of = [&](unsigned d) -> int { return (NPW > 0 && (d & 2u)) ? NPW : IPT; };
+    auto pieces_of = [&](unsigned d) -> int { return (NPW > 0 && (d & 2u)) ? (PK && !KVP_TWO ? 2 * NPW : NPW) : IPT; };
     auto issue_tile = [&](int tau, unsigned d) {
       unsigned char* slot = smem + MDT_SLOT_IDX(tau) * SLOT + iw * 1024;
       const unsigned kind = d & 3u, aux = d >> 2;
-      if (NPW > 0 && kind >= 2u) {
-        if constexpr (NPW > 0) {
+      if (PK && kind >= 2u) {
+        if constexpr (PK) {
+          const int64_t ck = (int64_t)(aux >> 4) * a.nheads + (int64_t)(aux & 15u);
+          const unsigned char* base = (second ? a.kvp2 + ck * (kvp::FIXED_GROUPS * CH)
+                                              : a.kvp + (ck * a.kvp_groups + (int64_t)blockIdx.x * a.kvp_gstep) * CH) + iw * 1024 + lane * 16;
+          if constexpr (KVP_TWO) {
+#pragma unroll
+            for (int q = 0; q < NPW; ++q) {
+              const int L = q * 4096 + iw * 1024 + lane * 16;
+              const unsigned char* src = base - (iw * 1024 + lane * 16) + (L / (2 * PB)) * CH + (kind == 3u ? 2 * PB : 0) + L % (2 * PB);
+              __builtin_amdgcn_global_load_lds(src, (__attribute__((address_space(3))) void*)(slot + q * 4096), 16, 0, MDT_KV_CPOL);
+            }
+          } else {
+#pragma unroll
+          for (int q = 0; q < 2 * NPW; ++q)
+            __builtin_amdgcn_global_load_lds(base + q * 4096, (__attribute__((address_space(3))) void*)(slot + q * 4096), 16, 0, MDT_KV_CPOL);
+          }
+        }
+      } else if (NPW > 0 && kind >= 2u) {
+        if constexpr (NPW > 0 && !PK) {
           const int layer = (int)(aux >> 4), head = (int)(aux & 15u);
           const float* lb = second ? a.kv2 + (int64_t)layer * a.kv2_lstride
                                    : a.kv + (int64_t)layer * a.kv_lstride + (int64_t)sample0 * a.kv_bstride * a.ldkv;
@@ -161,7 +208,15 @@
         default: asm volatile("s_waitcnt vmcnt(8)" ::: "memory"); break;
       }
     };
-    const unsigned d0 = tiles[0], d1 = NT > 1 ? tiles[1] : 0u;
+    constexpr unsigned END = 0xffffffffu;
+    int pos = 0;
+    auto fetch = [&]() -> unsigned {
+      if (pos >= NT) return END;
+      const unsigned d = tiles[pos];
+      pos += (!KVP_TWO && (d & 3u) == 2u) ? 2 : 1;
+      return d;
+    };
+    const unsigned d0 = PK ? fetch() : tiles[0], d1 = PK ? fetch() : (NT > 1 ? tiles[1] : 0u);
     __builtin_amdgcn_s_barrier();
     for (int q = iw; q * 256 < a.nvec; q += 4)
       __builtin_amdgcn_global_load_lds(reinterpret_cast<const unsigned char*>(a.vec) + q * 1024 + lane * 16,
@@ -172,8 +227,20 @@
                                          (__attribute__((address_space(3))) void*)(smem + NS * SLOT + a.nvec * 4 + q * 1024), 16, 0, 0);
     }
     issue_tile(0, d0);
-    if (NT > 1) issue_tile(1, d1);
+    if (PK ? d1 != END : NT > 1) issue_tile(1, d1);
     unsigned dn = d1;
+    if constexpr (PK) {
+      for (int k = 0;; ++k) {
+        const unsigned d2 = fetch();
+        if (dn != END && pieces_of(dn) == IPT) asm volatile("s_waitcnt vmcnt(8)" ::: "memory");
+        else if (dn != END) asm volatile("s_waitcnt vmcnt(%0)" ::"n"(PK ? (KVP_TWO ? NPW : 2 * NPW) : 1) : "memory");
+        else asm volatile("s_waitcnt vmcnt(0)" ::: "memory");
+        __builtin_amdgcn_s_barrier();
+        if (dn == END) break;
+        if (d2 != END) issue_tile(k + 2, d2);
+        dn = d2;
+      }
+    } else
     for (int k = 0; k < NT; ++k) {
       const unsigned d2 = k + 2 < NT ? tiles[k + 2] : 0u;
       if (k + 1 < NT && pieces_of(dn) == IPT) asm volatile("s_waitcnt vmcnt(8)" ::: "memory");
@@ -567,7 +634,17 @@
   const float scale2 = a.scale * 1.44269504088896340736f;
   int aK = 0, xK = 0, aV[4] = {0, 0, 0, 0}, xV[4] = {0, 0, 0, 0};
   bool kok[4] = {false, false, false, false};
-  if constexpr (NPW > 0) {
+  int aKp = 0, aVp = 0;
+  if constexpr (PK) {
+    const int nkeys = (16 / a.T) * a.Tk;
+    aKp = wave * (KVP_TWO ? 2 * PB : CH) + kvp::k_read_offset(NKP, nkeys, 0, 0, i, g);
+    aVp = wave * (KVP_TWO ? 2 * PB : CH) + kvp::v_read_offset(NKP, 0, 0, i, g) - (KVP_TWO ? 2 * PB : 0);
+#pragma unroll
+    for (int r = 0; r < 4; ++r) {
+      const int jj = 4 * g + r;
+      kok[r] = jj < nkeys && (jj / a.Tk) == samp_q;
+    }
+  } else if constexpr (NPW > 0) {
     const int nkeys = (16 / a.T) * a.Tk;
     const int Rw = wave * nkeys;
     const int Rk = Rw + min(i, nkeys - 1);
@@ -715,6 +792,65 @@
         for (int ft = 0; ft < 4; ++ft) qT[ft] = zero4;
         phase(kT, IC0{}, kT, false, qT, xh, xl);
         __builtin_amdgcn_s_barrier();
+        if constexpr (PK) {
+          const unsigned char* sk = slot_of(tau);
+          bf16x8 kh[2], kl[2];
+          bf16x4 vh[4], vl[4];
+#pragma unroll
+          for (int sp = 0; sp < 2; ++sp) {
+            kh[sp] = *reinterpret_cast<const bf16x8*>(sk + aKp + sp * (NKP * 64));
+            kl[sp] = *reinterpret_cast<const bf16x8*>(sk + aKp + PB + sp * (NKP * 64));
+          }
+          if constexpr (!KVP_TWO) {
+#pragma unroll
+            for (int dt = 0; dt < 4; ++dt) {
+              vh[dt] = *reinterpret_cast<const bf16x4*>(sk + aVp + dt * (32 * NKP));
+              vl[dt] = *reinterpret_cast<const bf16x4*>(sk + aVp + PB + dt * (32 * NKP));
+            }
+          }
+          {
+            f32x4 bq[4];
+            lds_read_f4_off<0>(bq[0], bias_l + 256 * h); lds_read_f4_off<64>(bq[1], bias_l + 256 * h);
+            lds_read_f4_off<128>(bq[2], bias_l + 256 * h); lds_read_f4_off<192>(bq[3], bias_l + 256 * h);
+            lgkm_wait<0>();
+#pragma unroll
+            for (int ft = 0; ft < 4; ++ft) qT[ft] += bq[ft];
+          }
+          const f32x4 s0 = scores_packed(kh, kl, qT);
+          if constexpr (KVP_TWO) {
+            ++tau;
+            __builtin_amdgcn_s_barrier();
+            const unsigned char* sv = slot_of(tau);
+#pragma unroll
+            for (int dt = 0; dt < 4; ++dt) {
+              vh[dt] = *reinterpret_cast<const bf16x4*>(sv + aVp + dt * (32 * NKP));
+              vl[dt] = *reinterpret_cast<const bf16x4*>(sv + aVp + PB + dt * (32 * NKP));
+            }
+          }
+          f32x4 st;
+          float mx = -INFINITY;
+#pragma unroll
+          for (int r = 0; r < 4; ++r) {
+            const float sv2 = kok[r] ? s0[r] * scale2 : -INFINITY;
+            st[r] = sv2;
+            mx = fmaxf(mx, sv2);
+          }
+          mx = xg16_max(mx);
+          mx = xg32_max(mx);
+          float sum = 0.f;
+#pragma unroll
+          for (int r = 0; r < 4; ++r) {
+            const float e = __builtin_amdgcn_exp2f(st[r] - mx);
+            st[r] = e;
+            sum += e;
+          }
+          sum = xg16_add(sum);
+          sum = xg32_add(sum);
+          const float inv = __builtin_amdgcn_rcpf(sum);
+          const float p[4] = {st[0] * inv, st[1] * inv, st[2] * inv, st[3] * inv};
+          pv_split(vh, vl, p, oT);
+          asm volatile("s_waitcnt lgkmcnt(0)" ::: "memory");
+        } else {
         const unsigned char* sk = slot_of(tau);
         float4 kk[4];
 #pragma unroll
@@ -742,7 +878,13 @@
           f32x4 kf[4];
 #pragma unroll
           for (int ft = 0; ft < 4; ++ft) kf[ft] = f32x4{kk[ft].x, kk[ft].y, kk[ft].z, kk[ft].w};
+#ifdef MDT_ABL_KVSPLIT
+          const bf16x8 ka[2] = {__builtin_bit_cast(bf16x8, kf[0]), __builtin_bit_cast(bf16x8, kf[2])};
+          const bf16x8 kb[2] = {__builtin_bit_cast(bf16x8, kf[1]), __builtin_bit_cast(bf16x8, kf[3])};
+          s0 = scores_packed(ka, kb, qT);
+#else
           s0 = scores_split(kf, qT);
+#endif
         }
 #endif
         ++tau;
@@ -759,7 +901,18 @@
         for (int dt = 0; dt < 4; ++dt) oT[dt] = qT[dt] + f32x4{kk[dt].x, kk[dt].y, kk[dt].z, kk[dt].w} + vT[dt] + s0 + s1;
 #else
         bf16x4 vh[4], vl[4];
+#ifdef MDT_ABL_KVSPLIT
+        if constexpr (!F32) {
+#pragma unroll
+          for (int dt = 0; dt < 4; ++dt) {
+            typedef float f32x2 __attribute__((ext_vector_type(2)));
+            vh[dt] = __builtin_bit_cast(bf16x4, f32x2{vT[dt][0], vT[dt][1]});
+            vl[dt] = __builtin_bit_cast(bf16x4, f32x2{vT[dt][2], vT[dt][3]});
+          }
+        }
+#else
         if constexpr (!F32) split_v(vT, vh, vl);
+#endif
         f32x4 st;
         float mx = -INFINITY;
 #pragma unroll
@@ -795,6 +948,7 @@
         }
 #endif
         asm volatile("s_waitcnt lgkmcnt(0)" ::: "memory");
+        }
         ++tau;
         __builtin_amdgcn_s_barrier();
         prefetch2(kO, slot_of(tau), 1);
@@ -864,21 +1018,32 @@
   }
 }
 
-template <int NPW, int RES, bool F32>
+template <int NPW, int RES, bool F32, bool PK = false>
 static hipError_t launch_tf(const TFArgs& a, hipStream_t s) {
   const size_t smem = (size_t)NS * SLOT + (size_t)(a.nvec + (RES > 0 ? a.nfilm : 0)) * sizeof(float);
   static DevOnce attr_once;
   if (attr_once.first()) {
-    (void)hipFuncSetAttribute(reinterpret_cast<const void*>(&k_tf128<NPW, RES, F32>), hipFuncAttributeMaxDynamicSharedMemorySize,
+    (void)hipFuncSetAttribute(reinterpret_cast<const void*>(&k_tf128<NPW, RES, F32, PK>), hipFuncAttributeMaxDynamicSharedMemorySize,
                               (int)(160 * 1024));
   }
-  hipLaunchKernelGGL((k_tf128<NPW, RES, F32>), dim3((unsigned)((a.M + 63) / 64)), dim3(512), smem, s, a);
+  hipLaunchKernelGGL((k_tf128<NPW, RES, F32, PK>), dim3((unsigned)((a.M + 63) / 64)), dim3(512), smem, s, a);
   return hipGetLastError();
 }
 
 template <int RES, bool F32>
 static hipError_t launch_tf_res(const TFArgs& a, hipStream_t s, bool cross) {
   if (!cross) return launch_tf<0, RES, F32>(a, s);
+  if constexpr (!F32) {
+    if (a.kvp != nullptr && (a.kv2 == nullptr || a.kvp2 != nullptr)) {
+      switch (((64 / a.T) * a.Tk + 15) / 16) {
+        case 1: return launch_tf<1, RES, F32, true>(a, s);
+        case 2: return launch_tf<2, RES, F32, true>(a, s);
+        case 3: return launch_tf<3, RES, F32, true>(a, s);
+        case 4: return launch_tf<4, RES, F32, true>(a, s);
+        default: return hipErrorInvalidValue;
+      }
+    }
+  }
   switch (((64 / a.T) * a.Tk + 15) / 16) {
     case 1: return launch_tf<1, RES, F32>(a, s);
     case 2: return launch_tf<2, RES, F32>(a, s);
diff --git a/moleculediffusiontransformer_amd/csrc/mdt_api.cpp b/moleculediffusiontransformer_amd/csrc/mdt_api.cpp
--- a/moleculediffusiontransformer_amd/csrc/mdt_api.cpp
+++ b/moleculediffusiontransformer_amd/csrc/mdt_api.cpp
@@ -8,6 +8,7 @@
 
 #include "../../include/mdt_hip.h"
 #include "mdt_kernels.h"
+#include "mdt_kv_pack.h"
 
 namespace {
 thread_local std::string g_err;
@@ -555,6 +556,21 @@
         a.xflags = a.nsplit == 2 ? reinterpret_cast<unsigned*>(const_cast<float*>(ptr(o.p2))) : nullptr;
         a.xbuf = a.nsplit == 2 ? const_cast<float*>(ptr(o.p3)) : nullptr;
         a.wf32 = i[MDT_F_WF32]; a.rb_base = 0;
+        a.kvp = a.kvp2 = nullptr; a.kvp_groups = a.kvp_gstep = 0;
+        if (!wide && i[MDT_F_CROSS] && !i[MDT_F_WF32] && o.p2.space >= MDT_SP_EXT0 && o.p2.space + 1 < MDT_SP_EXT0 + MDT_N_EXT) {
+          const int nkp = mdt::kvp::padded_slots(a.T, a.Tk);
+          const int64_t groups = mdt::kvp::groups_of(B, a.T);
+          const unsigned char* per_sample = reinterpret_cast<const unsigned char*>(bd->ext[o.p2.space - MDT_SP_EXT0]);
+          const unsigned char* fixed = reinterpret_cast<const unsigned char*>(bd->ext[o.p2.space + 1 - MDT_SP_EXT0]);
+          if (per_sample) per_sample += o.p2.off * mdt::kvp::layer_bytes(groups, a.nheads, nkp);
+          if (fixed) fixed += o.p2.off * mdt::kvp::layer_bytes(mdt::kvp::FIXED_GROUPS, a.nheads, nkp);
+          const bool own = a.kv_bstride != 0;
+          const unsigned char* first = own ? per_sample : fixed;
+          if (first && (!i[MDT_F_KV2] || fixed)) {
+            a.kvp = first; a.kvp_groups = own ? (int)groups : mdt::kvp::FIXED_GROUPS; a.kvp_gstep = own ? 4 : 0;
+            a.kvp2 = i[MDT_F_KV2] ? fixed : nullptr;
+          }
+        }
         if (i[MDT_F_KV2]) {
           const int per_wg = (wide ? 32 : 64) / a.T;
           if (!o.p1.space || B % 2 || (B / 2) % (per_wg > 0 ? per_wg : 1))
diff --git a/moleculediffusiontransformer_amd/csrc/mdt_kernels.h b/moleculediffusiontransformer_amd/csrc/mdt_kernels.h
--- a/moleculediffusiontransformer_amd/csrc/mdt_kernels.h
+++ b/moleculediffusiontransformer_amd/csrc/mdt_kernels.h
@@ -3,7 +3,7 @@
 #include <stdint.h>
 
 #if (defined(MDT_ABL_BAR) || defined(MDT_ABL_VMWAIT) || defined(MDT_ABL_LGKM) || defined(MDT_ABL_LDSBC) || defined(MDT_ABL_GELU) ||     \
-     defined(MDT_ABL_ATTN) || defined(MDT_ABL_ATTNX) || defined(MDT_RING_NODRAIN) || defined(MDT_STAGGER) || defined(MDT_XH_D2) ||                               \
+     defined(MDT_ABL_ATTN) || defined(MDT_ABL_ATTNX) || defined(MDT_ABL_KVSPLIT) || defined(MDT_RING_NODRAIN) || defined(MDT_STAGGER) || defined(MDT_XH_D2) ||                               \
      (defined(MDT_XH_ADDR) && MDT_XH_ADDR == 0) || (defined(MDT_XH_MODE) && MDT_XH_MODE != 0)) &&                                       \
     !defined(MDT_TUNING)
 #error "MDT_ABL_* / MDT_RING_NODRAIN / MDT_STAGGER / MDT_XH_D2 / MDT_XH_ADDR=0 / MDT_XH_MODE!=0 give wrong results: timing builds only, add -DMDT_TUNING"
@@ -289,6 +289,9 @@
   unsigned* xflags;
   int wf32;
   int rb_base;
+  const unsigned char* kvp;
+  const unsigned char* kvp2;
+  int kvp_groups, kvp_gstep;
 };
 bool tf128_supported(int T, int Tk, int nvec, bool cross);
 hipError_t launch_tf128(const TFArgs& a, hipStream_t s);
diff --git a/moleculediffusiontransformer_amd/csrc/mdt_kv_pack.h b/moleculediffusiontransformer_amd/csrc/mdt_kv_pack.h
--- /dev/null
+++ b/moleculediffusiontransformer_amd/csrc/mdt_kv_pack.h
@@ -0,0 +1,121 @@
+#pragma once
+
+namespace mdt {
+namespace kvp {
+
+constexpr int imin(int a, int b) { return a < b ? a : b; }
+constexpr int live_slots(int T, int Tk) { return (16 / T) * Tk; }
+constexpr int padded_slots(int T, int Tk) { return (live_slots(T, Tk) + 3) & ~3; }
+constexpr int plane_bytes(int nkp) { return 128 * nkp; }
+constexpr int chunk_bytes(int nkp) { return 512 * nkp; }
+constexpr long long groups_of(long long B, int T) { return (B * T + 63) / 64 * 4; }
+constexpr int FIXED_GROUPS = 4;
+constexpr long long layer_bytes(long long groups, int nheads, int nkp) { return groups * nheads * chunk_bytes(nkp); }
+
+constexpr int k_elem_offset(int nkp, int plane, int ks, int f) {
+  return plane * plane_bytes(nkp) + (f >> 5) * (nkp * 64) + ks * 64 + ((f >> 2) & 3) * 16 + ((((f >> 4) & 1) << 2) | (f & 3)) * 2;
+}
+constexpr int v_elem_offset(int nkp, int plane, int ks, int f) {
+  return (2 + plane) * plane_bytes(nkp) + (f >> 4) * (32 * nkp) + (f & 15) * (2 * nkp) + ks * 2;
+}
+constexpr int slot_live(int nk, int ks) { return imin(ks, nk - 1); }
+
+constexpr int k_read_offset(int nkp, int nk, int plane, int sp, int i, int g) {
+  return plane * plane_bytes(nkp) + sp * (nkp * 64) + imin(i, nk - 1) * 64 + g * 16;
+}
+constexpr int v_read_offset(int nkp, int plane, int dt, int i, int g) {
+  return (2 + plane) * plane_bytes(nkp) + dt * (32 * nkp) + i * (2 * nkp) + imin(g, nkp / 4 - 1) * 8;
+}
+
+inline unsigned f32_bits(float x) {
+  unsigned u;
+  __builtin_memcpy(&u, &x, 4);
+  return u;
+}
+inline float bits_f32(unsigned u) {
+  float x;
+  __builtin_memcpy(&x, &u, 4);
+  return x;
+}
+inline unsigned short bf16_rne(float x) {
+  const unsigned u = f32_bits(x);
+  if ((u & 0x7fffffffu) > 0x7f800000u) return (unsigned short)((u >> 16) | 0x40u);
+  return (unsigned short)((u + 0x7fffu + ((u >> 16) & 1u)) >> 16);
+}
+inline void split_host(float x, unsigned short& hi, unsigned short& lo) {
+  hi = bf16_rne(x);
+  lo = bf16_rne(x - bits_f32((unsigned)hi << 16));
+}
+
+struct Walk {
+  long long barriers = 0, slots = 0;
+};
+inline Walk walk_loader(const unsigned* tiles, int nt, bool pk) {
+  Walk w;
+  w.barriers = 1;
+  for (int k = 0; k < nt;) {
+    const unsigned kind = tiles[k] & 3u;
+    k += (pk && kind == 2u) ? 2 : 1;
+    ++w.barriers;
+    ++w.slots;
+  }
+  return w;
+}
+struct Shape {
+  int res_kind, n_res, has_in, nblocks, nheads, nff, npost, cross;
+};
+inline Walk walk_compute(const Shape& s, bool pk) {
+  Walk w;
+  auto phase = [&](bool has_next) { w.slots += 1; w.barriers += has_next ? 1 : 0; };
+  auto barrier = [&]() { w.barriers += 1; };
+  auto conv3 = [&](bool has_next) {
+    for (int k = 0; k < 5; ++k) phase(true);
+    phase(has_next);
+  };
+  auto skip_rows = [&]() { barrier(); w.slots += 1; barrier(); };
+  barrier();
+  barrier();
+  const bool tf_follows = s.has_in || s.nblocks > 0;
+  for (int rb = 0; rb < s.n_res; ++rb) {
+    const bool more = rb + 1 < s.n_res || tf_follows;
+    if (s.res_kind == 1) {
+      conv3(true);
+      conv3(more);
+    } else {
+      phase(true); phase(false);
+      skip_rows();
+      phase(true); phase(true);
+      conv3(false);
+      skip_rows();
+      conv3(true);
+      conv3(more);
+    }
+  }
+  if (s.has_in) { phase(true); phase(false); barrier(); }
+  for (int blk = 0; blk < s.nblocks; ++blk) {
+    const bool last_blk = blk + 1 == s.nblocks;
+    for (int h = 0; h < s.nheads; ++h) { phase(true); phase(true); phase(false); barrier(); phase(true); }
+    if (s.cross)
+      for (int h = 0; h < s.nheads; ++h) {
+        phase(false);
+        barrier();
+        w.slots += 1;
+        if (!pk) { barrier(); w.slots += 1; }
+        barrier();
+        phase(true);
+      }
+    const int npost = last_blk ? s.npost : 0;
+    for (int h = 0; h < s.nff; ++h) {
+      const bool more = h + 1 < s.nff;
+      phase(false);
+      barrier();
+      if (npost > 0 && !more) phase(true);
+      else phase(more || !last_blk);
+    }
+    if (npost > 0) { phase(true); phase(false); }
+  }
+  return w;
+}
+
+}
+}
diff --git a/moleculediffusiontransformer_amd/engine.py b/moleculediffusiontransformer_amd/engine.py
--- a/moleculediffusiontransformer_amd/engine.py
+++ b/moleculediffusiontransformer_amd/engine.py
@@ -7,7 +7,7 @@
 import torch
 
 from . import runtime as rt
-from .compiler import EXT_CTX, EXT_FILM, EXT_OUT, EXT_XBUF, EXT_XFLAGS, EXT_XIN, CompiledUNet
+from .compiler import EXT_CTX, EXT_FILM, EXT_KVP, EXT_KVP_FIXED, EXT_OUT, EXT_XBUF, EXT_XFLAGS, EXT_XIN, CompiledUNet
 
 
 def _require_gpu(device: torch.device) -> None:
@@ -56,6 +56,8 @@
         self._graphs: Dict[str, torch.cuda.CUDAGraph] = {}
         self._time_rows = 0
         self._fixed_ready = False
+        self.kvp = self.kvp_fixed = None
+        self._kvp_ready = self._kvp_fixed_ready = False
 
     def reserve(self, B: int) -> None:
         if B == self.B:
@@ -69,6 +71,9 @@
         self.pred_fixed = torch.zeros(B, c.length, c.in_pad, device=self.device)
         self.xflags = self.xbuf = None
         self.film = torch.empty(B, c.ss_total, device=self.device) if c.rows else None
+        self.kvp, self._kvp_ready = None, False
+        if c.kv_pack and B > 0:
+            self.kvp = torch.empty(self._kvp_bytes(B, False), dtype=torch.uint8, device=self.device)
         if c.xchg_tokens:
             nrb = (B * c.xchg_tokens + 31) // 32
             self.xflags = torch.zeros(64 + 64 * nrb + (8 * 4096 + 16384 if os.environ.get("MDT_XH_LOG") else 0), dtype=torch.int32,
@@ -82,7 +87,28 @@
         b.ext[EXT_XIN], b.ext[EXT_CTX], b.ext[EXT_OUT] = rt.ptr(xin), rt.ptr(ctx), rt.ptr(out)
         b.ext[EXT_XFLAGS], b.ext[EXT_XBUF] = rt.ptr(getattr(self, "xflags", None)), rt.ptr(getattr(self, "xbuf", None))
         b.ext[EXT_FILM] = rt.ptr(getattr(self, "film", None))
+        b.ext[EXT_KVP] = rt.ptr(self.kvp if self._kvp_ready else None)
+        b.ext[EXT_KVP_FIXED] = rt.ptr(self.kvp_fixed if self._kvp_fixed_ready else None)
         return b
+
+    def _kvp_bytes(self, B: int, fixed: bool) -> int:
+        k = self.c.kv_pack
+        return int(rt.load_library().mdt_kv_pack_bytes(k["layers"], B, k["T"], k["Tk"], k["heads"], int(fixed)))
+
+    def _kv_pack(self, fixed: bool) -> None:
+        k = self.c.kv_pack
+        lib, B = rt.load_library(), self.B
+        table = self.kvp_fixed if fixed else self.kvp
+        per_layer = table.numel() // k["layers"]
+        for cross0, layers, packed0 in k["runs"]:
+            if fixed:
+                src = self.shr.data_ptr() + 4 * (k["kv_fixed"] + cross0 * k["lstride"])
+                lstride, bstride = k["lstride"], 0
+            else:
+                src = self.act.data_ptr() + 4 * (k["kv"] + cross0 * k["lstride"]) * B
+                lstride, bstride = k["lstride"] * B, k["Tk"]
+            rt.check(lib.mdt_kv_pack(src, table.data_ptr() + packed0 * per_layer, layers, lstride, B, k["T"], k["Tk"], k["ldkv"],
+                                     k["heads"], bstride, rt.current_stream()))
 
     sync_handoff_check = True
 
@@ -167,11 +193,23 @@
         emb = embedding.to(device=self.device, dtype=torch.float32).contiguous()
         assert emb.shape[1] == self.c.cond_len and emb.shape[2] == self.c.cfg.ctx_features, emb.shape
         self.programs["ctx"].run(self._bind(ctx=emb), B)
+        if self.kvp is not None:
+            self._kv_pack(False)
+            if not self._kvp_ready:
+                self._graphs.clear()
+            self._kvp_ready = True
 
     def prepare_fixed(self) -> None:
         if not self._fixed_ready:
             self.programs["ctx_fixed"].run(self._bind(), max(self.B, 1))
             self._fixed_ready = True
+            self._kvp_fixed_ready = False
+        if self.c.kv_pack and not self._kvp_fixed_ready and self.B > 0:
+            if self.kvp_fixed is None:
+                self.kvp_fixed = torch.empty(self._kvp_bytes(1, True), dtype=torch.uint8, device=self.device)
+            self._kv_pack(True)
+            self._graphs.clear()
+            self._kvp_fixed_ready = True
 
     @property
     def has_dual(self) -> bool:
diff --git a/moleculediffusiontransformer_amd/runtime.py b/moleculediffusiontransformer_amd/runtime.py
--- a/moleculediffusiontransformer_amd/runtime.py
+++ b/moleculediffusiontransformer_amd/runtime.py
@@ -106,6 +106,8 @@
     "mdt_init_noise": (_I, [_P, _P, _F, _U64, _U32, _L, _I, _I, _I, _P]),
     "mdt_clamp": (_I, [_P, _F, _F, _L, _P]),
     "mdt_copy_f32": (_I, [_P, _P, _L, _P]),
+    "mdt_kv_pack_bytes": (_L, [_I, _I, _I, _I, _I, _I]),
+    "mdt_kv_pack": (_I, [_P, _P, _I, _L, _I, _I, _I, _I, _I, _I, _P]),
     "mdt_inpaint_merge": (_I, [_P, _P, _P, _P, _F, _U64, _U32, _L, _I, _I, _I, _P]),
     "mdt_add_noise": (_I, [_P, _P, _F, _U64, _U32, _L, _I, _I, _I, _P]),
     "mdt_inpaint_enter": (_I, [_P, _P, _P, _P, _P, _I, _P, _P, _F, _F, _F, _U64, _U32, _U32, _L, _I, _I, _I, _I, _P]),
```
